# chongminggao/CIRS-codes

Hardware: AMD Instinct MI355X
Metric: simulator env-steps/s (collect + PPO update in the timed region), KuaishouEnv (higher is better)
Workload: dtype f32 (policy/tracker; rollout on the fp32 MFMA, PPO head products fp32-accurate from two fp16 pieces per operand (3 f16 MFMAs per product), fp32 accumulate) + f64 (env rewards, GAE)

## Files before the change

cirs-codes_amd/csrc/ppo.hip:

```cpp
#include "internal.h"
#include "optim.h"
#include "bf16x6.h"
#include "small_gemm.h"
#include "permutation.h"
#include "policy_kernels.h"

namespace cirs {
typedef float f32x4 __attribute__((ext_vector_type(4)));


constexpr int kBwdWaves = 4;
__host__ __device__ inline int n_row_blocks_of(int n_pad) { return (n_pad / kTileM + kBwdWaves - 1) / kBwdWaves; }
__host__ __device__ inline size_t dwa_slab_stride(int I) { return (((size_t)I * 64 + I) + 3) & ~(size_t)3; }
__host__ __device__ inline int n_dwa_slabs_of(int n_pad) { return n_row_blocks_of(n_pad); }

struct PpoLayout {
    long w1, b1, w2, b2, wa, ba, wc, bc, total, trunk;
};
__host__ __device__ inline PpoLayout ppo_layout(int I, int S) {
    PpoLayout L;
    L.w1 = 0; L.b1 = L.w1 + (long)kH * S; L.w2 = L.b1 + kH; L.b2 = L.w2 + (long)kH * kH;
    L.trunk = L.b2 + kH;
    L.wa = L.trunk; L.ba = L.wa + (long)I * kH; L.wc = L.ba + I; L.bc = L.wc + kH; L.total = L.bc + 1;
    return L;
// ... 350 lines not shown
#pragma unroll
    for (int off = 32; off > 0; off >>= 1) {
        const float om = __shfl_xor(m, off, CIRS_WAVE), os = __shfl_xor(s, off, CIRS_WAVE), ot = __shfl_xor(t, off, CIRS_WAVE);
        const float mn = fmaxf(m, om);
        if (mn > -INFINITY) {
            const float fa = __expf(m - mn), fb = __expf(om - mn);
            s = s * fa + os * fb; t = t * fa + ot * fb; m = mn;
        }
    }
    sRow[threadIdx.x >> 6][0][lane] = hl;
    sRow[threadIdx.x >> 6][1][lane] = wl;
    __builtin_amdgcn_wave_barrier();
    if (lane != 0) return;
    const float* hr = sRow[threadIdx.x >> 6][0];
    const float* wr = sRow[threadIdx.x >> 6][1];
    float z;
    if (za_in) {
        z = 0.f;
        for (int c = 0; c < n_chunks; ++c) {
            const float zc = za_in[(size_t)c * n_pad + j];
            if (zc == zc) z = zc;
        }
    } else {
        z = ba[a];
#pragma unroll
        for (int kk = 0; kk < 32; ++kk) {
            z = __builtin_fmaf(hr[kk], wr[kk], z);
            z = __builtin_fmaf(hr[32 + kk], wr[32 + kk], z);
        }
    }
    const float lse = m + __logf(s);
    v.lse[j] = lse;
    v.act[j] = a - item_base;
    v.dst_row[j] = (long)b.row_t[src] * n_env + b.row_env[src];
    const RowTerms rt = ppo_row_terms(cfg, z, lse, t / s, b.logp_old[src], b.adv[src], v.red[0], v.red[1], v.value[j], b.v_s[src], b.ret[src],
                                      1.0f / (float)mb_norm);
    v.clip_row[j] = rt.clip_row; v.c_logp[j] = rt.c_logp; v.vf_row[j] = rt.vf_row; v.dvalue[j] = rt.dvalue;
    v.c_ent[j] = rt.c_ent; v.h_ent[j] = rt.h_ent;
}

__device__ __forceinline__ float dz_of(float z, float lse, float c_logp, float c_ent, float h_ent, bool is_act, float& p_out) {
    const float p = __expf(z - lse);
    p_out = p;
    return c_logp * ((is_act ? 1.0f : 0.0f) - p) + c_ent * p * (z - lse + h_ent);
}

__device__ __forceinline__ void st_sc1(float* p, float a) { __hip_atomic_store(p, a, __ATOMIC_RELAXED, __HIP_MEMORY_SCOPE_AGENT); }
__device__ __forceinline__ float ld_sc1(const float* p) { return __hip_atomic_load(p, __ATOMIC_RELAXED, __HIP_MEMORY_SCOPE_AGENT); }
__device__ __forceinline__ float2 ld_sc1x2(const float* p) {
    const unsigned long long u = __hip_atomic_load(reinterpret_cast<const unsigned long long*>(p), __ATOMIC_RELAXED, __HIP_MEMORY_SCOPE_AGENT);
    return make_float2(__uint_as_float((unsigned)u), __uint_as_float((unsigned)(u >> 32)));
}
typedef unsigned wt_u32x4 __attribute__((ext_vector_type(4)));
struct WtBuf { __amdgpu_buffer_rsrc_t r; };
__device__ __forceinline__ WtBuf wt_buf(const void* base, unsigned bytes) {
    const unsigned long long a = reinterpret_cast<unsigned long long>(base);
    const unsigned lo = __builtin_amdgcn_readfirstlane((unsigned)a), hi = __builtin_amdgcn_readfirstlane((unsigned)(a >> 32));
    return WtBuf{__builtin_amdgcn_make_buffer_rsrc(reinterpret_cast<void*>(((unsigned long long)hi << 32) | lo), 0, (int)bytes, 0x00020000)};
}
__device__ __forceinline__ void st_wt16(const WtBuf& b, int byte_off, f32x4 x) {
    __builtin_amdgcn_raw_buffer_store_b128(__builtin_bit_cast(wt_u32x4, x), b.r, byte_off, 0, 16);
}
__device__ __forceinline__ void st_wt16(const WtBuf& b, int byte_off, uint4 x) { st_wt16(b, byte_off, __builtin_bit_cast(f32x4, x)); }

template <bool kWt = false> __device__ __forceinline__ void wa_planes_from_lds(int tile, uint4* __restrict__ planes, const float* sw);
__device__ __forceinline__ void wa_planes_block(int tile, int I, const float* __restrict__ wa, uint4* __restrict__ planes, float* sw) {
    const int tid = threadIdx.x, tile0 = tile * kTileN;
#pragma unroll
    for (int q = 0; q < 2; ++q) {
        const int f = tid + 256 * q, item = f >> 4, col = (f & 15) * 4;
        float4 t4 = make_float4(0.f, 0.f, 0.f, 0.f);
        if (tile0 + item < I) t4 = *reinterpret_cast<const float4*>(wa + (size_t)(tile0 + item) * kH + col);
        float* d = &sw[item * 65 + col];
        d[0] = t4.x; d[1] = t4.y; d[2] = t4.z; d[3] = t4.w;
    }
    __syncthreads();
    wa_planes_from_lds(tile, planes, sw);
}
template <bool kWt> __device__ __forceinline__ void wa_planes_from_lds(int tile, uint4* __restrict__ planes, const float* sw) {
    const int tid = threadIdx.x;
    uint4* out = planes + (size_t)tile * kPlaneTileU4;
    const WtBuf ob = wt_buf(out, kPlaneTileU4 * 16);
    {
        const float* r = &sw[(tid >> 3) * 65 + 8 * (tid & 7)];
        const HPl pl = hsplit8(kScWa * r[0], kScWa * r[1], kScWa * r[2], kScWa * r[3], kScWa * r[4], kScWa * r[5], kScWa * r[6], kScWa * r[7]);
        if constexpr (kWt) { st_wt16(ob, 16 * tid, __builtin_bit_cast(uint4, pl.h)); st_wt16(ob, 16 * (512 + tid), __builtin_bit_cast(uint4, pl.l)); }
        else { out[tid] = __builtin_bit_cast(uint4, pl.h); out[512 + tid] = __builtin_bit_cast(uint4, pl.l); }
    }
    {
        const int n = tid >> 2, t = (tid >> 1) & 1, hi = tid & 1;
        float x[8];
#pragma unroll
        for (int j = 0; j < 8; ++j) x[j] = kScWa * sw[acc_row(8 * t + j, hi) * 65 + n];
        const HPl pl = hsplit8(x[0], x[1], x[2], x[3], x[4], x[5], x[6], x[7]);
        if constexpr (kWt) { st_wt16(ob, 16 * (768 + tid), __builtin_bit_cast(uint4, pl.h)); st_wt16(ob, 16 * (1280 + tid), __builtin_bit_cast(uint4, pl.l)); }
        else { out[768 + tid] = __builtin_bit_cast(uint4, pl.h); out[1280 + tid] = __builtin_bit_cast(uint4, pl.l); }
    }
}

struct TrunkRowOut {
    float *h2, *value, *h1, *obs_copy;
    int32_t* act; long* dst;
    float* row4;
    uint4 *h2z, *h2b;
};
struct TrunkLds { const float* w1; int ld1; const float* w2; const float* wc; };

struct TrunkRowIn { int ri; float x; };
__device__ __forceinline__ TrunkRowIn trunk_row_gather(int j, int mb, const int32_t* __restrict__ idx, const float* __restrict__ obs_flat, long stride, int S,
                                                       int lane) {
    TrunkRowIn in;
    in.ri = idx[j < mb ? j : mb - 1];
    in.x = (j < mb && lane < S) ? obs_flat[(size_t)in.ri * stride + lane] : 0.f;
    return in;
}
__device__ __forceinline__ void trunk_row_pre(int S, const TrunkRowIn& in, int j, int mb, int n_pad, int lane, float* xs, const cirs_ppo_batch& bt, int n_env,
                                              const TrunkRowOut& o) {
    if (lane < S) {
        xs[lane] = in.x;
        o.obs_copy[(size_t)j * S + lane] = in.x;
    }
    if (o.act) {
        if (lane == 0) {
            o.act[j] = j < mb ? bt.act[in.ri] : 0;
            o.dst[j] = j < mb ? (long)bt.row_t[in.ri] * n_env + bt.row_env[in.ri] : 0;
        } else if (lane <= 4) {
            const float* srcp = lane == 1 ? bt.adv : lane == 2 ? bt.logp_old : lane == 3 ? bt.ret : bt.v_s;
            o.row4[(size_t)(lane - 1) * n_pad + j] = j < mb ? srcp[in.ri] : 0.f;
        }
    }
}
__device__ __forceinline__ void trunk_row_planes(float a, int j, int lane, const TrunkRowOut& o) {
    a *= kScH2;
    const uint32_t hp = cvt_pk_f16(a, 0.f) & 0xffffu;
    const float r1 = a - (float)__builtin_bit_cast(f16x2_b, hp).x;
    const uint32_t lp = cvt_pk_f16(r1, 0.f) & 0xffffu;
    const int tile = j >> 5, rr = j & 31, c = lane;
    unsigned short* z = reinterpret_cast<unsigned short*>(o.h2z + ((size_t)(tile * 12 + (c >> 4) * 3) * 64 + ((c >> 3) & 1) * 32 + rr)) + (c & 7);
    z[0] = (unsigned short)hp; z[2 * 64 * 8] = (unsigned short)lp;
    const int hi_b = (rr >> 2) & 1, sb = (rr & 3) + 4 * (rr >> 3);
    unsigned short* bq = reinterpret_cast<unsigned short*>(o.h2b + ((size_t)(tile * 12 + ((c >> 5) * 2 + (sb >> 3)) * 3) * 64 + hi_b * 32 + (c & 31))) + (sb & 7);
    bq[0] = (unsigned short)hp; bq[2 * 64 * 8] = (unsigned short)lp;
}
__device__ __forceinline__ void trunk_row_job(const cirs_policy_cfg& cfg, const cirs_policy_weights& w, const TrunkLds& L, const TrunkRowIn& in, int j, int mb,
                                              int n_pad, int lane, float* xs, float* hs, const cirs_ppo_batch& bt, int n_env, const TrunkRowOut& o) {
    trunk_row_pre(cfg.dim_state, in, j, mb, n_pad, lane, xs, bt, n_env, o);
    trunk_compute(cfg, w, xs, hs, lane, j, o.h2, o.value, o.h1, L.w1, L.ld1, L.w2, L.wc);
    trunk_row_planes(xs[lane], j, lane, o);
}
__global__ __launch_bounds__(256) void trunk_adv_kernel(cirs_policy_cfg cfg, cirs_policy_weights w, const float* __restrict__ obs_flat,
                                                        long stride, int n_pad, const int32_t* __restrict__ idx, int mb,
                                                        const float* __restrict__ adv_flat, const int32_t* __restrict__ sidx,
                                                        int m_stats, int enable, float* __restrict__ red, int n_row_wgs,
                                                        uint4* __restrict__ planes, cirs_ppo_batch bt, int n_env, TrunkRowOut out) {
    __shared__ float lds_raw[kTileN * 65];
    static_assert(kTileN * 65 >= 4 * 2 * kH, "the trunk rows use 4 x 2 x 64 floats of the same buffer");
    if ((int)blockIdx.x > n_row_wgs) {
        wa_planes_block((int)blockIdx.x - n_row_wgs - 1, cfg.n_items, w.wa, planes, lds_raw);
        return;
    }
    if ((int)blockIdx.x == n_row_wgs) {
        adv_stats_block(adv_flat, sidx, m_stats, enable, red, lds_raw);
        return;
    }
    __shared__ __attribute__((aligned(16))) float sW2[kH * kLdsRow2];
    __shared__ float sW1[kH * 33];
    __shared__ float sWc[kH];
    const int tid = threadIdx.x, lane = tid & 63, wv = tid >> 6, S = cfg.dim_state;
    const int j = blockIdx.x * 4 + wv;
    const int ld1 = S | 1;
    const bool al16 = (reinterpret_cast<uintptr_t>(w.w2) & 15) == 0;
    f32x4 t2[4];
    float t1[8];
#pragma unroll
    for (int q = 0; q < 4; ++q) {
        const float* p = w.w2 + (size_t)(tid + 256 * q) * 4;
        t2[q] = al16 ? *reinterpret_cast<const f32x4*>(p) : f32x4{p[0], p[1], p[2], p[3]};
    }
#pragma unroll
    for (int q = 0; q < 8; ++q) t1[q] = tid + 256 * q < kH * S ? w.w1[tid + 256 * q] : 0.f;
    const float tc = tid < kH ? w.wc[tid] : 0.f;
    const TrunkRowIn in = trunk_row_gather(j, mb, idx, obs_flat, stride, S, lane);
#pragma unroll
    for (int q = 0; q < 4; ++q) {
        const int i4 = tid + 256 * q;
        *reinterpret_cast<f32x4*>(&sW2[(i4 >> 4) * kLdsRow2 + (i4 & 15) * 4]) = t2[q];
    }
#pragma unroll
    for (int q = 0; q < 8; ++q) {
        const int i = tid + 256 * q;
        if (i < kH * S) sW1[(i / S) * ld1 + (i % S)] = t1[q];
    }
    if (tid < kH) sWc[tid] = tc;
    float (*rows)[2][kH] = reinterpret_cast<float (*)[2][kH]>(lds_raw);
    __syncthreads();
    trunk_row_job(cfg, w, TrunkLds{sW1, ld1, sW2, sWc}, in, j, mb, n_pad, lane, rows[wv][0], rows[wv][1], bt, n_env, out);
}

constexpr int kTStride = 36;
constexpr int kRSize = kTileN * kH + 2 * kTileN;
constexpr int kRowB = 144, kColB = 80;
constexpr int kRPlaneB = kTileN * kRowB, kCPlaneB = kH * kColB;
constexpr int kWBufB = 3 * kRPlaneB + 3 * kCPlaneB;

#ifdef CIRS_HEAD_PROF
__device__ unsigned long long g_step_prof[64];
#define CIRS_PSTAMP(COND, K) do { if ((COND) && threadIdx.x == 0) g_step_prof[K] = __builtin_amdgcn_s_memtime(); } while (0)
#else
#define CIRS_PSTAMP(COND, K) do { } while (0)
#endif
#ifdef CIRS_HEAD_PROF
__device__ unsigned long long g_head_prof[64];
#define CIRS_HSTAMP(K) do { if (blockIdx.x == 0 && blockIdx.y == 0 && threadIdx.x == 0 && it == 2) g_head_prof[K] = __builtin_amdgcn_s_memtime(); } while (0)
#define CIRS_HSTAMPB(K) do { if (blockIdx.x == 0 && blockIdx.y == 0 && threadIdx.x == 256 && it == 3) g_head_prof[K] = __builtin_amdgcn_s_memtime(); } while (0)
#define CIRS_TSTAMP(B, K) do { if ((int)blockIdx.x == (B) && threadIdx.x == 0) g_head_prof[K] = __builtin_amdgcn_s_memtime(); } while (0)
#define CIRS_SSTAMP(K) do { if (blockIdx.x == 0 && blockIdx.y == 0 && threadIdx.x == 0) g_head_prof[K] = __builtin_amdgcn_s_memtime(); } while (0)
#else
#define CIRS_HSTAMP(K) do { } while (0)
#define CIRS_HSTAMPB(K) do { } while (0)
#define CIRS_TSTAMP(B, K) do { } while (0)
#define CIRS_SSTAMP(K) do { } while (0)
#endif
template <bool kZout>
__global__ __launch_bounds__(256, 2) void head_stats_kernel(int I, int mb, int n_pad, int tiles_per_chunk,
                                                            const uint4* __restrict__ planes, const float* __restrict__ ba,
                                                            const uint4* __restrict__ h2z, ActorPartialView pv,
                                                            const int32_t* __restrict__ act_rows, float* __restrict__ za_out,
                                                            float4* __restrict__ zslab) {
    __shared__ __attribute__((aligned(16))) unsigned char sW[2][3 * kRPlaneB];
    __shared__ __attribute__((aligned(16))) float sB[2][kTileN];
    const int tid = threadIdx.x;
    CIRS_SSTAMP(40);
    const int lane = tid & 63, wv = tid >> 6;
    const int hi = lane >> 5, lo = lane & 31;
    const int row0 = (blockIdx.y * 4 + wv) * kTileM;
    const int chunk = blockIdx.x;
    const int jr = row0 + lo;
    const bool wave_ok = row0 < n_pad && (kZout || row0 < mb);
    const bool active = jr < mb;
    HPl hz[4];
    {
        const uint4* zp = h2z + (size_t)((wave_ok ? row0 : 0) >> 5) * 12 * 64 + lane;
#pragma unroll
        for (int s4 = 0; s4 < 4; ++s4) {
            HPL_SET(hz[s4], zp[(3 * s4) * 64], zp[(3 * s4 + 2) * 64]);
        }
    }
    float run_m = -INFINITY, run_s = 0.f, run_t = 0.f;
    const int act_r = (act_rows && active) ? act_rows[jr] : -1;
    float za_val = 0.f;
    bool za_have = false;
    const int first_tile = chunk * tiles_per_chunk * kTileN;
    const int n_tiles = max(0, min(tiles_per_chunk, (I - first_tile + kTileN - 1) / kTileN));
    const int dst_r = (tid >> 3) * kRowB + (tid & 7) * 16;
    uint4 g0, g2;
    float gb = 0.f;
#define CIRS_ISSUE(TILE0)                                                                                  \
    do {                                                                                                   \
        const uint4* src_ = planes + (size_t)((TILE0) / kTileN) * kPlaneTileU4 + tid;                      \
        g0 = src_[0]; g2 = src_[512];                                             \
        if (tid < kTileN) gb = ((TILE0) + tid) < I ? kScZ * ba[(TILE0) + tid] : 0.f;    \
    } while (0)
#define CIRS_COMMIT(BUF)                                                                                   \
    do {                                                                                                   \
        unsigned char* base_ = sW[BUF];                                                                    \
        *reinterpret_cast<uint4*>(base_ + dst_r) = g0;                                                     \
        \
        *reinterpret_cast<uint4*>(base_ + 2 * kRPlaneB + dst_r) = g2;                                      \
        if (tid < kTileN) sB[BUF][tid] = gb;                                                               \
    } while (0)
    CIRS_SSTAMP(41);
    if (n_tiles > 0) { CIRS_ISSUE(first_tile); CIRS_COMMIT(0); }
    __syncthreads();
    CIRS_SSTAMP(42);
    for (int it = 0; it < n_tiles; ++it) {
        const int buf = it & 1;
        const int tile0 = first_tile + it * kTileN;
        if (it == 2) CIRS_SSTAMP(43);
        if (it + 1 < n_tiles) CIRS_ISSUE(tile0 + kTileN);
        if (wave_ok) {
            const unsigned char* tw = sW[buf];
            HPl za[4];
#pragma unroll
            for (int s4 = 0; s4 < 4; ++s4) {
                const unsigned char* ap = tw + lo * kRowB + (16 * s4 + 8 * hi) * 2;
                HPL_SET(za[s4], *reinterpret_cast<const uint4*>(ap), *reinterpret_cast<const uint4*>(ap + 2 * kRPlaneB));
            }
            f32x16 acc, accs, acct;
#pragma unroll
            for (int r = 0; r < 16; ++r) { acc[r] = sB[buf][acc_row(r, hi)]; accs[r] = 0.f; acct[r] = 0.f; }
            if (it == 2) CIRS_SSTAMP(44);
            hmfma_split2(za[0], hz[0], za[1], hz[1], acc, accs, acct);
            hmfma_split2(za[2], hz[2], za[3], hz[3], acc, accs, acct);
#pragma unroll
            for (int r = 0; r < 16; ++r) acc[r] = acc[r] + (accs[r] + acct[r]);
            if (kZout) {
                const WtBuf zb = wt_buf(zslab + ((size_t)(tile0 / kTileN) * (n_pad / kTileM) + (row0 / kTileM)) * kZTileF4, kZTileF4 * 16);
#pragma unroll
                for (int q = 0; q < 4; ++q) st_wt16(zb, 16 * (q * 64 + lane), f32x4{acc[4 * q], acc[4 * q + 1], acc[4 * q + 2], acc[4 * q + 3]});
            }
#pragma unroll
            for (int r = 0; r < 16; ++r) acc[r] *= kScZi;
            if (it == 2) CIRS_SSTAMP(45);
            {
                const int arel = act_r - tile0;
                const bool mine = act_r >= 0 && arel >= 0 && arel < kTileN && ((arel >> 2) & 1) == hi;
                if (__any(mine)) {
                    const int rsel = (arel & 3) + 4 * (arel >> 3);
                    float zsel = acc[0];
// ... 1750 lines not shown
        }
    }
    acc = block_sum<256>(acc, sh);
    if (tid == 0) stats[blockIdx.x] = acc;
    if (blockIdx.x == 0 && tid < 8) {
        const long gi = P + tid;
        stats[kShardNormBlocks + tid] = (tid < 4 && gi >= begin && gi < begin + len) ? g_shard[gi - begin] : 0.f;
    }
}
__global__ __launch_bounds__(256) void shard_adam_kernel(float* __restrict__ p, const float* __restrict__ g, float* __restrict__ m,
                                                         float* __restrict__ v, long begin, long len, long n_first, long P, AdamSeg sa,
                                                         AdamSeg sb, float beta1, float beta2, float eps, cirs_ppo_cfg cfg,
                                                         const float* __restrict__ stats_all, int world, float* __restrict__ loss_out) {
    __shared__ float sh[256];
    const int tid = threadIdx.x;
    float acc = 0.f;
    const int n_part = world * kShardNormBlocks;
    for (int q = tid; q < n_part; q += 256) acc += stats_all[(size_t)(q / kShardNormBlocks) * kShardStatFloats + (q % kShardNormBlocks)];
    float total_norm;
    const float c = norm_coef(block_sum<256>(acc, sh), cfg, total_norm);
    if (blockIdx.x == 0 && tid == 0 && loss_out) {
        float t3[3] = {0.f, 0.f, 0.f};
        for (int r = 0; r < world; ++r)
            for (int j = 0; j < 3; ++j) t3[j] += stats_all[(size_t)r * kShardStatFloats + kShardNormBlocks + j];
        write_loss_row(loss_out, cfg, t3[0], t3[1], t3[2]);
    }
    const long i = blockIdx.x * (long)blockDim.x + threadIdx.x;
    if (i >= len || begin + i >= P) return;
    const AdamSeg sg = begin + i < n_first ? sa : sb;
    float gi = g[i];
    float pi = p[i], mi = m[i], vi = v[i];
    adam_elem_seg(pi, mi, vi, gi, sg, c, beta1, beta2, eps);
    p[i] = pi; m[i] = mi; v[i] = vi;
}

static int launch_adam(float* p, const float* g, float* m, float* v, long n, long step_before, int n_sub, float lr, float b1,
                       float b2, float eps, const float* grad_scale, int scale_pow, hipStream_t s) {
    CIRS_REQUIRE(n_sub == 1 || n_sub == 2, "n_sub must be 1 or 2");
    AdamBias ab[2] = {{0.f, 1.f, 1.f}, {0.f, 1.f, 1.f}};
    for (int q = 0; q < n_sub; ++q) ab[q] = adam_bias(lr, b1, b2, step_before + 1 + q);
    hipLaunchKernelGGL(adam_kernel, dim3(cdiv(n, 256)), dim3(256), 0, s, p, g, m, v, n, n_sub, b1, b2, eps, ab[0].step_size, ab[0].bc2s,
                       ab[1].step_size, ab[1].bc2s, grad_scale, scale_pow);
    CIRS_CHECK_LAUNCH("adam_kernel");
    return CIRS_OK;
}

#ifdef CIRS_HEAD_PROF
extern "C" int cirs_debug_step_prof(unsigned long long* out_host64) {
    return hipMemcpyFromSymbol(out_host64, HIP_SYMBOL(cirs::g_step_prof), 64 * sizeof(unsigned long long)) == hipSuccess ? 0 : -2;
}
extern "C" int cirs_debug_head_prof(unsigned long long* out_host32) {
    return hipMemcpyFromSymbol(out_host32, HIP_SYMBOL(cirs::g_head_prof), 64 * sizeof(unsigned long long)) == hipSuccess ? 0 : -2;
}
#endif

static int validate_ppo(const cirs_ppo_cfg* cfg) {
    CIRS_REQUIRE(cfg, "ppo cfg null");
    if (cfg->hidden != kH) return fail(CIRS_E_UNSUPPORTED, "this build supports hidden == 64 only");
    CIRS_REQUIRE(cfg->n_items > 0 && cfg->dim_state > 0 && cfg->dim_state <= 64, "bad n_items/dim_state");
    return CIRS_OK;
}

}

extern "C" int64_t cirs_ppo_param_count(const cirs_ppo_cfg* cfg) {
    if (!cfg) return 0;
    return cirs::ppo_layout(cfg->n_items, cfg->dim_state).total;
}

extern "C" int64_t cirs_ppo_workspace_bytes(const cirs_ppo_cfg* cfg, int32_t max_minibatch) {
    using namespace cirs;
    if (!cfg || max_minibatch <= 0) return 0;
    return (int64_t)(mb_ws_floats(n_pad_of(max_minibatch), cfg->n_items, cfg->dim_state) + 64 * 32) * 4;
}

extern "C" int cirs_ppo_prepare(const cirs_ppo_cfg* cfg, const cirs_traj* traj, const int32_t* lens,
                                const int32_t* offsets, int32_t n_env, int32_t max_turn, int32_t n_rows,
                                double* rms_state, const cirs_ppo_batch* out, void* stream) {
    using namespace cirs;
    if (int rc = validate_ppo(cfg)) return rc;
    CIRS_REQUIRE(traj && lens && offsets && rms_state && out, "null argument");
    CIRS_REQUIRE(out->obs && out->act && out->adv && out->ret && out->v_s && out->logp_old && out->row_env && out->row_t, "batch pointer null");
    CIRS_REQUIRE(n_env > 0 && max_turn > 0 && n_rows > 0, "bad sizes");
    hipStream_t s = (hipStream_t)stream;
    double* unnorm = nullptr;
    CIRS_HIP(hipMallocAsync((void**)&unnorm, sizeof(double) * (size_t)n_rows, s));
    hipLaunchKernelGGL(gae_kernel, dim3(cdiv(n_env, 64)), dim3(64), 0, s, *cfg, *traj, lens, offsets, n_env, cfg->dim_state,
                       rms_state, *out, unnorm);
    hipLaunchKernelGGL(compact_obs_kernel, dim3(cdiv((long)n_rows * cfg->dim_state, 256)), dim3(256), 0, s, *traj, *out, n_rows, n_env, cfg->dim_state);
    CIRS_CHECK_LAUNCH("gae_kernel");
    hipLaunchKernelGGL(returns_kernel, dim3(1), dim3(1024), 0, s, *cfg, unnorm, n_rows, rms_state, out->ret);
    CIRS_CHECK_LAUNCH("returns_kernel");
    CIRS_HIP(hipFreeAsync(unnorm, s));
    return CIRS_OK;
}

extern "C" int cirs_ppo_prepare_async_perms(const cirs_ppo_cfg* cfg, const cirs_traj* traj, const int32_t* lens, int32_t n_env, int32_t max_turn,
                                            int32_t* offsets_out, int32_t* n_rows_out, double* rms_state, const cirs_ppo_batch* out,
                                            double* scratch, uint64_t perm_seed, uint64_t perm_tag0, int32_t n_perm, int32_t* perm_out, int32_t offsets_ready,
                                            void* stream) {
    using namespace cirs;
    if (int rc = validate_ppo(cfg)) return rc;
    CIRS_REQUIRE(traj && lens && offsets_out && n_rows_out && rms_state && out && scratch, "null argument");
    CIRS_REQUIRE(out->obs && out->act && out->adv && out->ret && out->v_s && out->logp_old && out->row_env && out->row_t, "batch pointer null");
    CIRS_REQUIRE(n_env > 0 && n_env <= (1 << 20) && max_turn > 0, "bad sizes");
    CIRS_REQUIRE(n_perm >= 0 && n_perm <= kMaxPermKeys && (n_perm == 0 || perm_out), "permutations: at most 8 per call, perm_out non-null");
    hipStream_t s = (hipStream_t)stream;
    if (!offsets_ready) hipLaunchKernelGGL(offsets_kernel, dim3(1), dim3(1024), 0, s, lens, n_env, offsets_out, n_rows_out);
    hipLaunchKernelGGL(gae_kernel, dim3(cdiv(n_env, 64)), dim3(64), 0, s, *cfg, *traj, lens, (const int32_t*)offsets_out, n_env, cfg->dim_state,
                       rms_state, *out, scratch);
    const long upper = (long)n_env * max_turn;
    const int n_compact = (int)cdiv(upper * cfg->dim_state, 1024L);
    PermKeys keys{};
    for (int q = 0; q < n_perm; ++q) keys.k[q] = perm_key(perm_seed, perm_tag0 + (uint64_t)q);
    hipLaunchKernelGGL(prepare_tail_kernel, dim3(1 + n_compact + (int)cdiv((long)n_perm * upper, 1024L)), dim3(1024), 0, s, *cfg, *traj, *out, (const double*)scratch,
                       rms_state, (const int32_t*)n_rows_out, n_env, cfg->dim_state, n_compact, keys, (int)n_perm, upper, perm_out);
    CIRS_CHECK_LAUNCH("cirs_ppo_prepare_async");
    return CIRS_OK;
}
extern "C" int cirs_ppo_prepare_async(const cirs_ppo_cfg* cfg, const cirs_traj* traj, const int32_t* lens, int32_t n_env, int32_t max_turn,
                                      int32_t* offsets_out, int32_t* n_rows_out, double* rms_state, const cirs_ppo_batch* out,
                                      double* scratch, void* stream) {
    return cirs_ppo_prepare_async_perms(cfg, traj, lens, n_env, max_turn, offsets_out, n_rows_out, rms_state, out, scratch, 0, 0, 0, nullptr, 0, stream);
}

extern "C" int cirs_adam_step(float* params, const float* grads, float* m, float* v, int64_t n, int64_t step_before,
                              int32_t n_sub, float lr, float beta1, float beta2, float eps, const float* grad_scale,
                              int32_t scale_pow, void* stream) {
    using namespace cirs;
    CIRS_REQUIRE(params && grads && m && v && n > 0, "bad arguments");
    return launch_adam(params, grads, m, v, n, step_before, n_sub, lr, beta1, beta2, eps, grad_scale, scale_pow, (hipStream_t)stream);
}

struct PpoRun {
    const cirs_ppo_cfg* cfg;
    float *params, *grads, *adam_m, *adam_v;
    const cirs_ppo_batch* batch;
    int n_env;
    void* workspace;
    int n_pad_carve;
    hipStream_t s;
    int I, S;
    cirs::PpoLayout L;
    cirs_policy_cfg pcfg;
    cirs_policy_weights w;
    cirs::MbView v;
    float* tail;
    bool merge_launch;
    bool head_recompute;
    bool rows_kernel;
    bool learn_prefetch;
    int drop_arrival;
};
struct PpoStep { const int32_t* idx; int mb; const int32_t* sidx; int mb_norm; float* dobs; float* loss_out; long opt_step; };

static int env_int(const char* name, int unset) {
    const char* e = getenv(name);
    return e ? atoi(e) : unset;
}
static PpoRun ppo_run(const cirs_ppo_cfg* cfg, float* params, float* grads, float* adam_m, float* adam_v, const cirs_ppo_batch* batch, int n_env,
                      void* workspace, int max_mb, hipStream_t s) {
    using namespace cirs;
    PpoRun r;
    r.cfg = cfg; r.params = params; r.grads = grads; r.adam_m = adam_m; r.adam_v = adam_v; r.batch = batch; r.n_env = n_env; r.workspace = workspace;
    r.n_pad_carve = n_pad_of(max_mb); r.s = s; r.I = cfg->n_items; r.S = cfg->dim_state;
    r.L = ppo_layout(r.I, r.S);
    r.pcfg = cirs_policy_cfg{r.I, r.S, kH};
    r.w = cirs_policy_weights{params + r.L.w1, params + r.L.b1, params + r.L.w2, params + r.L.b2, params + r.L.wa, params + r.L.ba, params + r.L.wc,
                              params + r.L.bc};
    r.v = carve(workspace, r.n_pad_carve, r.I, r.S);
    r.tail = grads + r.L.total;
    r.merge_launch = env_int("CIRS_PPO_MERGE_KERNEL", 0) != 0;
    r.head_recompute = env_int("CIRS_PPO_HEAD_RECOMPUTE", 0) != 0;
    r.rows_kernel = env_int("CIRS_PPO_ROWS_KERNEL", 1) != 0;
    r.learn_prefetch = env_int("CIRS_PPO_LEARN_PREFETCH", 1) != 0;
    r.drop_arrival = env_int("CIRS_PPO_TEST_DROP_ARRIVAL", 0);
    return r;
}
static cirs::TrunkRowOut trunk_out_of(const cirs::MbView& v) { return cirs::TrunkRowOut{v.h2, v.value, v.h1, v.obs, v.act, v.dst_row, v.adv, v.h2z, v.h2b}; }
static long head_seg(const PpoRun& r) { return (long)r.I * cirs::kH + r.I; }

static int launch_trunk_adv(const PpoRun& r, const PpoStep& st, const cirs::TrunkRowOut& out) {
    using namespace cirs;
    const int n_pad = n_pad_of(st.mb);
    hipLaunchKernelGGL(trunk_adv_kernel, dim3(cdiv(n_pad, 4) + 1 + cdiv(r.I, kTileN)), dim3(256), 0, r.s, r.pcfg, r.w, (const float*)r.batch->obs, (long)r.S,
                       n_pad, st.idx, st.mb, (const float*)r.batch->adv, st.sidx, st.mb_norm, (int)r.cfg->norm_adv, r.v.red, (int)cdiv(n_pad, 4),
                       r.v.wa_planes, *r.batch, r.n_env, out);
    CIRS_CHECK_LAUNCH("trunk_adv_kernel");
    return CIRS_OK;
}
static int launch_head_stats(const PpoRun& r, const PpoStep& st, const int32_t* act_rows, float* za_out, cirs::HeadMergeArgs* hma) {
    using namespace cirs;
    const int n_pad = n_pad_of(st.mb), n_slabs = n_row_blocks_of(n_pad), n_item_tiles = cdiv(r.I, kTileN);
    const int tpc_s = head_tiles_per_chunk(n_item_tiles, n_slabs, 2);
    const int n_schunks = cdiv(n_item_tiles, tpc_s);
    *hma = HeadMergeArgs{*r.cfg, *r.batch, st.idx, st.mb_norm, n_schunks, partial_view(r.v.head_ws, n_pad, r.I)};
    const auto stats_fn = r.head_recompute ? head_stats_kernel<false> : head_stats_kernel<true>;
    CIRS_PROF_LAUNCH(2, r.s, hipLaunchKernelGGL(stats_fn, dim3(n_schunks, n_slabs), dim3(256), 0, r.s, r.I, st.mb, n_pad, tpc_s, (const uint4*)r.v.wa_planes,
                                                r.w.ba, (const uint4*)r.v.h2z, hma->pv, act_rows, za_out, r.v.zslab));
    CIRS_CHECK_LAUNCH("head_stats_kernel");
    return CIRS_OK;
}
static int launch_head_bwd(const PpoRun& r, const PpoStep& st, const cirs::HeadMergeArgs& hma, bool merge, int* n_bchunks_out) {
    using namespace cirs;
    const int n_pad = n_pad_of(st.mb), n_slabs = n_row_blocks_of(n_pad), n_item_tiles = cdiv(r.I, kTileN);
    const int tpc = head_tiles_per_chunk(n_item_tiles, n_slabs, 1);
    const int n_bchunks = cdiv(n_item_tiles, tpc);
    const dim3 bgrid((n_bchunks + 7) & ~7, n_slabs), bblock(head_bwd_threads(!r.head_recompute));
    const HeadBwdFn bwd_fn = head_bwd_fn(r.cfg->ent_coef != 0.f, merge, !r.head_recompute);
    CIRS_PROF_LAUNCH(1, r.s, hipLaunchKernelGGL(bwd_fn, bgrid, bblock, 0, r.s, r.I, st.mb, n_pad, tpc, (const uint4*)r.v.wa_planes, (const float*)r.w.ba, r.v,
                                                r.v.dwap, hma));
    CIRS_CHECK_LAUNCH("head_bwd_fused_kernel");
    *n_bchunks_out = n_bchunks;
    return CIRS_OK;
}
static int launch_dh2_sum(const PpoRun& r, const PpoStep& st, int n_bchunks, float* tp_dh2 = nullptr, float* tp_ent = nullptr) {
    using namespace cirs;
    const int n_pad = n_pad_of(st.mb);
    hipLaunchKernelGGL(dh2_sum_kernel, dim3(n_pad * (kH / 4) / 64 + cdiv(n_pad, 64)), dim3(64), 0, r.s, st.mb, n_pad, n_bchunks, r.v, tp_dh2, tp_ent);
    CIRS_CHECK_LAUNCH("dh2_sum_kernel");
    return CIRS_OK;
}
static cirs::DwJobs trunk_dw_jobs(const PpoRun& r, int n_pad) {
    using namespace cirs;
    const MbView& v = r.v;
    DwJobs jobs{};
    jobs.n = 3;
    jobs.j[0] = DwJob{v.dvalue, 1, v.h2, kH, 1, kH, r.grads + r.L.wc, r.grads + r.L.bc, 0, 0};
    jobs.j[1] = DwJob{v.da2, kH, v.h1, kH, kH, kH, r.grads + r.L.w2, r.grads + r.L.b2, 0, 0};
    jobs.j[2] = DwJob{v.da1, kH, v.obs, r.S, kH, r.S, r.grads + r.L.w1, r.grads + r.L.b1, 0, 0};
    const int n_dw_slabs = n_pad / kTileM;
    int off = 0, out = 0;
    for (int q = 0; q < 3; ++q) {
        jobs.j[q].part_off = off;
        off += n_dw_slabs * jobs.j[q].O * (jobs.j[q].K + 1);
        out += jobs.j[q].O * (jobs.j[q].K + 1);
    }
    jobs.total_out = out;
    return jobs;
}
static int launch_trunk_bwd(const PpoRun& r, const PpoStep& st, const cirs::MbView& v, int n_chunks, bool wa_sum) {
    using namespace cirs;
    static_assert(kH == 64, "trunk_bwd_kernel tiles assume hidden == 64");
    CIRS_REQUIRE(r.S <= 32, "dim_state > 32 is not supported by the trunk backward kernel");
    const int n_pad = n_pad_of(st.mb), n_slabs = n_row_blocks_of(n_pad);
    hipLaunchKernelGGL(trunk_bwd_kernel, dim3(n_pad / kTileM + (wa_sum ? kWaSumBlocks : 0)), dim3(512), 0, r.s, st.mb, n_pad, n_chunks, r.S, r.w.w1, r.w.w2,
                       r.w.wc, v, st.dobs, r.grads, (long)r.L.wa, head_seg(r), (long)dwa_slab_stride(r.I), n_slabs, trunk_dw_jobs(r, n_pad), v.dwp);
    CIRS_CHECK_LAUNCH("trunk_bwd_kernel");
    return CIRS_OK;
}
static bool rows_kernel_wanted(const PpoRun& r, int mb) {
    return cirs::n_pad_of(mb) / cirs::kRR <= cirs::kSyncA0 && r.rows_kernel;
}
static int launch_trunk_rows(const PpoRun& r, const PpoStep& st, int n_bchunks, bool with_loss_partials) {
    using namespace cirs;
    CIRS_REQUIRE(r.S <= 32, "dim_state > 32 is not supported by the trunk backward kernel");
    const int n_pad = n_pad_of(st.mb), n_slabs = n_row_blocks_of(n_pad);
    const long seg = head_seg(r);
    const int n_r = n_pad / kRR, n_f = cdiv(snap_floats(r.S), kFOut);
    CIRS_REQUIRE(n_r <= kSyncA0, "trunk_rows_kernel: more than 2048 rows in a minibatch (one arrival flag per 8 rows)");
    const long n4 = seg >> 2;
    int n_w = (int)cdiv(n4, 512L);
    n_w = n_w > kWaSlotsMax ? kWaSlotsMax : n_w;
    n_w = std::min(n_w, std::max(64, device_cu_count() - n_r));
    hipLaunchKernelGGL(trunk_rows_kernel, dim3(n_r + n_w + n_f + (with_loss_partials ? 1 : 0)), dim3(512), 0, r.s, st.mb, n_pad, n_bchunks, r.S, r.w.w1,
                       r.w.w2, r.w.wc, r.v, st.dobs, r.grads, (long)r.L.wa, seg, (long)dwa_slab_stride(r.I), n_slabs, n_r, snap_stride(r.S),
                       with_loss_partials ? r.tail : (float*)nullptr, st.mb_norm, n_w);
    CIRS_CHECK_LAUNCH("trunk_rows_kernel");
    return CIRS_OK;
}
static int launch_dw_final_loss(const PpoRun& r, const PpoStep& st) {
    using namespace cirs;
    const int n_pad = n_pad_of(st.mb);
    const DwJobs jobs = trunk_dw_jobs(r, n_pad);
    hipLaunchKernelGGL(dw_multi_final, dim3(cdiv(jobs.total_out, 256)), dim3(256), 0, r.s, jobs, n_pad / kTileM, (const float*)r.v.dwp);
    CIRS_CHECK_LAUNCH("dw_multi_final");
    hipLaunchKernelGGL(loss_partials_kernel, dim3(1), dim3(256), 0, r.s, st.mb, st.mb_norm, r.v, r.tail);
    CIRS_CHECK_LAUNCH("loss_partials_kernel");
    return CIRS_OK;
}
static int launch_sumsq(const PpoRun& r, const PpoStep& st, bool from_slabs) {
    using namespace cirs;
    const int n_pad = n_pad_of(st.mb);
    const DwJobs jobs = from_slabs ? trunk_dw_jobs(r, n_pad) : DwJobs{};
    hipLaunchKernelGGL(sumsq_partial_kernel, dim3(kNormBlocks), dim3(256), 0, r.s, r.grads, r.L.trunk, r.L.total, r.L.wa, head_seg(r), (int)from_slabs, jobs,
                       from_slabs ? n_pad / kTileM : 0, from_slabs ? (const float*)r.v.dwp : (const float*)nullptr, r.S, r.v.normp);
    CIRS_CHECK_LAUNCH("sumsq_partial_kernel");
    return CIRS_OK;
}
static cirs::AdamSeg adam_seg_of(const cirs_ppo_cfg* cfg, long step_before, int n_sub, int scale_pow) {
    cirs::AdamSeg sg{n_sub, scale_pow, 0.f, 1.f, 0.f, 1.f, 1.f, 1.f};
    for (int q = 0; q < n_sub; ++q) {
        const cirs::AdamBias ab = cirs::adam_bias(cfg->lr, cfg->beta1, cfg->beta2, step_before + 1 + q);
        if (q == 0) { sg.step_size0 = ab.step_size; sg.bc2s0 = ab.bc2s; sg.rbc2s0 = ab.rbc2s; }
        else { sg.step_size1 = ab.step_size; sg.bc2s1 = ab.bc2s; sg.rbc2s1 = ab.rbc2s; }
    }
    return sg;
}
static int launch_norm_adam(const PpoRun& r, const PpoStep& st, int phase, bool folded, const PpoStep* next) {
    using namespace cirs;
    const MbView& v = r.v;
    if (!(phase == 0 && folded)) { if (int rc = launch_sumsq(r, st, phase == 0)) return rc; }
    const AdamSeg sa = adam_seg_of(r.cfg, 2 * st.opt_step, 2, 2), sb = adam_seg_of(r.cfg, st.opt_step, 1, 1);
    AdamNext nx{};
    nx.n_p = cdiv(r.I, kTileN);
    nx.planes = v.wa_planes;
    if (next) {
        const int np = n_pad_of(next->mb);
        nx.n_t = np / kTrunkRowsPerWg; nx.n_s = 1;
        nx.pcfg = r.pcfg; nx.obs_flat = r.batch->obs; nx.idx = next->idx; nx.mb = next->mb; nx.n_pad = np;
        nx.adv_flat = r.batch->adv; nx.sidx = next->sidx; nx.m_stats = next->mb_norm; nx.enable = (int)r.cfg->norm_adv; nx.red = v.red;
        nx.bt = *r.batch; nx.n_env = r.n_env; nx.out = trunk_out_of(v); nx.s_magic = (65536 + r.S - 1) / r.S;
        nx.drop_arrival = r.drop_arrival;
    }
    nx.n_a0 = cdiv(r.L.trunk + kH + 1, 256);
    const int n_a = nx.n_a0 + cdiv(r.I, 256);
    const AdamArgs aa{r.params, r.grads, r.adam_m, r.adam_v, r.L, sa, sb, r.cfg->beta1, r.cfg->beta2, r.cfg->adam_eps, *r.cfg, v.normp, r.tail, st.loss_out,
                      phase == 0 ? st.mb : 0, st.mb_norm};
    hipLaunchKernelGGL(adam_next_kernel, dim3(nx.n_t + nx.n_s + nx.n_p + n_a), dim3(256), 0, r.s, aa, v, nx);
    CIRS_CHECK_LAUNCH("adam_next_kernel");
    return CIRS_OK;
}

static int launch_step_grads(const PpoRun& r, const PpoStep& st, bool head_done, bool for_allreduce) {
    using namespace cirs;
    const int n_pad = n_pad_of(st.mb);
    HeadMergeArgs hma;
    int n_bchunks = 0;
    if (!head_done) { if (int rc = launch_trunk_adv(r, st, trunk_out_of(r.v))) return rc; }
    if (int rc = launch_head_stats(r, st, r.v.act, r.v.za, &hma)) return rc;
    if (r.merge_launch) {
        hipLaunchKernelGGL(head_stats_merge_kernel, dim3(cdiv(n_pad, 4)), dim3(256), 0, r.s, *r.cfg, *r.batch, st.idx, st.mb, st.mb_norm, n_pad, hma.n_schunks,
                           r.n_env, hma.pv, r.w.wa, r.w.ba, r.v, (const float*)nullptr, 0);
        CIRS_CHECK_LAUNCH("head_stats_merge_kernel");
    }
    if (int rc = launch_head_bwd(r, st, hma, !r.merge_launch, &n_bchunks)) return rc;
    if (rows_kernel_wanted(r, st.mb)) return launch_trunk_rows(r, st, n_bchunks, for_allreduce);
    if (int rc = launch_dh2_sum(r, st, n_bchunks)) return rc;
    if (int rc = launch_trunk_bwd(r, st, r.v, n_bchunks, true)) return rc;
    return for_allreduce ? launch_dw_final_loss(r, st) : CIRS_OK;
}
static int launch_step(const PpoRun& r, const PpoStep& st, bool head_done, const PpoStep* next) {
    if (int rc = launch_step_grads(r, st, head_done, false)) return rc;
    return launch_norm_adam(r, st, 0, rows_kernel_wanted(r, st.mb), next);
}

struct DpChain { int max_mb; int head_done; const int32_t* next_idx; int next_mb; const int32_t* next_idx_global; int next_mb_global; };
static int ppo_minibatch_impl(const cirs_ppo_cfg* cfg, float* params, float* grads, float* adam_m, float* adam_v, int64_t opt_step,
                              const cirs_ppo_batch* batch, const int32_t* idx, int32_t mb, const int32_t* idx_global,
                              int32_t mb_global, float* dobs_accum, int32_t n_env, float* loss_out, void* workspace,
                              int64_t workspace_bytes, int phase, void* stream, const DpChain* ch = nullptr) {
    using namespace cirs;
    if (int rc = validate_ppo(cfg)) return rc;
    CIRS_REQUIRE(params && grads && adam_m && adam_v && batch && loss_out && workspace, "null argument");
    CIRS_REQUIRE(phase >= 0 && phase <= 2, "phase must be 0, 1 or 2");
    CIRS_REQUIRE(mb >= 1 && mb_global >= 2 && mb <= mb_global, "bad minibatch sizes (need mb_global >= 2 for the unbiased std)");
    const int carve_mb = ch ? (ch->max_mb > mb ? ch->max_mb : mb) : mb;
    CIRS_REQUIRE(!ch || !ch->next_idx || ch->next_mb <= carve_mb, "next minibatch larger than max_mb");
    CIRS_REQUIRE(workspace_bytes >= cirs_ppo_workspace_bytes(cfg, carve_mb), "workspace too small");
    const PpoRun r = ppo_run(cfg, params, grads, adam_m, adam_v, batch, n_env, workspace, carve_mb, (hipStream_t)stream);
    const PpoStep st{idx, (int)mb, idx_global ? idx_global : idx, (int)(idx_global ? mb_global : mb), dobs_accum, loss_out, (long)opt_step};
    if (phase == 2) {
        if (!(ch && ch->next_idx)) return launch_norm_adam(r, st, 2, false, nullptr);
        const PpoStep nxt{ch->next_idx, ch->next_mb, ch->next_idx_global ? ch->next_idx_global : ch->next_idx,
                          ch->next_idx_global ? ch->next_mb_global : ch->next_mb, nullptr, nullptr, (long)opt_step + 1};
        return launch_norm_adam(r, st, 2, false, &nxt);
    }
    const bool head_done = ch && ch->head_done;
    CIRS_REQUIRE(idx != nullptr || head_done, "idx is null");
    if (phase == 1) return launch_step_grads(r, st, head_done, true);
    return launch_step(r, st, head_done, nullptr);
}

extern "C" int cirs_ppo_minibatch(const cirs_ppo_cfg* cfg, float* params, float* grads, float* adam_m, float* adam_v,
                                  int64_t opt_step, const cirs_ppo_batch* batch, const int32_t* idx, int32_t mb,
                                  float* dobs_accum, int32_t n_env, float* loss_out, void* workspace,
                                  int64_t workspace_bytes, void* stream) {
    if (mb < 2) return cirs::fail(CIRS_E_INVALID, "minibatch needs >= 2 rows (unbiased std)");
    return ppo_minibatch_impl(cfg, params, grads, adam_m, adam_v, opt_step, batch, idx, mb, nullptr, mb, dobs_accum, n_env, loss_out,
                              workspace, workspace_bytes, 0, stream);
}

static int ppo_slice_count(int n, int bs) {
    int k = 0;
    const bool merge_last = n % bs > 0;
    for (int s0 = 0; s0 < n; s0 += bs) { ++k; if (merge_last && s0 + 2 * bs >= n) break; }
    return k;
}
static void ppo_slice(int n, int bs, int k, int* b, int* e) {
    const bool merge_last = n % bs > 0;
    const int s0 = k * bs;
    *b = s0;
    *e = (merge_last && s0 + 2 * bs >= n) ? n : (s0 + bs < n ? s0 + bs : n);
}
extern "C" int cirs_ppo_handoff_status(int32_t* lost_out, int32_t reset, void* stream) {
    CIRS_REQUIRE(lost_out, "cirs_ppo_handoff_status: lost_out is null");
    hipLaunchKernelGGL(cirs::handoff_status_kernel, dim3(1), dim3(1), 0, (hipStream_t)stream, (int*)lost_out, (int)reset);
    CIRS_CHECK_LAUNCH("handoff_status_kernel");
    return CIRS_OK;
}

extern "C" int cirs_ppo_update_readback(const int32_t* lens, int32_t n_env, int32_t* lens_host_pinned, int32_t* lost_host_pinned, int32_t* offsets_out,
                                        int32_t* n_rows_out, void* stream) {
    CIRS_REQUIRE(lens && lens_host_pinned && n_env > 0 && (!offsets_out == !n_rows_out), "cirs_ppo_update_readback: bad arguments");
    if (offsets_out) {
        CIRS_REQUIRE(n_env <= (1 << 20), "cirs_ppo_update_readback: n_env");
        hipLaunchKernelGGL(cirs::update_readback_offsets_kernel, dim3(1), dim3(1024), 0, (hipStream_t)stream, lens, (int)n_env, lens_host_pinned, lost_host_pinned,
                           offsets_out, n_rows_out);
    } else
    hipLaunchKernelGGL(cirs::update_readback_kernel, dim3(cirs::cdiv(n_env, 256)), dim3(256), 0, (hipStream_t)stream, lens, (int)n_env, lens_host_pinned,
                       lost_host_pinned);
    CIRS_CHECK_LAUNCH("update_readback_kernel");
    return CIRS_OK;
}

extern "C" int32_t cirs_ppo_learn_steps(int32_t n_rows, int32_t batch_size, int32_t n_repeat) {
    if (n_rows < 1 || batch_size < 1 || n_repeat < 1) return 0;
    return n_repeat * ppo_slice_count(n_rows, batch_size);
}
extern "C" int cirs_ppo_learn(const cirs_ppo_cfg* cfg, float* params, float* grads, float* adam_m, float* adam_v, int64_t opt_step,
                              const cirs_ppo_batch* batch, const int32_t* perms, int32_t n_rows, int32_t batch_size, int32_t n_repeat,
                              float* dobs_accum, int64_t dobs_floats, int32_t n_env, float* losses, void* workspace, int64_t workspace_bytes,
                              void* stream) {
    using namespace cirs;
    if (int rc = validate_ppo(cfg)) return rc;
    CIRS_REQUIRE(params && grads && adam_m && adam_v && batch && perms && losses && workspace, "null argument");
    CIRS_REQUIRE(n_rows >= 2 && batch_size >= 2 && n_repeat >= 1, "need n_rows >= 2, batch_size >= 2, n_repeat >= 1");
    CIRS_REQUIRE(!dobs_accum || dobs_floats > 0, "dobs_floats must be the size of dobs_accum");
    const int n_sl = ppo_slice_count(n_rows, batch_size);
    int max_mb = 0;
    for (int k = 0; k < n_sl; ++k) { int b, e; ppo_slice(n_rows, batch_size, k, &b, &e); CIRS_REQUIRE(e - b >= 2, "a minibatch of one row has no unbiased std"); max_mb = e - b > max_mb ? e - b : max_mb; }
    CIRS_REQUIRE(workspace_bytes >= cirs_ppo_workspace_bytes(cfg, max_mb), "workspace too small");
    const PpoRun r = ppo_run(cfg, params, grads, adam_m, adam_v, batch, n_env, workspace, max_mb, (hipStream_t)stream);
    const bool prefetch = r.learn_prefetch && !r.merge_launch;
    const int n_steps = n_repeat * n_sl;
    auto step_of = [&](int k) {
        const int rep = k / n_sl;
        int b, e; ppo_slice(n_rows, batch_size, k % n_sl, &b, &e);
        const int32_t* idx = perms + (size_t)rep * n_rows + b;
        return PpoStep{idx, e - b, idx, e - b, (dobs_accum && rep == n_repeat - 1) ? dobs_accum : nullptr, losses + 4 * (size_t)k, (long)(opt_step + k)};
    };
    bool have_head = false;
    for (int k = 0; k < n_steps; ++k) {
        const PpoStep st = step_of(k);
        if (dobs_accum && k == (n_repeat - 1) * n_sl) {
            if (hipMemsetAsync(dobs_accum, 0, sizeof(float) * (size_t)dobs_floats, r.s) != hipSuccess) return fail(CIRS_E_LAUNCH, "hipMemsetAsync(dobs_accum)");
        }
        const bool has_next = prefetch && k + 1 < n_steps;
        const PpoStep nxt = has_next ? step_of(k + 1) : PpoStep{};
        if (int rc = launch_step(r, st, have_head, has_next ? &nxt : nullptr)) return rc;
        have_head = has_next;
    }
    return CIRS_OK;
}

extern "C" int cirs_ppo_minibatch_dp(const cirs_ppo_cfg* cfg, float* params, float* grads, float* adam_m, float* adam_v,
                                     int64_t opt_step, const cirs_ppo_batch* batch, const int32_t* idx_local, int32_t mb_local,
                                     const int32_t* idx_global, int32_t mb_global, float* dobs_accum, int32_t n_env,
                                     float* loss_out, void* workspace, int64_t workspace_bytes, int32_t phase, void* stream) {
    if (phase != 2 && !idx_global) return cirs::fail(CIRS_E_INVALID, "idx_global is null");
    return ppo_minibatch_impl(cfg, params, grads, adam_m, adam_v, opt_step, batch, idx_local, mb_local, idx_global, mb_global,
                              dobs_accum, n_env, loss_out, workspace, workspace_bytes, phase, stream);
}

extern "C" int cirs_ppo_minibatch_dp_chain(const cirs_ppo_cfg* cfg, float* params, float* grads, float* adam_m, float* adam_v, int64_t opt_step,
                                           const cirs_ppo_batch* batch, const int32_t* idx_local, int32_t mb_local, const int32_t* idx_global,
                                           int32_t mb_global, float* dobs_accum, int32_t n_env, float* loss_out, void* workspace,
                                           int64_t workspace_bytes, int32_t phase, int32_t max_mb_local, int32_t head_done,
                                           const int32_t* next_idx_local, int32_t next_mb_local, const int32_t* next_idx_global,
                                           int32_t next_mb_global, void* stream) {
    if (phase != 1 && phase != 2) return cirs::fail(CIRS_E_INVALID, "phase must be 1 or 2");
    if (phase == 1 && !idx_global) return cirs::fail(CIRS_E_INVALID, "idx_global is null");
    if (next_idx_local && (!next_idx_global || next_mb_local < 1 || next_mb_global < 2)) return cirs::fail(CIRS_E_INVALID, "bad next minibatch");
    const DpChain ch{(int)max_mb_local, (int)head_done, next_idx_local, (int)next_mb_local, next_idx_global, (int)next_mb_global};
    return ppo_minibatch_impl(cfg, params, grads, adam_m, adam_v, opt_step, batch, idx_local, mb_local, idx_global, mb_global, dobs_accum, n_env,
                              loss_out, workspace, workspace_bytes, phase, stream, &ch);
}

extern "C" int64_t cirs_ppo_tp_exchange_floats(int32_t n_rows, int32_t world) {
    return (int64_t)cirs::n_pad_of(n_rows) * (cirs::kH + 1) + (int64_t)world * cirs::kWaSumBlocks;
}

extern "C" int cirs_ppo_minibatch_tp(const cirs_ppo_cfg* cfg, float* params, float* grads, float* adam_m, float* adam_v, int64_t opt_step,
                                     const cirs_ppo_batch* batch, const int32_t* idx, int32_t mb, int32_t item_base, int32_t rank,
                                     int32_t world, float* stats4, const float* stats_all, float* red, float* dobs_accum, int32_t n_env,
                                     float* loss_out, void* workspace, int64_t workspace_bytes, int32_t phase, void* stream) {
    using namespace cirs;
    if (int rc = validate_ppo(cfg)) return rc;
    CIRS_REQUIRE(params && grads && adam_m && adam_v && batch && idx && workspace && red, "null argument");
    CIRS_REQUIRE(phase >= 1 && phase <= 3, "phase must be 1, 2 or 3");
    CIRS_REQUIRE(mb >= 2 && world >= 1 && rank >= 0 && rank < world && item_base >= 0, "bad minibatch / rank arguments");
    CIRS_REQUIRE(workspace_bytes >= cirs_ppo_workspace_bytes(cfg, mb), "workspace too small");
    CIRS_REQUIRE(cfg->dim_state <= 32, "dim_state > 32 is not supported by the trunk backward kernel");
    const PpoRun r = ppo_run(cfg, params, grads, adam_m, adam_v, batch, n_env, workspace, mb, (hipStream_t)stream);
    const PpoStep st{idx, (int)mb, idx, (int)mb, dobs_accum, loss_out, (long)opt_step};
    const MbView& v = r.v;
    const int n_pad = n_pad_of(mb);
    float* red_dh2 = red;
    float* red_ent = red + (size_t)n_pad * kH;
    float* red_slots = red_ent + n_pad;
    if (phase == 1) {
        CIRS_REQUIRE(stats4, "stats4 is null");
        if (int rc = launch_trunk_adv(r, st, TrunkRowOut{v.h2, v.value, v.h1, v.obs, nullptr, nullptr, nullptr, v.h2z, v.h2b})) return rc;
        HeadMergeArgs hma;
        if (int rc = launch_head_stats(r, st, nullptr, nullptr, &hma)) return rc;
        hipLaunchKernelGGL(head_tp_fold_kernel, dim3(cdiv(n_pad, 4)), dim3(256), 0, r.s, *batch, idx, (int)mb, n_pad, hma.n_schunks, hma.pv, (const float*)r.w.wa,
                           (const float*)r.w.ba, (int)item_base, r.I, (const float*)v.h2, stats4);
        CIRS_CHECK_LAUNCH("head_tp_fold_kernel");
        return CIRS_OK;
    }
    if (phase == 2) {
        CIRS_REQUIRE(stats_all, "stats_all is null");
        ActorPartialView pa{};
        pa.m = const_cast<float*>(stats_all); pa.s = pa.m + (size_t)world * n_pad; pa.score = pa.s + (size_t)world * n_pad;
        const float* za = pa.score + (size_t)world * n_pad;
        hipLaunchKernelGGL(head_stats_merge_kernel, dim3(cdiv(n_pad, 4)), dim3(256), 0, r.s, *cfg, *batch, idx, (int)mb, (int)mb, n_pad, (int)world,
                           (int)n_env, pa, (const float*)nullptr, (const float*)nullptr, v, za, (int)item_base);
        CIRS_CHECK_LAUNCH("head_stats_merge_kernel");
        int n_bchunks = 0;
        if (int rc = launch_head_bwd(r, st, HeadMergeArgs{}, false, &n_bchunks)) return rc;
        CIRS_HIP(hipMemsetAsync(red_slots, 0, sizeof(float) * (size_t)world * kWaSumBlocks, r.s));
        if (int rc = launch_dh2_sum(r, st, n_bchunks, red_dh2, red_ent)) return rc;
        hipLaunchKernelGGL(wa_slab_sum_kernel, dim3(kWaSumBlocks), dim3(512), 0, r.s, grads, (long)r.L.wa, head_seg(r), (const float*)v.dwap,
                           (long)dwa_slab_stride(r.I), n_row_blocks_of(n_pad), red_slots + (size_t)rank * kWaSumBlocks);
        CIRS_CHECK_LAUNCH("wa_slab_sum_kernel");
        return CIRS_OK;
    }
    CIRS_REQUIRE(loss_out, "loss_out is null");
    hipLaunchKernelGGL(tp_post_kernel, dim3(cdiv(n_pad, 256)), dim3(256), 0, r.s, (int)mb, n_pad, (int)world, (const float*)red_ent, (const float*)red_slots, v);
    CIRS_CHECK_LAUNCH("tp_post_kernel");
    MbView v3 = v;
    v3.dh2p = red_dh2;
    if (int rc = launch_trunk_bwd(r, st, v3, 1, false)) return rc;
    if (int rc = launch_sumsq(r, st, true)) return rc;
    hipLaunchKernelGGL(adam2_kernel, dim3(cdiv(r.L.total, 256)), dim3(256), 0, r.s, params, grads, adam_m, adam_v, r.L.total, r.L.trunk,
                       adam_seg_of(cfg, 2 * opt_step, 2, 2), adam_seg_of(cfg, opt_step, 1, 1), cfg->beta1, cfg->beta2, cfg->adam_eps, *cfg, v.normp, r.tail, v3,
                       loss_out, (int)mb, (int)mb);
    CIRS_CHECK_LAUNCH("adam2_kernel");
    return CIRS_OK;
}

extern "C" int32_t cirs_ppo_shard_stat_floats(void) { return cirs::kShardStatFloats; }

extern "C" int cirs_ppo_shard_norm(const cirs_ppo_cfg* cfg, const float* grads_shard, int64_t shard_begin, int64_t shard_len,
                                   float* stats_out, void* stream) {
    using namespace cirs;
    if (int rc = validate_ppo(cfg)) return rc;
    CIRS_REQUIRE(grads_shard && stats_out && shard_begin >= 0 && shard_len > 0, "bad shard arguments");
    const PpoLayout L = ppo_layout(cfg->n_items, cfg->dim_state);
    hipLaunchKernelGGL(shard_sumsq_kernel, dim3(kShardNormBlocks), dim3(256), 0, (hipStream_t)stream, grads_shard, (long)shard_begin,
                       (long)shard_len, L.trunk, L.total, stats_out);
    CIRS_CHECK_LAUNCH("shard_sumsq_kernel");
    return CIRS_OK;
}

extern "C" int cirs_ppo_shard_adam(const cirs_ppo_cfg* cfg, float* params_shard, const float* grads_shard, float* adam_m_shard,
                                   float* adam_v_shard, int64_t shard_begin, int64_t shard_len, int64_t opt_step,
                                   const float* stats_all, int32_t world, float* loss_out, void* stream) {
    using namespace cirs;
    if (int rc = validate_ppo(cfg)) return rc;
    CIRS_REQUIRE(params_shard && grads_shard && adam_m_shard && adam_v_shard && stats_all, "null argument");
    CIRS_REQUIRE(shard_begin >= 0 && shard_len > 0 && world >= 1, "bad shard arguments");
    const PpoLayout L = ppo_layout(cfg->n_items, cfg->dim_state);
    hipLaunchKernelGGL(shard_adam_kernel, dim3(cdiv(shard_len, 256)), dim3(256), 0, (hipStream_t)stream, params_shard, grads_shard,
                       adam_m_shard, adam_v_shard, (long)shard_begin, (long)shard_len, L.trunk, L.total, adam_seg_of(cfg, 2 * opt_step, 2, 2),
                       adam_seg_of(cfg, opt_step, 1, 1), cfg->beta1, cfg->beta2, cfg->adam_eps, *cfg, stats_all, (int)world, loss_out);
    CIRS_CHECK_LAUNCH("shard_adam_kernel");
    return CIRS_OK;
}
```

cirs-codes_amd/csrc/tracker_bwd.hip:

```cpp
#include <algorithm>
#include "tracker_rows.h"
#include "rng.h"

namespace cirs {

#ifdef CIRS_TBWD_PROF
__device__ unsigned long long g_tbwd_prof[64];
#define CIRS_BSTAMP(K) do { if ((int)blockIdx.x == 300 && threadIdx.x == 0) g_tbwd_prof[K] = __builtin_amdgcn_s_memtime(); } while (0)
__device__ unsigned long long g_tbwd_wg[2048 * 3];
#define CIRS_BWG(SEL, WHICH) do { if ((SEL) && threadIdx.x == 0 && blockIdx.x < 2048) { g_tbwd_wg[blockIdx.x * 3 + (WHICH)] = __builtin_amdgcn_s_memtime(); \
    if ((WHICH) == 0) { unsigned hw; asm volatile("s_getreg_b32 %0, hwreg(HW_REG_HW_ID)" : "=s"(hw)); unsigned xcc; asm volatile("s_getreg_b32 %0, hwreg(HW_REG_XCC_ID)" : "=s"(xcc)); g_tbwd_wg[blockIdx.x * 3 + 2] = ((unsigned long long)xcc << 32) | hw; } } } while (0)
#else
#define CIRS_BSTAMP(K) do { } while (0)
#define CIRS_BWG(SEL, WHICH) do { } while (0)
#endif
constexpr int kChunkRows = 256;

struct DropCfg {
    int on;
    uint32_t thr;
    float inv;
    uint64_t seed;
    int env_base;
};
// ... 148 lines not shown
    __builtin_amdgcn_fence(__ATOMIC_ACQUIRE, "wavefront");
    const int half = lane >> 5, d = lane & (tD - 1), hd = d / HD;
    float acc = 0.f;
    for (int j0 = half; j0 <= p; j0 += 16) {
        float k8[8];
#pragma unroll
        for (int u = 0; u < 8; ++u) k8[u] = j0 + 2 * u <= p ? QKV[(size_t)(base + j0 + 2 * u) * 96 + tD + d] : 0.f;
#pragma unroll
        for (int u = 0; u < 8; ++u)
            if (j0 + 2 * u <= p) acc = __builtin_fmaf(sds[hd * Lp + j0 + 2 * u], k8[u], acc);
    }
    acc += __shfl_xor(acc, 32, CIRS_WAVE);
    if (lane < tD) dQKV[(size_t)r * 96 + d] = acc * scale;
}

template <int NH>
__global__ __launch_bounds__(256) void attn_bwd_kv(const float* __restrict__ QKV, const float* __restrict__ P, const float* __restrict__ dS,
                                                   const float* __restrict__ dATT, const int32_t* __restrict__ row_env,
                                                   const int32_t* __restrict__ row_t, const int32_t* __restrict__ offsets,
                                                   const int32_t* __restrict__ lens, int R, int Lp, float* __restrict__ dQKV) {
    constexpr int HD = tD / NH;
    const int lane = threadIdx.x & 63;
    const int r = blockIdx.x * 4 + (threadIdx.x >> 6);
    if (r >= R) return;
    const int b = row_env[r], pk = row_t[r], base = offsets[b], len = lens[b];
    const float scale = 1.0f / sqrtf((float)HD);
    const int d = lane & (tD - 1), which = lane >> 5, h = d / HD;
    const float* coef = (which == 0 ? dS : P) + ((size_t)base * NH + h) * Lp + pk;
    const float* vec = which == 0 ? QKV + (size_t)base * 96 + d : dATT + (size_t)base * tD + d;
    const size_t cstride = (size_t)NH * Lp, vstride = which == 0 ? 96 : tD;
    const float cs = which == 0 ? scale : 1.0f;
    float acc = 0.f;
    int p = pk;
    for (; p < len; p += 8) {
        float c8[8], v8[8];
#pragma unroll
        for (int u = 0; u < 8; ++u) {
            const bool ok = p + u < len;
            c8[u] = ok ? coef[(size_t)(p + u) * cstride] : 0.f;
            v8[u] = ok ? vec[(size_t)(p + u) * vstride] : 0.f;
        }
#pragma unroll
        for (int u = 0; u < 8; ++u)
            if (p + u < len) acc = __builtin_fmaf(c8[u] * cs, v8[u], acc);
    }
    dQKV[(size_t)r * 96 + tD + lane] = acc;
}

template <int NH> struct EpGeo {
    static constexpr int NW = NH < 4 ? NH : 4;
    static constexpr int SL = 64 / NW;
    static constexpr int HPL = NH / NW;
    static constexpr int HD = tD / NH;
    static constexpr int DPL = HPL * HD;
    __host__ __device__ static constexpr int strip(int Lp) { return (HPL * Lp) | 1; }
    __host__ __device__ static constexpr size_t keep_words(int Lp) { return 2 * (size_t)NH * Lp; }
    __host__ __device__ static constexpr size_t fwd_floats(int Lp) { return (size_t)Lp * 64 + (size_t)NW * (Lp + 1) * strip(Lp) + keep_words(Lp); }
    __host__ __device__ static constexpr size_t bwd_floats(int Lp) { return (size_t)Lp * 128 + (size_t)NW * (Lp + 1) * strip(Lp) + 2 * (size_t)NH * Lp + keep_words(Lp); }
};

__device__ __forceinline__ void ep_stage(float* __restrict__ dst, const float* __restrict__ src, int rows, int src_stride, int cols, int tid, int nt) {
    const int c4n = cols >> 2;
    for (int i = tid; i < rows * c4n; i += nt) {
        const int row = i / c4n, c4 = i - row * c4n;
        *reinterpret_cast<f32x4*>(dst + (size_t)row * cols + 4 * c4) = *reinterpret_cast<const f32x4*>(src + (size_t)row * src_stride + 4 * c4);
    }
}
template <int COLS, int NQ>
__device__ __forceinline__ void ep_stage_issue(f32x4 (&r)[NQ], const float* __restrict__ src, int rows, int src_stride, int tid) {
    constexpr int c4n = COLS >> 2;
    static_assert(NQ * 64 >= 32 * c4n, "registers for 32 rows");
    const int n = rows * c4n;
#pragma unroll
    for (int q = 0; q < NQ; ++q) {
        const int i = min(tid + 64 * q, n - 1), row = i / c4n, c4 = i - row * c4n;
        r[q] = *reinterpret_cast<const f32x4*>(src + (size_t)row * src_stride + 4 * c4);
    }
}
template <int COLS, int NQ>
__device__ __forceinline__ void ep_stage_commit(float* __restrict__ dst, const f32x4 (&r)[NQ], int rows, int tid) {
    constexpr int c4n = COLS >> 2;
    const int n = rows * c4n;
#pragma unroll
    for (int q = 0; q < NQ; ++q) {
        const int i = tid + 64 * q, row = i / c4n, c4 = i - row * c4n;
        if (i < n) *reinterpret_cast<f32x4*>(dst + (size_t)row * COLS + 4 * c4) = r[q];
    }
}
__device__ __forceinline__ void ep_wave_sync() {
    asm volatile("s_waitcnt lgkmcnt(0)" ::: "memory");
    __builtin_amdgcn_wave_barrier();
}
template <int N> __device__ __forceinline__ void ep_load(float (&v)[N], const float* __restrict__ src) {
#pragma unroll
    for (int d4 = 0; d4 < N / 4; ++d4) {
        const f32x4 t = *reinterpret_cast<const f32x4*>(src + 4 * d4);
        v[4 * d4] = t.x; v[4 * d4 + 1] = t.y; v[4 * d4 + 2] = t.z; v[4 * d4 + 3] = t.w;
    }
}
template <int N> __device__ __forceinline__ void ep_store(float* __restrict__ dst, const float (&v)[N], float a) {
#pragma unroll
    for (int d4 = 0; d4 < N / 4; ++d4)
        *reinterpret_cast<f32x4*>(dst + 4 * d4) = f32x4{v[4 * d4] * a, v[4 * d4 + 1] * a, v[4 * d4 + 2] * a, v[4 * d4 + 3] * a};
}
__device__ __forceinline__ float ep_exp2(float x) { return __builtin_amdgcn_exp2f(x); }
template <int HD> __device__ __forceinline__ float ep_dot(const float* a, const float* b) {
    float s = 0.f;
#pragma unroll
    for (int d = 0; d < HD; ++d) s = __builtin_fmaf(a[d], b[d], s);
    return s;
}
template <int NH>
__device__ __forceinline__ void ep_keep_build(uint32_t* __restrict__ sK, int len, int b, int layer, const DropCfg& dc, int tid, int nt) {
    for (int i = tid; i < len * NH * 2; i += nt) sK[i] = 0u;
    ep_wave_sync();
    const int half = (len + 1) >> 1;
    const int bpr = (((len + 1) * NH + 3) >> 2) + 1;
    for (int i = tid; i < half * bpr; i += nt) {
        const int fr = i / bpr, g0 = i - fr * bpr;
        const int pA = fr, pB = len - 1 - fr;
        const int nA = ((pA + 1) * NH + 3) >> 2, nB = pB > pA ? ((pB + 1) * NH + 3) >> 2 : 0;
        const bool inA = g0 < nA;
        const int p = inA ? pA : pB, g = inA ? g0 : g0 - nA;
        if (g0 < nA + nB) {
            const u32x4 r = dropout_block(dc.seed, (uint32_t)(dc.env_base + b), (uint32_t)p, (uint32_t)layer, (uint32_t)CIRS_DROP_ATTN, (uint32_t)g);
#pragma unroll
            for (int wd = 0; wd < 4; ++wd) {
                const int elem = 4 * g + wd, j = elem / NH, h = elem - j * NH;
                if (j <= p && block_word(r, (uint32_t)wd) >= dc.thr) atomicOr(&sK[(p * NH + h) * 2 + (j >> 5)], 1u << (j & 31));
            }
        }
    }
    ep_wave_sync();
}
template <int NH>
__device__ __forceinline__ void ep_keep_build_row(uint32_t* __restrict__ sK, int p, int b, int layer, const DropCfg& dc, int tid, int nt) {
    for (int i = tid; i < NH * 2; i += nt) sK[i] = 0u;
    __syncthreads();
    for (int g = tid; 4 * g < (p + 1) * NH; g += nt) {
        const u32x4 r = dropout_block(dc.seed, (uint32_t)(dc.env_base + b), (uint32_t)p, (uint32_t)layer, (uint32_t)CIRS_DROP_ATTN, (uint32_t)g);
#pragma unroll
        for (int wd = 0; wd < 4; ++wd) {
            const int elem = 4 * g + wd, j = elem / NH, h = elem - j * NH;
            if (j <= p && block_word(r, (uint32_t)wd) >= dc.thr) atomicOr(&sK[h * 2 + (j >> 5)], 1u << (j & 31));
        }
    }
    __syncthreads();
}
__device__ __forceinline__ bool ep_keep_bit(const uint32_t (&m)[2], int j) { return ((j < 32 ? m[0] : m[1]) >> (j & 31)) & 1u; }

template <int NH, bool kDrop>
__global__ __launch_bounds__(64) void attn_fwd_ep(const float* __restrict__ QKV, const int32_t* __restrict__ offsets,
                                                  const int32_t* __restrict__ lens, int Lp, float* __restrict__ ATT, DropCfg dc, int layer,
                                                  uint32_t* __restrict__ keep_out ) {
    using G = EpGeo<NH>;
    constexpr int HPL = G::HPL, DPL = G::DPL, HD = G::HD, SL = G::SL;
    extern __shared__ __attribute__((aligned(16))) float smem[];
    const int b = blockIdx.x, len = lens[b];
    if (len <= 0) return;
    const int lane = threadIdx.x, hg = lane / SL, slot = lane - hg * SL;
    const int base = offsets[b], STR = G::strip(Lp);
    float* sKV = smem;
    float* sS = smem + (size_t)Lp * 64;
    uint32_t* sK = reinterpret_cast<uint32_t*>(sS + (size_t)G::NW * (Lp + 1) * STR);
    const int len32 = min(len, 32);
    f32x4 st_kv[8];
    ep_stage_issue<64, 8>(st_kv, QKV + (size_t)base * 96 + tD, len32, 96, lane);
    if (kDrop) {
        ep_keep_build<NH>(sK, len, b, layer, dc, lane, 64);
        if (keep_out)
            for (int i = lane; i < len * NH * 2; i += 64) keep_out[(size_t)base * NH * 2 + i] = sK[i];
    }
    ep_stage_commit<64, 8>(sKV, st_kv, len32, lane);
    if (len > 32) ep_stage(sKV + 32 * 64, QKV + (size_t)(base + 32) * 96 + tD, len - 32, 96, 64, lane, 64);
    __syncthreads();
    const float scale = 1.0f / sqrtf((float)HD), qs = scale * 1.4426950408889634f;
    for (int s0 = 0; 2 * s0 < len; s0 += SL) {
        const int pA = s0 + slot, pB = len - 1 - pA;
        const bool actA = pA <= pB, actB = pA < pB;
        const int rA = actA ? pA : 0, rB = actB ? pB : 0;
        const int jn = len - s0;
        float* myA = sS + ((size_t)hg * (Lp + 1) + (actA ? pA : Lp)) * STR;
        float* myB = sS + ((size_t)hg * (Lp + 1) + (actB ? pB : Lp)) * STR;
        float qA[DPL], qB[DPL];
        ep_load(qA, QKV + (size_t)(base + rA) * 96 + hg * DPL);
        ep_load(qB, QKV + (size_t)(base + rB) * 96 + hg * DPL);
#pragma unroll
        for (int d = 0; d < DPL; ++d) { qA[d] *= qs; qB[d] *= qs; }
        float mxA[HPL], mxB[HPL], smA[HPL], smB[HPL];
#pragma unroll
        for (int h = 0; h < HPL; ++h) { mxA[h] = mxB[h] = -INFINITY; smA[h] = smB[h] = 0.f; }
        float kq[DPL];
        ep_load(kq, sKV + hg * DPL);
#pragma unroll 4
        for (int j = 0; j < jn; ++j) {
            float k[DPL];
#pragma unroll
            for (int d = 0; d < DPL; ++d) k[d] = kq[d];
            ep_load(kq, sKV + (size_t)(j + 1 < jn ? j + 1 : j) * 64 + hg * DPL);
            const bool inA = actA && j <= pA, inB = actB && j <= pB;
#pragma unroll
            for (int h = 0; h < HPL; ++h) {
                const float sa = ep_dot<HD>(qA + h * HD, k + h * HD), sb = ep_dot<HD>(qB + h * HD, k + h * HD);
                myA[h * Lp + j] = sa; myB[h * Lp + j] = sb;
                mxA[h] = inA ? fmaxf(mxA[h], sa) : mxA[h];
                mxB[h] = inB ? fmaxf(mxB[h], sb) : mxB[h];
            }
        }
        float accA[DPL], accB[DPL];
#pragma unroll
        for (int d = 0; d < DPL; ++d) accA[d] = accB[d] = 0.f;
        uint32_t kmA[HPL][2], kmB[HPL][2];
        if (kDrop) {
#pragma unroll
            for (int h = 0; h < HPL; ++h) {
                kmA[h][0] = sK[(rA * NH + hg * HPL + h) * 2]; kmA[h][1] = sK[(rA * NH + hg * HPL + h) * 2 + 1];
                kmB[h][0] = sK[(rB * NH + hg * HPL + h) * 2]; kmB[h][1] = sK[(rB * NH + hg * HPL + h) * 2 + 1];
            }
        }
        float vq[DPL];
        ep_load(vq, sKV + 32 + hg * DPL);
#pragma unroll 4
        for (int j = 0; j < jn; ++j) {
            float v[DPL];
#pragma unroll
            for (int d = 0; d < DPL; ++d) v[d] = vq[d];
            ep_load(vq, sKV + (size_t)(j + 1 < jn ? j + 1 : j) * 64 + 32 + hg * DPL);
            const bool inA = actA && j <= pA, inB = actB && j <= pB;
#pragma unroll
            for (int h = 0; h < HPL; ++h) {
                float ea = ep_exp2(myA[h * Lp + j] - mxA[h]), eb = ep_exp2(myB[h * Lp + j] - mxB[h]);
                ea = inA ? ea : 0.f; eb = inB ? eb : 0.f;
                smA[h] += ea; smB[h] += eb;
                if (kDrop) {
                    if (!ep_keep_bit(kmA[h], j)) ea = 0.f;
                    if (!ep_keep_bit(kmB[h], j)) eb = 0.f;
                }
#pragma unroll
                for (int d = 0; d < HD; ++d) {
                    accA[h * HD + d] = __builtin_fmaf(ea, v[h * HD + d], accA[h * HD + d]);
                    accB[h * HD + d] = __builtin_fmaf(eb, v[h * HD + d], accB[h * HD + d]);
                }
            }
        }
#pragma unroll
        for (int h = 0; h < HPL; ++h) {
            const float ia = (kDrop ? dc.inv : 1.0f) / smA[h], ib = (kDrop ? dc.inv : 1.0f) / smB[h];
#pragma unroll
            for (int d = 0; d < HD; ++d) { accA[h * HD + d] *= ia; accB[h * HD + d] *= ib; }
        }
        if (actA) ep_store(ATT + (size_t)(base + pA) * tD + hg * DPL, accA, 1.0f);
        if (actB) ep_store(ATT + (size_t)(base + pB) * tD + hg * DPL, accB, 1.0f);
    }
}

template <int NH, bool kDrop>
__global__ __launch_bounds__(64) void attn_bwd_ep(const float* __restrict__ QKV, const float* __restrict__ dATT,
                                                  const int32_t* __restrict__ offsets, const int32_t* __restrict__ lens, int Lp,
                                                  float* __restrict__ dQKV, DropCfg dc, int layer,
                                                  const uint32_t* __restrict__ keep_in ) {
    using G = EpGeo<NH>;
    constexpr int HPL = G::HPL, DPL = G::DPL, HD = G::HD, SL = G::SL;
    extern __shared__ __attribute__((aligned(16))) float smem[];
    const int b = blockIdx.x, len = lens[b];
    if (len <= 0) return;
    const int lane = threadIdx.x, hg = lane / SL, slot = lane - hg * SL;
    const int base = offsets[b], STR = G::strip(Lp);
    float* sQKV = smem;
    float* sdA = smem + (size_t)Lp * 96;
    float* sS = sdA + (size_t)Lp * 32;
    float* sM = sS + (size_t)G::NW * (Lp + 1) * STR;
    float* sI = sM + (size_t)NH * Lp;
    uint32_t* sK = reinterpret_cast<uint32_t*>(sI + (size_t)NH * Lp);
    CIRS_BWG(layer == 1, 0);
    CIRS_BSTAMP(39);
    const int len32 = min(len, 32);
    f32x4 st_q[12], st_d[4];
    ep_stage_issue<96, 12>(st_q, QKV + (size_t)base * 96, len32, 96, lane);
    ep_stage_issue<tD, 4>(st_d, dATT + (size_t)base * tD, len32, tD, lane);
    CIRS_BSTAMP(38);
    if (kDrop) {
        if (keep_in) {
            for (int i = lane; i < len * NH * 2; i += 64) sK[i] = keep_in[(size_t)base * NH * 2 + i];
        } else {
            ep_keep_build<NH>(sK, len, b, layer, dc, lane, 64);
        }
    }
    ep_stage_commit<96, 12>(sQKV, st_q, len32, lane);
    ep_stage_commit<tD, 4>(sdA, st_d, len32, lane);
    if (len > 32) {
        ep_stage(sQKV + 32 * 96, QKV + (size_t)(base + 32) * 96, len - 32, 96, 96, lane, 64);
        ep_stage(sdA + 32 * tD, dATT + (size_t)(base + 32) * tD, len - 32, tD, tD, lane, 64);
    }
    __syncthreads();
    CIRS_BSTAMP(40);
    const float scale = 1.0f / sqrtf((float)HD), qs = scale * 1.4426950408889634f;
    const float dinv = kDrop ? dc.inv : 1.0f;
    for (int s0 = 0; 2 * s0 < len; s0 += SL) {
        const int pA = s0 + slot, pB = len - 1 - pA;
        const bool actA = pA <= pB, actB = pA < pB;
        const int rA = actA ? pA : 0, rB = actB ? pB : 0;
        const int jn = len - s0;
        float* myA = sS + ((size_t)hg * (Lp + 1) + (actA ? pA : Lp)) * STR;
        float* myB = sS + ((size_t)hg * (Lp + 1) + (actB ? pB : Lp)) * STR;
        float qA[DPL], qB[DPL], daA[DPL], daB[DPL];
        ep_load(qA, sQKV + (size_t)rA * 96 + hg * DPL);
        ep_load(qB, sQKV + (size_t)rB * 96 + hg * DPL);
        ep_load(daA, sdA + (size_t)rA * tD + hg * DPL);
        ep_load(daB, sdA + (size_t)rB * tD + hg * DPL);
#pragma unroll
// ... 58 lines not shown
            dotA[h] *= invA[h]; dotB[h] *= invB[h];
            if (actA) { sM[((size_t)hg * Lp + pA) * HPL + h] = mxA[h]; sI[((size_t)hg * Lp + pA) * HPL + h] = invA[h]; }
            if (actB) { sM[((size_t)hg * Lp + pB) * HPL + h] = mxB[h]; sI[((size_t)hg * Lp + pB) * HPL + h] = invB[h]; }
        }
        float dqA[DPL], dqB[DPL];
#pragma unroll
        for (int d = 0; d < DPL; ++d) dqA[d] = dqB[d] = 0.f;
        ep_load(kq, sQKV + 32 + hg * DPL);
        ep_load(vq, sQKV + 64 + hg * DPL);
#pragma unroll 4
        for (int j = 0; j < jn; ++j) {
            float k[DPL], v[DPL];
#pragma unroll
            for (int d = 0; d < DPL; ++d) { k[d] = kq[d]; v[d] = vq[d]; }
            ep_load(kq, sQKV + (size_t)(j + 1 < jn ? j + 1 : j) * 96 + 32 + hg * DPL);
            ep_load(vq, sQKV + (size_t)(j + 1 < jn ? j + 1 : j) * 96 + 64 + hg * DPL);
            const bool inA = actA && j <= pA, inB = actB && j <= pB;
#pragma unroll
            for (int h = 0; h < HPL; ++h) {
                float dpa = ep_dot<HD>(daA + h * HD, v + h * HD), dpb = ep_dot<HD>(daB + h * HD, v + h * HD);
                if (kDrop) {
                    dpa = (inA && ep_keep_bit(kmA[h], j)) ? dpa * dinv : 0.f;
                    dpb = (inB && ep_keep_bit(kmB[h], j)) ? dpb * dinv : 0.f;
                }
                float dsa = myA[h * Lp + j] * invA[h] * (dpa - dotA[h]), dsb = myB[h * Lp + j] * invB[h] * (dpb - dotB[h]);
                dsa = inA ? dsa : 0.f; dsb = inB ? dsb : 0.f;
                myA[h * Lp + j] = dsa; myB[h * Lp + j] = dsb;
#pragma unroll
                for (int d = 0; d < HD; ++d) {
                    dqA[h * HD + d] = __builtin_fmaf(dsa, k[h * HD + d], dqA[h * HD + d]);
                    dqB[h * HD + d] = __builtin_fmaf(dsb, k[h * HD + d], dqB[h * HD + d]);
                }
            }
        }
        if (actA) ep_store(dQKV + (size_t)(base + pA) * 96 + hg * DPL, dqA, scale);
        if (actB) ep_store(dQKV + (size_t)(base + pB) * 96 + hg * DPL, dqB, scale);
    }
    __syncthreads();
    CIRS_BSTAMP(41);
    for (int s0 = 0; 2 * s0 < len; s0 += SL) {
        const int jA = s0 + slot, jB = len - 1 - jA;
        const bool actA = jA <= jB, actB = jA < jB;
        const int rA = actA ? jA : 0, rB = actB ? jB : 0;
        float kA[DPL], kB[DPL], dKA[DPL], dVA[DPL], dKB[DPL], dVB[DPL];
        ep_load(kA, sQKV + (size_t)rA * 96 + 32 + hg * DPL);
        ep_load(kB, sQKV + (size_t)rB * 96 + 32 + hg * DPL);
#pragma unroll
        for (int d = 0; d < DPL; ++d) { kA[d] *= qs; kB[d] *= qs; dKA[d] = dVA[d] = dKB[d] = dVB[d] = 0.f; }
        float qn[DPL], dn[DPL];
        ep_load(qn, sQKV + (size_t)s0 * 96 + hg * DPL);
        ep_load(dn, sdA + (size_t)s0 * tD + hg * DPL);
#pragma unroll 4
        for (int pq = s0; pq < len; ++pq) {
            float q[DPL], da[DPL];
#pragma unroll
            for (int d = 0; d < DPL; ++d) { q[d] = qn[d]; da[d] = dn[d]; }
            ep_load(qn, sQKV + (size_t)(pq + 1 < len ? pq + 1 : pq) * 96 + hg * DPL);
            ep_load(dn, sdA + (size_t)(pq + 1 < len ? pq + 1 : pq) * tD + hg * DPL);
            const size_t st = ((size_t)hg * Lp + pq), ss = ((size_t)hg * (Lp + 1) + pq) * STR;
            const bool inA = actA && pq >= jA, inB = actB && pq >= jB;
#pragma unroll
            for (int h = 0; h < HPL; ++h) {
                const float m = sM[st * HPL + h], iv = sI[st * HPL + h];
                float pa = ep_exp2(fminf(ep_dot<HD>(q + h * HD, kA + h * HD) - m, 0.f)) * iv;
                float pb = ep_exp2(fminf(ep_dot<HD>(q + h * HD, kB + h * HD) - m, 0.f)) * iv;
                pa = inA ? pa : 0.f; pb = inB ? pb : 0.f;
                if (kDrop) {
                    const uint32_t* kw = sK + (pq * NH + hg * HPL + h) * 2;
                    pa = (inA && ((kw[rA >> 5] >> (rA & 31)) & 1u)) ? pa * dinv : 0.f;
                    pb = (inB && ((kw[rB >> 5] >> (rB & 31)) & 1u)) ? pb * dinv : 0.f;
                }
                float dsa = sS[ss + h * Lp + rA], dsb = sS[ss + h * Lp + rB];
                dsa = inA ? dsa : 0.f; dsb = inB ? dsb : 0.f;
#pragma unroll
                for (int d = 0; d < HD; ++d) {
                    dKA[h * HD + d] = __builtin_fmaf(dsa, q[h * HD + d], dKA[h * HD + d]);
                    dVA[h * HD + d] = __builtin_fmaf(pa, da[h * HD + d], dVA[h * HD + d]);
                    dKB[h * HD + d] = __builtin_fmaf(dsb, q[h * HD + d], dKB[h * HD + d]);
                    dVB[h * HD + d] = __builtin_fmaf(pb, da[h * HD + d], dVB[h * HD + d]);
                }
            }
        }
        if (actA) {
            float* o = dQKV + (size_t)(base + jA) * 96 + 32 + hg * DPL;
            ep_store(o, dKA, scale); ep_store(o + 32, dVA, 1.0f);
        }
        if (actB) {
            float* o = dQKV + (size_t)(base + jB) * 96 + 32 + hg * DPL;
            ep_store(o, dKB, scale); ep_store(o + 32, dVB, 1.0f);
        }
    }
    CIRS_BSTAMP(42);
    CIRS_BWG(layer == 1, 1);
}
#undef EP_KEEP

constexpr int kRowT = 132;
__device__ __forceinline__ void mm_block(sg_f32x16& acc, const float (&a)[16], const float* __restrict__ wr) {
    float bv[16];
    ep_load(bv, wr);
#pragma unroll
    for (int j = 0; j < 16; ++j) acc = __builtin_amdgcn_mfma_f32_32x32x2f32(a[j], bv[j], acc, 0, 0, 0);
}
__device__ __forceinline__ void acc_to_lds(float* __restrict__ sT, const sg_f32x16& acc, int col, int hi) {
#pragma unroll
    for (int s = 0; s < 16; ++s) sT[acc_row(s, hi) * kRowT + col] = acc[s];
}
__device__ __forceinline__ void ln_half_row(const float (&y)[16], const float* __restrict__ g, const float* __restrict__ b, int hi,
                                            float (&xh)[16], float (&out)[16], float& rs) {
    float sum = 0.f;
#pragma unroll
    for (int j = 0; j < 16; ++j) sum += y[j];
    sum += __shfl_xor(sum, 32, CIRS_WAVE);
    const float mean = sum * (1.0f / tD);
    float q = 0.f;
#pragma unroll
    for (int j = 0; j < 16; ++j) { const float t = y[j] - mean; q = __builtin_fmaf(t, t, q); }
    q += __shfl_xor(q, 32, CIRS_WAVE);
    rs = 1.0f / sqrtf(q * (1.0f / tD) + 1e-5f);
    float gg[16], bb[16];
    ep_load(gg, g + 16 * hi);
    ep_load(bb, b + 16 * hi);
#pragma unroll
    for (int j = 0; j < 16; ++j) { xh[j] = (y[j] - mean) * rs; out[j] = xh[j] * gg[j] + bb[j]; }
}

struct LayerFwdArgs {
    const float *ATT, *H;
    cirs_tracker_layer y;
    const float *win_next, *bin_next;
    float *XH1, *RS1, *H1N, *FF1, *XH2, *RS2, *Hout, *QKVnext;
    const int32_t *row_env, *row_t;
    int R, layer;
};
__device__ __forceinline__ void mm_regs(sg_f32x16& acc, const float (&a)[16], const float (&bv)[16]) {
#pragma unroll
    for (int j = 0; j < 16; ++j) acc = __builtin_amdgcn_mfma_f32_32x32x2f32(a[j], bv[j], acc, 0, 0, 0);
}
__device__ __forceinline__ void ln_apply(const float (&y)[16], const float (&gg)[16], const float (&bb)[16], float (&xh)[16], float (&out)[16], float& rs) {
    float sum = 0.f;
#pragma unroll
    for (int j = 0; j < 16; ++j) sum += y[j];
    sum += __shfl_xor(sum, 32, CIRS_WAVE);
    const float mean = sum * (1.0f / tD);
    float q = 0.f;
#pragma unroll
    for (int j = 0; j < 16; ++j) { const float t = y[j] - mean; q = __builtin_fmaf(t, t, q); }
    q += __shfl_xor(q, 32, CIRS_WAVE);
    rs = 1.0f / sqrtf(q * (1.0f / tD) + 1e-5f);
#pragma unroll
    for (int j = 0; j < 16; ++j) { xh[j] = (y[j] - mean) * rs; out[j] = xh[j] * gg[j] + bb[j]; }
}
template <bool kDrop>
__global__ __launch_bounds__(64) void layer_rows_fwd(LayerFwdArgs a, DropCfg dc) {
    __shared__ __attribute__((aligned(16))) float sT[10 * 1024];
    CIRS_BSTAMP(0);
    const int lane = threadIdx.x, hi = lane >> 5, lo = lane & 31;
    const int row0 = blockIdx.x * 32, row = row0 + lo;
    const bool row_ok = row < a.R;
    const size_t rr = (size_t)(row_ok ? row : 0);
    const int env = kDrop ? a.row_env[rr] : 0, pos = kDrop ? a.row_t[rr] : 0;
    float x[16], hrow[16], wo[16], w1[4][16], g1[16], be1[16];
    ep_load(x, a.ATT + rr * tD + 16 * hi);
    ep_load(wo, a.y.out_proj_w + (size_t)lo * tD + 16 * hi);
    ep_load(hrow, a.H + rr * tD + 16 * hi);
    ep_load(g1, a.y.norm1_w + 16 * hi);
    ep_load(be1, a.y.norm1_b + 16 * hi);
#pragma unroll
    for (int nt = 0; nt < 4; ++nt) ep_load(w1[nt], a.y.lin1_w + (size_t)(nt * 32 + lo) * tD + 16 * hi);
    const float bo = a.y.out_proj_b[lo], bl2 = a.y.lin2_b[lo];
    float bl1[4];
#pragma unroll
    for (int nt = 0; nt < 4; ++nt) bl1[nt] = a.y.lin1_b[nt * 32 + lo];
    if (!row_ok) {
#pragma unroll
        for (int j = 0; j < 16; ++j) x[j] = 0.f;
    }
    sg_f32x16 acc;
#pragma unroll
    for (int s = 0; s < 16; ++s) acc[s] = bo;
    CIRS_BSTAMP(1);
    mm_regs(acc, x, wo);
    CIRS_BSTAMP(2);
    acc_to_lds(sT, acc, lo, hi);
    __syncthreads();
    float w2[4][16];
#pragma unroll
    for (int kb = 0; kb < 4; ++kb) ep_load(w2[kb], a.y.lin2_w + (size_t)lo * tH + kb * 32 + 16 * hi);
    float y[16], xh[16], h1n[16], rs;
    {
        float t[16];
        ep_load(t, sT + lo * kRowT + 16 * hi);
#pragma unroll
        for (int j = 0; j < 16; ++j) {
            float v = t[j];
            if (kDrop) v = drop_apply(dc, v, env, pos, a.layer, CIRS_DROP_RES1, 16 * hi + j);
            y[j] = row_ok ? hrow[j] + v : 0.f;
        }
    }
    CIRS_BSTAMP(3);
    ln_apply(y, g1, be1, xh, h1n, rs);
    CIRS_BSTAMP(4);
    if (row_ok) {
        ep_store(a.XH1 + rr * tD + 16 * hi, xh, 1.0f);
        ep_store(a.H1N + rr * tD + 16 * hi, h1n, 1.0f);
        if (hi == 0) a.RS1[rr] = rs;
    } else {
#pragma unroll
        for (int j = 0; j < 16; ++j) h1n[j] = 0.f;
    }
    __syncthreads();
    CIRS_BSTAMP(5);
#pragma unroll
    for (int nt = 0; nt < 4; ++nt) {
        const int n = nt * 32 + lo;
#pragma unroll
        for (int s = 0; s < 16; ++s) acc[s] = bl1[nt];
        mm_regs(acc, h1n, w1[nt]);
#pragma unroll
        for (int s = 0; s < 16; ++s) acc[s] = fmaxf(acc[s], 0.f);
        acc_to_lds(sT, acc, n, hi);
    }
    __syncthreads();
    CIRS_BSTAMP(6);
    float g2[16], be2[16], wn[3][16], bn[3];
    ep_load(g2, a.y.norm2_w + 16 * hi);
    ep_load(be2, a.y.norm2_b + 16 * hi);
    if (a.win_next) {
#pragma unroll
        for (int nt = 0; nt < 3; ++nt) {
            ep_load(wn[nt], a.win_next + (size_t)(nt * 32 + lo) * tD + 16 * hi);
            bn[nt] = a.bin_next[nt * 32 + lo];
        }
    }
#pragma unroll
    for (int s = 0; s < 16; ++s) acc[s] = bl2;
#pragma unroll
    for (int kb = 0; kb < 4; ++kb) {
        float f[16];
        ep_load(f, sT + lo * kRowT + kb * 32 + 16 * hi);
#pragma unroll
        for (int j = 0; j < 16; ++j) {
            if (kDrop) f[j] = drop_apply(dc, f[j], env, pos, a.layer, CIRS_DROP_FF, kb * 32 + 16 * hi + j);
            if (!row_ok) f[j] = 0.f;
        }
        if (row_ok) ep_store(a.FF1 + rr * tH + kb * 32 + 16 * hi, f, 1.0f);
        mm_regs(acc, f, w2[kb]);
    }
    CIRS_BSTAMP(7);
    __syncthreads();
    acc_to_lds(sT, acc, lo, hi);
    __syncthreads();
    float hn[16];
    {
        float t[16];
        ep_load(t, sT + lo * kRowT + 16 * hi);
#pragma unroll
        for (int j = 0; j < 16; ++j) {
            float v = t[j];
            if (kDrop) v = drop_apply(dc, v, env, pos, a.layer, CIRS_DROP_RES2, 16 * hi + j);
            y[j] = row_ok ? h1n[j] + v : 0.f;
        }
    }
    CIRS_BSTAMP(8);
    ln_apply(y, g2, be2, xh, hn, rs);
    CIRS_BSTAMP(9);
    if (row_ok) {
        ep_store(a.XH2 + rr * tD + 16 * hi, xh, 1.0f);
        ep_store(a.Hout + rr * tD + 16 * hi, hn, 1.0f);
        if (hi == 0) a.RS2[rr] = rs;
    } else {
#pragma unroll
        for (int j = 0; j < 16; ++j) hn[j] = 0.f;
    }
    CIRS_BSTAMP(10);
    if (a.win_next) {
#pragma unroll
        for (int nt = 0; nt < 3; ++nt) {
            const int n = nt * 32 + lo;
#pragma unroll
            for (int s = 0; s < 16; ++s) acc[s] = bn[nt];
            mm_regs(acc, hn, wn[nt]);
#pragma unroll
            for (int s = 0; s < 16; ++s) {
                const int r = row0 + acc_row(s, hi);
                if (r < a.R) a.QKVnext[(size_t)r * 96 + n] = acc[s];
            }
        }
    }
    CIRS_BSTAMP(11);
}

template <bool kDrop>
__global__ __launch_bounds__(64) void embed_inproj(const float* __restrict__ x_hist, const float* __restrict__ pe,
                                                   const int32_t* __restrict__ row_env, const int32_t* __restrict__ row_t, int R, int L,
                                                   const float* __restrict__ win, const float* __restrict__ bin, float* __restrict__ H0,
                                                   float* __restrict__ QKV, DropCfg dc) {
    const int lane = threadIdx.x, hi = lane >> 5, lo = lane & 31;
    const int row0 = blockIdx.x * 32, row = row0 + lo;
    const bool row_ok = row < R;
    const size_t rr = (size_t)(row_ok ? row : 0);
    const int b = row_env[rr], p = row_t[rr];
    float x[16], pp[16], h[16];
    ep_load(x, x_hist + ((size_t)b * L + p) * tD + 16 * hi);
    ep_load(pp, pe + (size_t)p * tD + 16 * hi);
#pragma unroll
    for (int j = 0; j < 16; ++j) {
        float v = x[j] * 5.656854249492381f + pp[j];
        if (kDrop) v = drop_apply(dc, v, b, p, 0, CIRS_DROP_POS, 16 * hi + j);
        h[j] = row_ok ? v : 0.f;
    }
    if (row_ok) ep_store(H0 + rr * tD + 16 * hi, h, 1.0f);
    sg_f32x16 acc;
#pragma unroll
    for (int nt = 0; nt < 3; ++nt) {
        const int n = nt * 32 + lo;
        const float bias = bin[n];
#pragma unroll
        for (int s = 0; s < 16; ++s) acc[s] = bias;
        mm_block(acc, h, win + (size_t)n * tD + 16 * hi);
#pragma unroll
        for (int s = 0; s < 16; ++s) {
            const int r = row0 + acc_row(s, hi);
            if (r < R) QKV[(size_t)r * 96 + n] = acc[s];
        }
    }
}

__device__ __forceinline__ void load_wcols(float (&bv)[16], const float* __restrict__ W, int ldw, int k0, int n) {
#pragma unroll
    for (int j = 0; j < 16; ++j) bv[j] = W[(size_t)(k0 + j) * ldw + n];
}
__device__ __forceinline__ void ln_bwd_half_row(const float (&dout)[16], const float (&xh)[16], const float (&gg)[16], float rs, float (&dy)[16]) {
    float s1 = 0.f, s2 = 0.f, dxh[16];
#pragma unroll
    for (int j = 0; j < 16; ++j) { dxh[j] = dout[j] * gg[j]; s1 += dxh[j]; s2 = __builtin_fmaf(dxh[j], xh[j], s2); }
    s1 += __shfl_xor(s1, 32, CIRS_WAVE);
    s2 += __shfl_xor(s2, 32, CIRS_WAVE);
    const float m1 = s1 * (1.0f / tD), m2 = s2 * (1.0f / tD);
#pragma unroll
    for (int j = 0; j < 16; ++j) dy[j] = rs * (dxh[j] - m1 - xh[j] * m2);
}
struct LayerBwdArgs {
    const float *dHin, *dY1p, *dQKVp, *winp;
    float* dHout;
    int only_pre;
    cirs_tracker_layer y;
    const float *XH2, *RS2, *FF1, *XH1, *RS1;
    float *dB2, *dFF1, *dH1N, *dY1, *dB1, *dATT;
    const int32_t *row_env, *row_t;
    int R, layer;
};
template <int LDW> __device__ __forceinline__ void load_wcols_c(float (&bv)[16], const float* __restrict__ W, int k0, int n) {
#pragma unroll
    for (int j = 0; j < 16; ++j) bv[j] = W[(k0 + j) * LDW + n];
}
template <bool kDrop>
__global__ __launch_bounds__(64) void layer_rows_bwd(LayerBwdArgs a, DropCfg dc) {
    __shared__ __attribute__((aligned(16))) float sT[10 * 1024];
    CIRS_BSTAMP(20);
    const int lane = threadIdx.x, hi = lane >> 5, lo = lane & 31;
    const int row0 = blockIdx.x * 32, row = row0 + lo;
    const bool row_ok = row < a.R;
    const size_t rr = (size_t)(row_ok ? row : 0);
    const int env = kDrop ? a.row_env[rr] : 0, pos = kDrop ? a.row_t[rr] : 0;
    const float dinv = kDrop ? dc.inv : 1.0f;
    sg_f32x16 acc;
    float dh[16];
    if (a.dQKVp) {
        float q[3][16], res[16], bv[3][16];
        ep_load(res, a.dY1p + rr * tD + 16 * hi);
#pragma unroll
        for (int kb = 0; kb < 3; ++kb) {
            ep_load(q[kb], a.dQKVp + rr * 96 + kb * 32 + 16 * hi);
            load_wcols_c<tD>(bv[kb], a.winp, kb * 32 + 16 * hi, lo);
        }
#pragma unroll
        for (int s = 0; s < 16; ++s) acc[s] = 0.f;
#pragma unroll
        for (int kb = 0; kb < 3; ++kb) {
            if (!row_ok) {
#pragma unroll
                for (int j = 0; j < 16; ++j) q[kb][j] = 0.f;
            }
            mm_regs(acc, q[kb], bv[kb]);
        }
        acc_to_lds(sT, acc, lo, hi);
        __syncthreads();
        float t[16];
        ep_load(t, sT + lo * kRowT + 16 * hi);
#pragma unroll
        for (int j = 0; j < 16; ++j) {
            dh[j] = row_ok ? res[j] + t[j] : 0.f;
            if (kDrop && a.only_pre) dh[j] = drop_apply(dc, dh[j], env, pos, 0, CIRS_DROP_POS, 16 * hi + j);
        }
        if (row_ok) ep_store(a.dHout + rr * tD + 16 * hi, dh, 1.0f);
        if (a.only_pre) return;
        __syncthreads();
    } else {
        ep_load(dh, a.dHin + rr * tD + 16 * hi);
        if (!row_ok) {
#pragma unroll
            for (int j = 0; j < 16; ++j) dh[j] = 0.f;
        }
    }
    CIRS_BSTAMP(21);
    float xh2[16], g2[16], xh1[16], g1[16], w2[4][16], ffr[4][16];
    ep_load(xh2, a.XH2 + rr * tD + 16 * hi);
    ep_load(g2, a.y.norm2_w + 16 * hi);
    const float rs2 = a.RS2[rr], rs1 = a.RS1[rr];
#pragma unroll
    for (int nt = 0; nt < 4; ++nt) load_wcols_c<tH>(w2[nt], a.y.lin2_w, 16 * hi, nt * 32 + lo);
#pragma unroll
    for (int kb = 0; kb < 4; ++kb) ep_load(ffr[kb], a.FF1 + rr * tH + kb * 32 + 16 * hi);
    ep_load(xh1, a.XH1 + rr * tD + 16 * hi);
    ep_load(g1, a.y.norm1_w + 16 * hi);
    float dy2[16], db2[16];
    ln_bwd_half_row(dh, xh2, g2, rs2, dy2);
#pragma unroll
    for (int j = 0; j < 16; ++j) {
        if (!row_ok) dy2[j] = 0.f;
        db2[j] = kDrop ? drop_apply(dc, dy2[j], env, pos, a.layer, CIRS_DROP_RES2, 16 * hi + j) : dy2[j];
    }
    if (row_ok) ep_store(a.dB2 + rr * tD + 16 * hi, db2, 1.0f);
    CIRS_BSTAMP(22);
#pragma unroll
    for (int nt = 0; nt < 4; ++nt) {
#pragma unroll
        for (int s = 0; s < 16; ++s) acc[s] = 0.f;
        mm_regs(acc, db2, w2[nt]);
        acc_to_lds(sT, acc, nt * 32 + lo, hi);
    }
    float w1[4][16], wo[16];
#pragma unroll
    for (int kb = 0; kb < 4; ++kb) load_wcols_c<tD>(w1[kb], a.y.lin1_w, kb * 32 + 16 * hi, lo);
    load_wcols_c<tD>(wo, a.y.out_proj_w, 16 * hi, lo);
    __syncthreads();
    CIRS_BSTAMP(23);
    float f[4][16];
#pragma unroll
    for (int kb = 0; kb < 4; ++kb) {
        ep_load(f[kb], sT + lo * kRowT + kb * 32 + 16 * hi);
#pragma unroll
        for (int j = 0; j < 16; ++j) f[kb][j] = (row_ok && ffr[kb][j] > 0.f) ? f[kb][j] * dinv : 0.f;
        if (row_ok) ep_store(a.dFF1 + rr * tH + kb * 32 + 16 * hi, f[kb], 1.0f);
    }
    CIRS_BSTAMP(24);
#pragma unroll
    for (int s = 0; s < 16; ++s) acc[s] = 0.f;
#pragma unroll
// ... 525 lines not shown
    constexpr int HD = tD / NH, EPW = 64 / NH;
    __shared__ uint32_t sK[EPW * NH * 2];
    const int tid = threadIdx.x, el = tid / NH, h = tid - el * NH, e0 = blockIdx.x * EPW, e = e0 + el;
    if (kDrop) last_keep_build<NH>(sK, lens, e0, E, Lp, layer, dc, tid);
    if (e >= E) return;
    const int len = lens[e];
    float acc[HD], hrow[HD];
    if (len <= 0) {
#pragma unroll
        for (int d = 0; d < HD; ++d) acc[d] = 0.f;
        ep_store(ATTc + (size_t)e * tD + h * HD, acc, 1.0f);
        ep_store(Hc + (size_t)e * tD + h * HD, acc, 1.0f);
        stats[((size_t)e * NH + h) * 2] = 0.f; stats[((size_t)e * NH + h) * 2 + 1] = 0.f;
        if (h == 0) { env_c[e] = e; t_c[e] = 0; }
        return;
    }
    const int p = len - 1;
    const size_t base = (size_t)offsets[e];
    const float* rows = QKV + base * 96 + h * HD;
    const float scale = 1.0f / sqrtf((float)HD), qs = scale * 1.4426950408889634f;
    float q[HD];
    ep_load(q, rows + (size_t)p * 96);
    ep_load(hrow, H + (base + p) * tD + h * HD);
#pragma unroll
    for (int d = 0; d < HD; ++d) q[d] *= qs;
    float mx = -INFINITY;
#pragma unroll 4
    for (int j = 0; j <= p; ++j) {
        float k[HD];
        ep_load(k, rows + (size_t)j * 96 + 32);
        mx = fmaxf(mx, ep_dot<HD>(q, k));
    }
    uint32_t km[2] = {0u, 0u};
    if (kDrop) { km[0] = sK[(el * NH + h) * 2]; km[1] = sK[(el * NH + h) * 2 + 1]; }
    float sm = 0.f;
#pragma unroll
    for (int d = 0; d < HD; ++d) acc[d] = 0.f;
#pragma unroll 4
    for (int j = 0; j <= p; ++j) {
        float k[HD], v[HD];
        ep_load(k, rows + (size_t)j * 96 + 32);
        ep_load(v, rows + (size_t)j * 96 + 64);
        float ex = ep_exp2(ep_dot<HD>(q, k) - mx);
        sm += ex;
        if (kDrop) {
            if (!ep_keep_bit(km, j)) ex = 0.f;
        }
#pragma unroll
        for (int d = 0; d < HD; ++d) acc[d] = __builtin_fmaf(ex, v[d], acc[d]);
    }
    const float ia = (kDrop ? dc.inv : 1.0f) / sm;
#pragma unroll
    for (int d = 0; d < HD; ++d) acc[d] *= ia;
    ep_store(ATTc + (size_t)e * tD + h * HD, acc, 1.0f);
    ep_store(Hc + (size_t)e * tD + h * HD, hrow, 1.0f);
    stats[((size_t)e * NH + h) * 2] = mx; stats[((size_t)e * NH + h) * 2 + 1] = 1.0f / sm;
    if (h == 0) { env_c[e] = row_env[base + p]; t_c[e] = row_t[base + p]; }
}
template <int NH, bool kDrop>
__global__ __launch_bounds__(64) void attn_last_bwd(const float* __restrict__ QKV, const float* __restrict__ dATTc, const float* __restrict__ dY1c,
                                                    const float* __restrict__ stats, const int32_t* __restrict__ offsets, const int32_t* __restrict__ lens,
                                                    int E, int Lp, float* __restrict__ dQKV, float* __restrict__ dY1, DropCfg dc, int layer) {
    constexpr int HD = tD / NH, EPW = 64 / NH;
    __shared__ uint32_t sK[EPW * NH * 2];
    const int tid = threadIdx.x, el = tid / NH, h = tid - el * NH, e0 = blockIdx.x * EPW, e = e0 + el;
    if (kDrop) last_keep_build<NH>(sK, lens, e0, E, Lp, layer, dc, tid);
    if (e >= E) return;
    const int len = lens[e];
    if (len <= 0) return;
    const int p = len - 1;
    const size_t base = (size_t)offsets[e];
    const float* rows = QKV + base * 96 + h * HD;
    const float scale = 1.0f / sqrtf((float)HD), qs = scale * 1.4426950408889634f, dinv = kDrop ? dc.inv : 1.0f;
    float qr[HD], q[HD], da[HD], res[HD], zero[HD];
    ep_load(qr, rows + (size_t)p * 96);
    ep_load(da, dATTc + (size_t)e * tD + h * HD);
    ep_load(res, dY1c + (size_t)e * tD + h * HD);
#pragma unroll
    for (int d = 0; d < HD; ++d) { q[d] = qr[d] * qs; zero[d] = 0.f; }
    const float mx = stats[((size_t)e * NH + h) * 2], inv = stats[((size_t)e * NH + h) * 2 + 1];
    uint32_t km[2] = {0u, 0u};
    if (kDrop) { km[0] = sK[(el * NH + h) * 2]; km[1] = sK[(el * NH + h) * 2 + 1]; }
    float dot = 0.f;
#pragma unroll 4
    for (int j = 0; j <= p; ++j) {
        float k[HD], v[HD];
        ep_load(k, rows + (size_t)j * 96 + 32);
        ep_load(v, rows + (size_t)j * 96 + 64);
        const float ex = ep_exp2(ep_dot<HD>(q, k) - mx);
        float dp = ep_dot<HD>(da, v);
        if (kDrop) dp = ep_keep_bit(km, j) ? dp * dinv : 0.f;
        dot = __builtin_fmaf(ex, dp, dot);
    }
    dot *= inv;
    float dq[HD];
#pragma unroll
    for (int d = 0; d < HD; ++d) dq[d] = 0.f;
    float* orow = dQKV + base * 96 + h * HD;
    float* yrow = dY1 + base * tD + h * HD;
#pragma unroll 2
    for (int j = 0; j <= p; ++j) {
        float k[HD], v[HD];
        ep_load(k, rows + (size_t)j * 96 + 32);
        ep_load(v, rows + (size_t)j * 96 + 64);
        const float pj = ep_exp2(ep_dot<HD>(q, k) - mx) * inv;
        float dp = ep_dot<HD>(da, v), pm = pj;
        if (kDrop) {
            const bool keep = ep_keep_bit(km, j);
            dp = keep ? dp * dinv : 0.f;
            pm = keep ? pj * dinv : 0.f;
        }
        const float ds = pj * (dp - dot);
#pragma unroll
        for (int d = 0; d < HD; ++d) dq[d] = __builtin_fmaf(ds, k[d], dq[d]);
        ep_store(orow + (size_t)j * 96 + 32, qr, ds * scale);
        ep_store(orow + (size_t)j * 96 + 64, da, pm);
        if (j < p) {
            ep_store(orow + (size_t)j * 96, zero, 1.0f);
            ep_store(yrow + (size_t)j * tD, zero, 1.0f);
        }
    }
    ep_store(orow + (size_t)p * 96, dq, scale);
    ep_store(yrow + (size_t)p * tD, res, 1.0f);
}
__global__ __launch_bounds__(256) void dstate_last_rows(const float* __restrict__ dstate_last, const int32_t* __restrict__ lens, int E, int S,
                                                        float* __restrict__ G) {
    const long i = blockIdx.x * (long)blockDim.x + threadIdx.x;
    if (i >= (long)E * S) return;
    G[i] = lens[i / S] > 0 ? dstate_last[i] : 0.f;
}
__global__ __launch_bounds__(256) void dstate_last_full(const float* __restrict__ dstate_last, const int32_t* __restrict__ row_env,
                                                        const int32_t* __restrict__ offsets, const int32_t* __restrict__ lens, int R, int S,
                                                        float* __restrict__ G) {
    const long i = blockIdx.x * (long)blockDim.x + threadIdx.x;
    if (i >= (long)R * S) return;
    const int r = (int)(i / S), s = (int)(i % S), b = row_env[r];
    G[i] = r == offsets[b] + lens[b] - 1 ? dstate_last[(size_t)b * S + s] : 0.f;
}
}

extern "C" int64_t cirs_tracker_backward_workspace_bytes(const cirs_tracker_cfg* cfg, int32_t n_rows) {
    if (!cfg || n_rows <= 0) return 0;
    return (int64_t)cirs::bwd_floats(cfg, n_rows) * 4;
}

static inline size_t spread_dyn_lds(long n_blocks, size_t static_bytes, size_t dyn_bytes) {
    if (n_blocks > cirs::device_cu_count()) return dyn_bytes;
    const size_t want = 81 * 1024;
    return static_bytes + dyn_bytes >= want ? dyn_bytes : want - static_bytes;
}
template <typename K> static inline void lds_optin(K k, size_t dyn) {
    if (dyn > 8 * 1024) (void)hipFuncSetAttribute(reinterpret_cast<const void*>(k), hipFuncAttributeMaxDynamicSharedMemorySize, (int)dyn);
}
#define CIRS_LAUNCH_SPREAD(KERNEL, GRID, STATIC_B, DYN_B, STREAM, ...)                                  \
    do {                                                                                               \
        const size_t dyn_ = spread_dyn_lds((long)(GRID), (STATIC_B), (DYN_B));                         \
        if (dyn_ != (size_t)(DYN_B)) lds_optin(KERNEL, dyn_);                                          \
        hipLaunchKernelGGL(KERNEL, dim3(GRID), dim3(64), dyn_, STREAM, __VA_ARGS__);                   \
    } while (0)

static int tracker_rows_impl(const cirs_tracker_cfg* cfg, const cirs_tracker_weights* w, const cirs_tracker_state* st,
                             const int32_t* users, const int64_t* act, const double* rew, const int32_t* row_env,
                             const int32_t* row_t, const int32_t* offsets, const int32_t* lens, int32_t n_rows,
                             const float* dstate, const cirs_tracker_grads* grads, void* workspace,
                             int64_t workspace_bytes, void* stream, float* state_out, int64_t state_stride, const float* dstate_last = nullptr,
                             const cirs::TrunkFuse* ptf = nullptr, int* ptf_fused = nullptr) {
    using namespace cirs;
    CIRS_REQUIRE(cfg && w && st && row_env && row_t && offsets && lens && workspace, "null argument");
    CIRS_REQUIRE(state_out || (users && act && rew && (dstate || dstate_last) && grads), "null argument");
    if (cfg->dim_model != tD || cfg->d_hid != tH) return fail(CIRS_E_UNSUPPORTED, "dim_model == 32 and d_hid == 128 only");
    CIRS_REQUIRE(cfg->nhead == 1 || cfg->nhead == 2 || cfg->nhead == 4 || cfg->nhead == 8, "nhead must be 1,2,4,8");
    CIRS_REQUIRE(n_rows > 0, "n_rows must be positive");
    const int n_carve = dstate_last && cfg->n_env > n_rows ? cfg->n_env : n_rows;
    CIRS_REQUIRE(workspace_bytes >= cirs_tracker_backward_workspace_bytes(cfg, n_carve), "workspace too small");
    hipStream_t s = (hipStream_t)stream;
    const int R = n_rows, B = cfg->n_env, S = cfg->dim_state, L = cfg->max_len, NH = cfg->nhead, nl = cfg->nlayers;
    BwdScratch sc = carve_bwd(workspace, cfg, n_carve);
    auto g1 = [&](long n) { return dim3(cdiv(n, 256)); };

    DwList dwl{};
#define ATT_DISPATCH_SH(KERNEL, SHMEM, ...)                                                               \
    do {                                                                                                  \
        switch (NH) {                                                                                     \
            case 1: hipLaunchKernelGGL(KERNEL<1>, dim3(cdiv(R, 4)), dim3(256), SHMEM, s, __VA_ARGS__); break; \
            case 2: hipLaunchKernelGGL(KERNEL<2>, dim3(cdiv(R, 4)), dim3(256), SHMEM, s, __VA_ARGS__); break; \
            case 4: hipLaunchKernelGGL(KERNEL<4>, dim3(cdiv(R, 4)), dim3(256), SHMEM, s, __VA_ARGS__); break; \
            default: hipLaunchKernelGGL(KERNEL<8>, dim3(cdiv(R, 4)), dim3(256), SHMEM, s, __VA_ARGS__); break; \
        }                                                                                                 \
    } while (0)
#define ATT_DISPATCH(KERNEL, ...) ATT_DISPATCH_SH(KERNEL, 0, __VA_ARGS__)
    auto ep_bytes = [&](bool bwd) -> size_t {
        switch (NH) {
            case 1: return 4 * (bwd ? EpGeo<1>::bwd_floats(L) : EpGeo<1>::fwd_floats(L));
            case 2: return 4 * (bwd ? EpGeo<2>::bwd_floats(L) : EpGeo<2>::fwd_floats(L));
            case 4: return 4 * (bwd ? EpGeo<4>::bwd_floats(L) : EpGeo<4>::fwd_floats(L));
            default: return 4 * (bwd ? EpGeo<8>::bwd_floats(L) : EpGeo<8>::fwd_floats(L));
        }
    };
    const bool ep = L <= 64 && ep_bytes(true) <= 64 * 1024 && !getenv("CIRS_TRACKER_ATTN_ROWS");
#define ATT_EP1(KERNEL, N, BWD, ...)                                                                                            \
    do {                                                                                                                        \
        if (dc.on) CIRS_LAUNCH_SPREAD((KERNEL<N, true>), B, 0, ep_bytes(BWD), s, __VA_ARGS__);       \
        else CIRS_LAUNCH_SPREAD((KERNEL<N, false>), B, 0, ep_bytes(BWD), s, __VA_ARGS__);           \
    } while (0)
#define ATT_EP(KERNEL, BWD, ...)                                  \
    do {                                                          \
        switch (NH) {                                             \
            case 1: ATT_EP1(KERNEL, 1, BWD, __VA_ARGS__); break;  \
            case 2: ATT_EP1(KERNEL, 2, BWD, __VA_ARGS__); break;  \
            case 4: ATT_EP1(KERNEL, 4, BWD, __VA_ARGS__); break;  \
            default: ATT_EP1(KERNEL, 8, BWD, __VA_ARGS__); break; \
        }                                                         \
    } while (0)

    DropCfg dc{};
    if (cfg->dropout_p > 0.f) {
        CIRS_REQUIRE(cfg->dropout_p < 1.f, "dropout_p must be in [0, 1)");
        dc.on = 1; dc.thr = dropout_threshold(cfg->dropout_p); dc.inv = 1.0f / (1.0f - cfg->dropout_p);
        dc.seed = cfg->dropout_seed; dc.env_base = cfg->drop_env_base;
    }
    if (state_out && ep && L <= 32 && S <= 64 && !getenv("CIRS_TRACKER_PREFIX_LAUNCHES")) {
        PrefixEnvArgs pa{};
        pa.x_hist = st->x_hist; pa.pe = w->pe; pa.row_env = row_env; pa.row_t = row_t; pa.offsets = offsets; pa.lens = lens;
        for (int l = 0; l < nl; ++l) pa.layer[l] = w->layer[l];
        pa.dec_w = w->dec_w; pa.dec_b = w->dec_b; pa.state_out = state_out; pa.state_stride = (long)state_stride; pa.nl = nl; pa.L = L; pa.S = S;
        if (ptf && ptf->on) {
            CIRS_REQUIRE(ptf->cfg.hidden == kH && ptf->cfg.dim_state == S && ptf->h2, "prefix states: trunk shape mismatch");
            pa.tf = *ptf;
            if (ptf_fused) *ptf_fused = 1;
        }
#define PREFIX_ENV(N)                                                                                                                        \
    do {                                                                                                                                     \
        const size_t sh = std::max<size_t>(4 * prefix_env_lds_floats<N>(), 40 * 1024);           \
        if (dc.on) hipLaunchKernelGGL((prefix_env_kernel<N, true>), dim3(B), dim3(64), sh, s, pa, dc);                                        \
        else hipLaunchKernelGGL((prefix_env_kernel<N, false>), dim3(B), dim3(64), sh, s, pa, dc);                                             \
    } while (0)
        switch (NH) {
            case 1: PREFIX_ENV(1); break;
            case 2: PREFIX_ENV(2); break;
            case 4: PREFIX_ENV(4); break;
            default: PREFIX_ENV(8); break;
        }
#undef PREFIX_ENV
        CIRS_CHECK_LAUNCH("prefix_env_kernel");
        return CIRS_OK;
    }
    if (dc.on) CIRS_LAUNCH_SPREAD(embed_inproj<true>, cdiv(R, 32), 0, 0, s, st->x_hist, w->pe, row_env, row_t, R, L, w->layer[0].in_proj_w,
                                  w->layer[0].in_proj_b, sc.H[0], sc.QKV[0], dc);
    else CIRS_LAUNCH_SPREAD(embed_inproj<false>, cdiv(R, 32), 0, 0, s, st->x_hist, w->pe, row_env, row_t, R, L, w->layer[0].in_proj_w,
                            w->layer[0].in_proj_b, sc.H[0], sc.QKV[0], dc);
    const bool top_last = dstate_last && ep && nl >= 2 && !getenv("CIRS_TRACKER_LAST_FULL");
    float *dY1c = sc.LC, *att_stats = sc.LC + (size_t)B * tD;
    int32_t *env_c = reinterpret_cast<int32_t*>(att_stats + (size_t)B * 16), *t_c = env_c + B;
#define ATT_LAST1(KERNEL, N, ...)                                                                                        \
    do {                                                                                                                 \
        if (dc.on) hipLaunchKernelGGL((KERNEL<N, true>), dim3(cdiv(B, 64 / N)), dim3(64), 0, s, __VA_ARGS__);             \
        else hipLaunchKernelGGL((KERNEL<N, false>), dim3(cdiv(B, 64 / N)), dim3(64), 0, s, __VA_ARGS__);                  \
    } while (0)
#define ATT_LAST(KERNEL, ...)                                  \
    do {                                                       \
        switch (NH) {                                          \
            case 1: ATT_LAST1(KERNEL, 1, __VA_ARGS__); break;  \
            case 2: ATT_LAST1(KERNEL, 2, __VA_ARGS__); break;  \
            case 4: ATT_LAST1(KERNEL, 4, __VA_ARGS__); break;  \
            default: ATT_LAST1(KERNEL, 8, __VA_ARGS__); break; \
        }                                                      \
    } while (0)
    for (int l = 0; l < nl; ++l) {
        const cirs_tracker_layer& y = w->layer[l];
        if (top_last && l == nl - 1) {
            float* Hc = sc.T1;
            ATT_LAST(attn_last_fwd, (const float*)sc.QKV[l], (const float*)sc.H[l], row_env, row_t, offsets, lens, B, L, sc.ATT[l], Hc, att_stats, env_c, t_c,
                     dc, l);
            LayerFwdArgs fa{sc.ATT[l], Hc, y, nullptr, nullptr, sc.XH1[l], sc.RS1[l], sc.H1N[l], sc.FF1[l], sc.XH2[l], sc.RS2[l], sc.H[l + 1], nullptr,
                            env_c, t_c, B, l};
            if (dc.on) CIRS_LAUNCH_SPREAD(layer_rows_fwd<true>, cdiv(B, 32), 40 * 1024, 0, s, fa, dc);
            else CIRS_LAUNCH_SPREAD(layer_rows_fwd<false>, cdiv(B, 32), 40 * 1024, 0, s, fa, dc);
            continue;
        }
        if (ep) ATT_EP(attn_fwd_ep, false, (const float*)sc.QKV[l], offsets, lens, L, sc.ATT[l], dc, l, (dc.on && !state_out) ? reinterpret_cast<uint32_t*>(sc.P[l]) : (uint32_t*)nullptr);
        else ATT_DISPATCH_SH(attn_fwd, (size_t)4 * NH * L * sizeof(float), sc.QKV[l], row_env, row_t, offsets, R, L, sc.P[l], sc.ATT[l], dc, l, sc.PM[l]);
        if (state_out && l == nl - 1) {
            static_assert(tD == 32, "prefix_last_rows_kernel maps 32 columns to 32 threads");
            float *ATTc = sc.T0, *Hc = sc.T1;
            int32_t *env_c = reinterpret_cast<int32_t*>(sc.T2), *t_c = env_c + B;
            hipLaunchKernelGGL(prefix_last_rows_kernel, dim3(cdiv(B, 8)), dim3(256), 0, s, (const float*)sc.ATT[l], (const float*)sc.H[l], row_env, row_t, offsets,
                               lens, B, ATTc, Hc, env_c, t_c);
            LayerFwdArgs fa{ATTc, Hc, y, nullptr, nullptr, sc.XH1[l], sc.RS1[l], sc.H1N[l], sc.FF1[l], sc.XH2[l], sc.RS2[l], sc.H[l + 1], nullptr,
                            env_c, t_c, B, l};
            if (dc.on) CIRS_LAUNCH_SPREAD(layer_rows_fwd<true>, cdiv(B, 32), 40 * 1024, 0, s, fa, dc);
            else CIRS_LAUNCH_SPREAD(layer_rows_fwd<false>, cdiv(B, 32), 40 * 1024, 0, s, fa, dc);
            continue;
        }
        LayerFwdArgs fa{sc.ATT[l], sc.H[l], y, l + 1 < nl ? w->layer[l + 1].in_proj_w : nullptr, l + 1 < nl ? w->layer[l + 1].in_proj_b : nullptr,
                        sc.XH1[l], sc.RS1[l], sc.H1N[l], sc.FF1[l], sc.XH2[l], sc.RS2[l], sc.H[l + 1], l + 1 < nl ? sc.QKV[l + 1] : nullptr,
                        row_env, row_t, R, l};
        if (dc.on) CIRS_LAUNCH_SPREAD(layer_rows_fwd<true>, cdiv(R, 32), 40 * 1024, 0, s, fa, dc);
        else CIRS_LAUNCH_SPREAD(layer_rows_fwd<false>, cdiv(R, 32), 40 * 1024, 0, s, fa, dc);
    }
    CIRS_CHECK_LAUNCH("tracker forward recompute");
    if (state_out) {
        hipLaunchKernelGGL(prefix_decoder_kernel, dim3(cdiv(B, 4)), dim3(256), 0, s, (const float*)sc.H[nl], lens, B, S, w->dec_w, w->dec_b,
                           state_out, (long)state_stride);
        CIRS_CHECK_LAUNCH("prefix_decoder_kernel");
        return CIRS_OK;
    }
    float* dH = sc.T0;
    if (top_last) {
        hipLaunchKernelGGL(dstate_last_rows, g1((long)B * S), dim3(256), 0, s, dstate_last, lens, B, S, sc.G);
        launch_rows_gemm(false, sc.G, S, w->dec_w, tD, nullptr, B, S, tD, 0, nullptr, 0, dH, tD, s);
    } else {
        if (dstate_last) hipLaunchKernelGGL(dstate_last_full, g1((long)R * S), dim3(256), 0, s, dstate_last, row_env, offsets, lens, R, S, sc.G);
        else hipLaunchKernelGGL(gather_dstate, g1((long)R * S), dim3(256), 0, s, dstate, row_env, row_t, R, S, B, sc.G);
        launch_rows_gemm_dw(dwl, sc.H[nl], tD, S, tD, grads->dec_w, grads->dec_b, sc.partial, false, sc.G, S, w->dec_w, tD, nullptr, R, S, tD, 0, nullptr, 0,
                            dH, tD, s);
    }
    for (int l = nl - 1; l >= 0; --l) {
        const cirs_tracker_layer& y = w->layer[l];
        const cirs_tracker_layer_grads& gy = grads->layer[l];
        if (top_last && l == nl - 1) {
            float* dB1 = dc.on ? sc.T4 : dY1c;
            LayerBwdArgs ba{sc.T0, nullptr, nullptr, nullptr, sc.T0, 0, y, sc.XH2[l], sc.RS2[l], sc.FF1[l], sc.XH1[l], sc.RS1[l], sc.T3, sc.dFF1, sc.T1, dY1c, dB1,
                            sc.T5, env_c, t_c, B, l};
            if (dc.on) CIRS_LAUNCH_SPREAD(layer_rows_bwd<true>, cdiv(B, 32), 40 * 1024, 0, s, ba, dc);
            else CIRS_LAUNCH_SPREAD(layer_rows_bwd<false>, cdiv(B, 32), 40 * 1024, 0, s, ba, dc);
            DwBatch bt{};
            dw_batch_add(bt, dwl, sc.G, S, sc.H[nl], tD, R, S, tD, grads->dec_w, grads->dec_b, 0, sc.partial);
            dw_batch_add(bt, dwl, sc.T0, tD, sc.XH2[l], tD, R, tD, tD, gy.norm2_w, gy.norm2_b, 1, sc.partial);
            dw_batch_add(bt, dwl, sc.T3, tD, sc.FF1[l], tH, R, tD, tH, gy.lin2_w, gy.lin2_b, 0, sc.partial);
            dw_batch_add(bt, dwl, sc.dFF1, tH, sc.H1N[l], tD, R, tH, tD, gy.lin1_w, gy.lin1_b, 0, sc.partial);
            dw_batch_add(bt, dwl, sc.T1, tD, sc.XH1[l], tD, R, tD, tD, gy.norm1_w, gy.norm1_b, 1, sc.partial);
            dw_batch_add(bt, dwl, dB1, tD, sc.ATT[l], tD, R, tD, tD, gy.out_proj_w, gy.out_proj_b, 0, sc.partial);
            dw_batch_launch(bt, R, s, B);
            ATT_LAST(attn_last_bwd, (const float*)sc.QKV[l], (const float*)sc.T5, (const float*)dY1c, (const float*)att_stats, offsets, lens, B, L, sc.dQKV,
                     sc.T2, dc, l);
            continue;
        }
        const bool pre = l + 1 < nl;
        float* dB1 = dc.on ? sc.T4 : sc.T2;
        LayerBwdArgs ba{sc.T0, pre ? sc.T2 : nullptr, pre ? sc.dQKV : nullptr, pre ? w->layer[l + 1].in_proj_w : nullptr, sc.T0, 0, y,
                        sc.XH2[l], sc.RS2[l], sc.FF1[l], sc.XH1[l], sc.RS1[l], sc.T3, sc.dFF1, sc.T1, sc.T2, dB1, sc.T5, row_env, row_t, R, l};
        if (dc.on) CIRS_LAUNCH_SPREAD(layer_rows_bwd<true>, cdiv(R, 32), 40 * 1024, 0, s, ba, dc);
        else CIRS_LAUNCH_SPREAD(layer_rows_bwd<false>, cdiv(R, 32), 40 * 1024, 0, s, ba, dc);
        DwBatch bt{};
        if (pre) dw_batch_add(bt, dwl, sc.dQKV, 96, sc.H[l + 1], tD, R, 96, tD, grads->layer[l + 1].in_proj_w, grads->layer[l + 1].in_proj_b, 0, sc.partial);
        dw_batch_add(bt, dwl, sc.T0, tD, sc.XH2[l], tD, R, tD, tD, gy.norm2_w, gy.norm2_b, 1, sc.partial);
        dw_batch_add(bt, dwl, sc.T3, tD, sc.FF1[l], tH, R, tD, tH, gy.lin2_w, gy.lin2_b, 0, sc.partial);
        dw_batch_add(bt, dwl, sc.dFF1, tH, sc.H1N[l], tD, R, tH, tD, gy.lin1_w, gy.lin1_b, 0, sc.partial);
        dw_batch_add(bt, dwl, sc.T1, tD, sc.XH1[l], tD, R, tD, tD, gy.norm1_w, gy.norm1_b, 1, sc.partial);
        dw_batch_add(bt, dwl, dB1, tD, sc.ATT[l], tD, R, tD, tD, gy.out_proj_w, gy.out_proj_b, 0, sc.partial);
        dw_batch_launch(bt, R, s);
        const float* dATT = sc.T5;
        if (ep) {
            ATT_EP(attn_bwd_ep, true, (const float*)sc.QKV[l], dATT, offsets, lens, L, sc.dQKV, dc, l, dc.on ? reinterpret_cast<const uint32_t*>(sc.P[l]) : (const uint32_t*)nullptr);
        } else {
            ATT_DISPATCH_SH(attn_bwd_q, (size_t)4 * NH * L * sizeof(float), sc.QKV[l], sc.P[l], dATT, row_env, row_t, offsets, R, L, sc.dS, sc.dQKV,
                            (const float*)sc.PM[l], dc.inv);
            ATT_DISPATCH(attn_bwd_kv, sc.QKV[l], dc.on ? sc.PM[l] : sc.P[l], sc.dS, dATT, row_env, row_t, offsets, lens, R, L, sc.dQKV);
        }
    }
    {
        LayerBwdArgs ba{};
        ba.dY1p = sc.T2; ba.dQKVp = sc.dQKV; ba.winp = w->layer[0].in_proj_w; ba.dHout = sc.T0; ba.only_pre = 1;
        ba.row_env = row_env; ba.row_t = row_t; ba.R = R;
        if (dc.on) CIRS_LAUNCH_SPREAD(layer_rows_bwd<true>, cdiv(R, 32), 40 * 1024, 0, s, ba, dc);
        else CIRS_LAUNCH_SPREAD(layer_rows_bwd<false>, cdiv(R, 32), 40 * 1024, 0, s, ba, dc);
    }
    CIRS_CHECK_LAUNCH("tracker backward layers");
    float* DU = sc.T1;
    float* EU = sc.H[nl];
    float* DPRE = sc.H1N[0];
    float* CU = sc.QKV[0];
    float* CI = sc.QKV[0] + (size_t)R * tD;
    int32_t* key_user = (int32_t*)sc.RS1[0];
    int32_t* key_item = (int32_t*)sc.RS2[0];
    const bool merged = B <= R;
    const int slot_rpw = R >= (1 << 17) ? 8 : 1;
    hipLaunchKernelGGL(slot_bwd, dim3(cdiv(R, 4 * slot_rpw)), dim3(256), 0, s, *w, dH, users, act, rew, row_env, row_t, R, B, DU, EU, DPRE,
                       sc.GIN, CU, CI, key_user, key_item, merged ? CI + (size_t)R * tD : nullptr, slot_rpw, 5.656854249492381f);
    if (merged) {
        if (int rc = emb_scatter_merged(key_item, users, lens, CI, R, B, cfg->n_items, cfg->n_users, grads->emb_item, grads->emb_user, sc.sort,
                                        emb_sort_bytes(R + B), s)) return rc;
    } else {
        int32_t* keys_c = (int32_t*)sc.T0;
        float* contrib_c = sc.T2;
        CIRS_HIP(hipMemsetAsync(keys_c, 0xFF, sizeof(int32_t) * (size_t)B, s));
        hipLaunchKernelGGL(compact_user_rows, dim3(cdiv(R, 8)), dim3(256), 0, s, row_env, row_t, users, (const float*)CU, R, keys_c, contrib_c);
        if (int rc = emb_scatter_sorted(keys_c, contrib_c, B, cfg->n_users, grads->emb_user, sc.sort, emb_sort_bytes(R), s)) return rc;
        if (int rc = emb_scatter_sorted(key_item, CI, R, cfg->n_items, grads->emb_item, sc.sort, emb_sort_bytes(R), s)) return rc;
    }
    DwBatch bt{};
    dw_batch_add(bt, dwl, sc.dQKV, 96, sc.H[0], tD, R, 96, tD, grads->layer[0].in_proj_w, grads->layer[0].in_proj_b, 0, sc.partial);
    dw_batch_add(bt, dwl, DU, tD, EU, tD, R, tD, tD, grads->ffn_user_w, grads->ffn_user_b, 0, sc.partial);
    dw_batch_add(bt, dwl, DPRE, tD, sc.GIN, tD + 1, R, tD, tD + 1, grads->gate_w, grads->gate_b, 0, sc.partial);
    dw_batch_launch(bt, R, s);
    launch_dw_list_final(dwl, R, sc.partial, s);
    CIRS_CHECK_LAUNCH("tracker backward slots");
#undef ATT_LAST
#undef ATT_LAST1
#undef ATT_DISPATCH
#undef ATT_EP
#undef ATT_EP1
#undef ATT_DISPATCH_SH
    return CIRS_OK;
}

extern "C" int cirs_tracker_backward(const cirs_tracker_cfg* cfg, const cirs_tracker_weights* w, const cirs_tracker_state* st,
                                     const int32_t* users, const int64_t* act, const double* rew, const int32_t* row_env,
                                     const int32_t* row_t, const int32_t* offsets, const int32_t* lens, int32_t n_rows,
                                     const float* dstate, const cirs_tracker_grads* grads, void* workspace,
                                     int64_t workspace_bytes, void* stream) {
    CIRS_REQUIRE(users && act && rew && dstate && grads, "null argument");
    return tracker_rows_impl(cfg, w, st, users, act, rew, row_env, row_t, offsets, lens, n_rows, dstate, grads, workspace, workspace_bytes, stream,
                             nullptr, 0);
}

extern "C" int cirs_tracker_backward_last(const cirs_tracker_cfg* cfg, const cirs_tracker_weights* w, const cirs_tracker_state* st,
                                          const int32_t* users, const int64_t* act, const double* rew, const int32_t* row_env,
                                          const int32_t* row_t, const int32_t* offsets, const int32_t* lens, int32_t n_rows,
                                          const float* dstate_last, const cirs_tracker_grads* grads, void* workspace,
                                          int64_t workspace_bytes, void* stream) {
    CIRS_REQUIRE(users && act && rew && dstate_last && grads, "null argument");
    return tracker_rows_impl(cfg, w, st, users, act, rew, row_env, row_t, offsets, lens, n_rows, nullptr, grads, workspace, workspace_bytes, stream,
                             nullptr, 0, dstate_last);
}

extern "C" int cirs_tracker_prefix_states(const cirs_tracker_cfg* cfg, const cirs_tracker_weights* w, const cirs_tracker_state* st,
                                          const int32_t* row_env, const int32_t* row_t, const int32_t* offsets, const int32_t* lens,
                                          int32_t n_rows, float* state_out, int64_t state_stride, void* workspace, int64_t workspace_bytes,
                                          void* stream) {
    CIRS_REQUIRE(state_out && state_stride >= (cfg ? cfg->dim_state : 0), "bad state_out");
    return tracker_rows_impl(cfg, w, st, nullptr, nullptr, nullptr, row_env, row_t, offsets, lens, n_rows, nullptr, nullptr, workspace, workspace_bytes,
                             stream, state_out, state_stride);
}

int cirs::tracker_prefix_states_trunk(const cirs_tracker_cfg* cfg, const cirs_tracker_weights* w, const cirs_tracker_state* st, const int32_t* row_env,
                                      const int32_t* row_t, const int32_t* offsets, const int32_t* lens, int32_t n_rows, float* state_out, int64_t state_stride,
                                      void* workspace, int64_t workspace_bytes, void* stream, const TrunkFuse* tf, int* fused) {
    CIRS_REQUIRE(state_out && state_stride >= (cfg ? cfg->dim_state : 0) && fused, "bad state_out");
    *fused = 0;
    return tracker_rows_impl(cfg, w, st, nullptr, nullptr, nullptr, row_env, row_t, offsets, lens, n_rows, nullptr, nullptr, workspace, workspace_bytes,
                             stream, state_out, state_stride, nullptr, tf, fused);
}

extern "C" int64_t cirs_embedding_scatter_workspace_bytes(int64_t n_rows) { return (int64_t)cirs::emb_sort_bytes(n_rows) + 1024; }

extern "C" int cirs_embedding_scatter(const int32_t* keys, const float* contrib, int64_t n_rows, int32_t n_table_rows, float* grad_table,
                                      void* workspace, int64_t workspace_bytes, void* stream) {
    using namespace cirs;
    CIRS_REQUIRE(keys && contrib && grad_table && workspace && n_rows > 0 && n_table_rows > 0, "bad arguments");
    CIRS_REQUIRE(n_rows < (1ll << 31), "too many rows");
    CIRS_REQUIRE(workspace_bytes >= cirs_embedding_scatter_workspace_bytes(n_rows), "workspace too small");
    void* ws = (void*)(((uintptr_t)workspace + 255) & ~(uintptr_t)255);
    return emb_scatter_sorted(keys, contrib, (int)n_rows, n_table_rows, grad_table, ws, (size_t)workspace_bytes - 256, (hipStream_t)stream);
}
```

cirs-codes_amd/csrc/tracker_rows.h:

```cpp
#pragma once
#include <hipcub/hipcub.hpp>
#include "small_gemm.h"
#include "internal.h"

namespace cirs {
typedef float f32x4 __attribute__((ext_vector_type(4)));

constexpr int tD = 32, tH = 128;

constexpr int kMaxDwBatch = 8;
struct DwBatchJob { const float* dY; int ldy; const float* X; int ldx; int O, K, tile_begin; float* partial; };
struct DwBatch { DwBatchJob j[kMaxDwBatch]; int n, total_tiles; };
static __global__ __launch_bounds__(64) void dw_batch_kernel(DwBatch jobs, int R, int rows_per_slab) {
    int ji = 0;
    for (; ji + 1 < jobs.n && (int)blockIdx.x >= jobs.j[ji + 1].tile_begin; ++ji) {}
    const DwBatchJob& jb = jobs.j[ji];
    dw_gemm_body((int)blockIdx.x - jb.tile_begin, blockIdx.y, jb.dY, jb.ldy, jb.X, jb.ldx, R, jb.O, jb.K, rows_per_slab, jb.partial);
}
static inline void dw_batch_add(DwBatch& b, DwList& list, const float* dY, int ldy, const float* X, int ldx, int R, int O, int K, float* dW,
                                float* db, int diag, float* partial) {
    const int slabs = dwg_slabs(R);
    DwListJob& lj = list.j[list.n++];
    lj.O = O; lj.K = K; lj.part_off = list.part_floats; lj.diag = diag; lj.dW = dW; lj.db = db;
    DwBatchJob& jb = b.j[b.n++];
    jb.dY = dY; jb.ldy = ldy; jb.X = X; jb.ldx = ldx; jb.O = O; jb.K = K; jb.tile_begin = b.total_tiles; jb.partial = partial + lj.part_off;
    b.total_tiles += cdiv(O, 32) * cdiv(K, 32);
    list.part_floats += slabs * O * (K + 1);
    list.total_out += O * (K + 1);
}
static inline void dw_batch_launch(const DwBatch& b, int R, hipStream_t s, int R_rows = -1) {
    if (!b.n) return;
    if (R_rows < 0) R_rows = R;
    const int slabs = dwg_slabs(R);
    int rows_per_slab = (R_rows + slabs - 1) / slabs;
    rows_per_slab = (rows_per_slab + 15) & ~15;
    hipLaunchKernelGGL(dw_batch_kernel, dim3(b.total_tiles, slabs), dim3(64), 0, s, b, R_rows, rows_per_slab);
}

static __global__ __launch_bounds__(256) void gather_dstate(const float* __restrict__ dstate, const int32_t* __restrict__ row_env,
                                                     const int32_t* __restrict__ row_t, int R, int S, int B, float* __restrict__ G) {
    const long i = blockIdx.x * (long)blockDim.x + threadIdx.x;
    if (i >= (long)R * S) return;
    const int r = (int)(i / S), s = (int)(i % S);
    G[i] = dstate[((size_t)row_t[r] * B + row_env[r]) * S + s];
}

__device__ __forceinline__ float lane_bcast(float x, int k) {
    return __builtin_bit_cast(float, __builtin_amdgcn_readlane(__builtin_bit_cast(int, x), k));
}

static __global__ __launch_bounds__(256) void slot_bwd(cirs_tracker_weights w, const float* __restrict__ dH0, const int32_t* __restrict__ users,
                                                const int64_t* __restrict__ act, const double* __restrict__ rew,
                                                const int32_t* __restrict__ row_env, const int32_t* __restrict__ row_t, int R, int B,
                                                float* __restrict__ DU, float* __restrict__ EU, float* __restrict__ DPRE,
                                                float* __restrict__ GIN, float* __restrict__ CU, float* __restrict__ CI,
                                                int32_t* __restrict__ key_user, int32_t* __restrict__ key_item,
                                                float* __restrict__ contrib_c ,
                                                int rows_per_wave, float in_scale ) {
    const int lane = threadIdx.x & 63;
    __shared__ float sG[tD * (tD + 1)];
    for (int q = threadIdx.x; q < tD * (tD + 1); q += 256) sG[q] = w.gate_w[q];
    __syncthreads();
    for (int it_r = 0; it_r < rows_per_wave; ++it_r) {
    const int r = (blockIdx.x * rows_per_wave + it_r) * 4 + (threadIdx.x >> 6);
    if (r >= R) return;
    const int b = row_env[r], p = row_t[r];
    const int d = lane & 31;
    const float dx = dH0[(size_t)r * tD + d] * in_scale;
    if (p == 0) {
        const int u = users[b];
        const float eu = w.emb_user[(size_t)u * tD + d];
        if (lane < tD) {
            DU[(size_t)r * tD + d] = dx; EU[(size_t)r * tD + d] = eu;
            DPRE[(size_t)r * tD + d] = 0.f;
        }
        if (lane <= tD) GIN[(size_t)r * (tD + 1) + lane] = 0.f;
        float acc = 0.f;
#pragma unroll
        for (int o = 0; o < tD; ++o) acc = __builtin_fmaf(lane_bcast(dx, o), w.ffn_user_w[(size_t)o * tD + d], acc);
        if (lane < tD) {
            CU[(size_t)r * tD + d] = acc; CI[(size_t)r * tD + d] = 0.f;
            if (contrib_c) contrib_c[(size_t)b * tD + d] = acc;
        }
        if (lane == 0) { key_user[r] = u; key_item[r] = -1; }
    } else {
        const size_t ti = (size_t)(p - 1) * B + b;
        const long it = act[ti];
        const float rw = (float)rew[ti];
        const float a = w.emb_item[(size_t)it * tD + d];
        const float* gw = sG + d * (tD + 1);
        float pre = w.gate_b[d];
        pre = __builtin_fmaf(gw[0], rw, pre);
#pragma unroll
        for (int k = 0; k < tD; ++k) pre = __builtin_fmaf(gw[1 + k], lane_bcast(a, k), pre);
        const float g = 1.0f / (1.0f + expf(-pre));
        const float dpre = dx * a * g * (1.0f - g);
        if (lane < tD) {
            DPRE[(size_t)r * tD + d] = dpre;
            DU[(size_t)r * tD + d] = 0.f; EU[(size_t)r * tD + d] = 0.f;
            GIN[(size_t)r * (tD + 1) + 1 + d] = a;
        }
        if (lane == 0) GIN[(size_t)r * (tD + 1)] = rw;
        float acc = dx * g;
#pragma unroll
        for (int o = 0; o < tD; ++o) acc = __builtin_fmaf(lane_bcast(dpre, o), sG[o * (tD + 1) + 1 + d], acc);
        if (lane < tD) { CI[(size_t)r * tD + d] = acc; CU[(size_t)r * tD + d] = 0.f; }
        if (lane == 0) { key_item[r] = (int32_t)it; key_user[r] = -1; }
    }
    }
}

static __global__ __launch_bounds__(256) void scatter_keys_kernel(const int32_t* __restrict__ keys, int R, int n_table,
                                                           uint32_t* __restrict__ keys_u, int32_t* __restrict__ rows) {
    const int r = blockIdx.x * blockDim.x + threadIdx.x;
    if (r >= R) return;
    const int32_t k = keys[r];
    keys_u[r] = (k < 0 || k >= n_table) ? (uint32_t)n_table : (uint32_t)k;
    rows[r] = r;
}

static __global__ __launch_bounds__(256) void compact_user_rows(const int32_t* __restrict__ row_env, const int32_t* __restrict__ row_t,
                                                         const int32_t* __restrict__ users, const float* __restrict__ CU, int R,
                                                         int32_t* __restrict__ keys_c, float* __restrict__ contrib_c) {
    const int d = threadIdx.x & 31;
    const int r = blockIdx.x * 8 + (threadIdx.x >> 5);
    if (r >= R || row_t[r] != 0) return;
    const int b = row_env[r];
    contrib_c[(size_t)b * tD + d] = CU[(size_t)r * tD + d];
    if (d == 0) keys_c[b] = users[b];
}

constexpr int kSubRun = 64;
static __global__ __launch_bounds__(256) void emb_subrun_kernel(const uint32_t* __restrict__ ks, const int32_t* __restrict__ rs,
                                                         const float* __restrict__ contrib, int R, int n_table, float* __restrict__ part) {
    const int d = threadIdx.x & 31, half = (threadIdx.x >> 5) & 1;
    const int p = blockIdx.x * 8 + (threadIdx.x >> 5);
    const bool in = p < R;
    const uint32_t key = in ? ks[p] : 0xffffffffu;
    const bool start = in && key < (uint32_t)n_table && ((p % kSubRun) == 0 || ks[p - 1] != key);
    const int end = min(R, (p / kSubRun + 1) * kSubRun);
    const int q0 = p + d, q1 = p + 32 + d;
    const bool s0 = start && q0 < end && ks[q0] == key, s1 = start && q1 < end && ks[q1] == key;
    const int r0 = s0 ? rs[q0] : 0, r1 = s1 ? rs[q1] : 0;
    const unsigned long long m0 = __ballot(s0), m1 = __ballot(s1);
    if (!start) return;
    const uint32_t h0 = (uint32_t)(m0 >> (32 * half)), h1 = (uint32_t)(m1 >> (32 * half));
    const int n = h0 == 0xffffffffu ? 32 + (h1 == 0xffffffffu ? 32 : __builtin_ctz(~h1)) : __builtin_ctz(~h0);
    float acc = 0.f;
    for (int q = 0; q < n; q += 16) {
        float t[16];
#pragma unroll
        for (int u = 0; u < 16; ++u) {
            const int qq = q + u;
            const int row = __shfl(qq < 32 ? r0 : r1, (qq & 31) + 32 * half, CIRS_WAVE);
            t[u] = qq < n ? contrib[(size_t)row * tD + d] : 0.f;
        }
#pragma unroll
        for (int u = 0; u < 16; ++u) acc += (q + u < n) ? t[u] : 0.f;
    }
    part[(size_t)p * tD + d] = acc;
}

static __global__ __launch_bounds__(256) void emb_segment_sum_kernel(const uint32_t* __restrict__ ks, const float* __restrict__ part, int R,
                                                              int n_table, float* __restrict__ g_emb, int n_first = 0x7fffffff,
                                                              float* __restrict__ g_second = nullptr) {
    const int d = threadIdx.x & 31;
    const int p = blockIdx.x * 8 + (threadIdx.x >> 5);
    if (p >= R) return;
    const uint32_t key = ks[p];
    if (key >= (uint32_t)n_table || (p > 0 && ks[p - 1] == key)) return;
    float acc = part[(size_t)p * tD + d];
    for (int q = (p / kSubRun + 1) * kSubRun; q < R; q += 8 * kSubRun) {
        float t8[8];
        int n_ok = 0;
#pragma unroll
        for (int u = 0; u < 8; ++u) {
            const int qq = q + u * kSubRun;
            const bool ok = (n_ok == u) && qq < R && ks[qq] == key;
            t8[u] = ok ? part[(size_t)qq * tD + d] : 0.f;
            n_ok += ok;
        }
#pragma unroll
        for (int u = 0; u < 8; ++u) acc += (u < n_ok) ? t8[u] : 0.f;
        if (n_ok < 8) break;
    }
    if (key < (uint32_t)n_first) g_emb[(size_t)key * tD + d] = acc;
    else g_second[(size_t)(key - (uint32_t)n_first) * tD + d] = acc;
}

static size_t emb_sort_bytes(long R) { return (size_t)R * (64 + 4 * tD) + (1u << 20); }

static int emb_scatter_sorted(const int32_t* keys, const float* contrib, int R, int n_table, float* g_emb, void* scratch,
                              size_t scratch_bytes, hipStream_t s) {
    static_assert(tD == 32, "emb_segment_sum_kernel maps one lane per embedding dimension");
    uint32_t* k_in = (uint32_t*)scratch;
    uint32_t* k_out = k_in + R;
    int32_t* r_in = (int32_t*)(k_out + R);
    int32_t* r_out = r_in + R;
    float* part = (float*)(((uintptr_t)(r_out + R) + 255) & ~(uintptr_t)255);
    char* temp = (char*)(((uintptr_t)(part + (size_t)R * tD) + 255) & ~(uintptr_t)255);
    const size_t avail = scratch_bytes - (size_t)(temp - (char*)scratch);
    int end_bit = 1;
    while ((1u << end_bit) <= (uint32_t)n_table && end_bit < 32) ++end_bit;
    size_t need = 0;
    CIRS_HIP(hipcub::DeviceRadixSort::SortPairs(nullptr, need, k_in, k_out, r_in, r_out, R, 0, end_bit, s));
    CIRS_REQUIRE(need <= avail, "embedding scatter: sort scratch too small");
    CIRS_HIP(hipMemsetAsync(g_emb, 0, (size_t)n_table * tD * sizeof(float), s));
    hipLaunchKernelGGL(scatter_keys_kernel, dim3(cdiv(R, 256)), dim3(256), 0, s, keys, R, n_table, k_in, r_in);
    CIRS_HIP(hipcub::DeviceRadixSort::SortPairs(temp, need, k_in, k_out, r_in, r_out, R, 0, end_bit, s));
    hipLaunchKernelGGL(emb_subrun_kernel, dim3(cdiv(R, 8)), dim3(256), 0, s, k_out, r_out, contrib, R, n_table, part);
    hipLaunchKernelGGL(emb_segment_sum_kernel, dim3(cdiv(R, 8)), dim3(256), 0, s, k_out, (const float*)part, R, n_table, g_emb);
    CIRS_CHECK_LAUNCH("emb_segment_sum_kernel");
    return CIRS_OK;
}

static __global__ __launch_bounds__(256) void scatter_keys2_kernel(const int32_t* __restrict__ key_item, const int32_t* __restrict__ users,
                                                            const int32_t* __restrict__ lens, int R, int B, int n_items, int n_users,
                                                            uint32_t* __restrict__ keys_u, int32_t* __restrict__ rows,
                                                            float* __restrict__ zero_table , long zero_floats) {
    const int p = blockIdx.x * blockDim.x + threadIdx.x;
    if (zero_table)
        for (long i = (long)p * 4; i < zero_floats; i += (long)gridDim.x * blockDim.x * 4) *reinterpret_cast<f32x4*>(zero_table + i) = f32x4{0.f, 0.f, 0.f, 0.f};
    if (p >= R + B) return;
    const uint32_t sent = (uint32_t)n_items + (uint32_t)n_users;
    uint32_t k = sent;
    if (p < R) {
        const int32_t v = key_item[p];
        if (v >= 0 && v < n_items) k = (uint32_t)v;
    } else {
        const int b = p - R;
        const int32_t u = users[b];
        if (lens[b] > 0 && u >= 0 && u < n_users) k = (uint32_t)n_items + (uint32_t)u;
    }
    keys_u[p] = k;
    rows[p] = p;
}
static int emb_scatter_merged(const int32_t* key_item, const int32_t* users, const int32_t* lens, const float* contrib, int R, int B,
                              int n_items, int n_users, float* g_item, float* g_user, void* scratch, size_t scratch_bytes, hipStream_t s) {
    const int N = R + B, n_table = n_items + n_users;
    uint32_t* k_in = (uint32_t*)scratch;
    uint32_t* k_out = k_in + N;
    int32_t* r_in = (int32_t*)(k_out + N);
    int32_t* r_out = r_in + N;
    float* part = (float*)(((uintptr_t)(r_out + N) + 255) & ~(uintptr_t)255);
    char* temp = (char*)(((uintptr_t)(part + (size_t)N * tD) + 255) & ~(uintptr_t)255);
    const size_t avail = scratch_bytes - (size_t)(temp - (char*)scratch);
    int end_bit = 1;
    while ((1u << end_bit) <= (uint32_t)n_table && end_bit < 32) ++end_bit;
    size_t need = 0;
    CIRS_HIP(hipcub::DeviceRadixSort::SortPairs(nullptr, need, k_in, k_out, r_in, r_out, N, 0, end_bit, s));
    CIRS_REQUIRE(need <= avail, "embedding scatter: sort scratch too small");
    float* zero_table = nullptr;
    if (g_user + (size_t)n_users * tD == g_item) zero_table = g_user;
    else if (g_item + (size_t)n_items * tD == g_user) zero_table = g_item;
    if (zero_table && ((uintptr_t)zero_table & 15)) zero_table = nullptr;
    if (!zero_table) {
        CIRS_HIP(hipMemsetAsync(g_item, 0, (size_t)n_items * tD * sizeof(float), s));
        CIRS_HIP(hipMemsetAsync(g_user, 0, (size_t)n_users * tD * sizeof(float), s));
    }
    hipLaunchKernelGGL(scatter_keys2_kernel, dim3(cdiv(N, 256)), dim3(256), 0, s, key_item, users, lens, R, B, n_items, n_users, k_in, r_in, zero_table,
                       (long)n_table * tD);
    CIRS_HIP(hipcub::DeviceRadixSort::SortPairs(temp, need, k_in, k_out, r_in, r_out, N, 0, end_bit, s));
    hipLaunchKernelGGL(emb_subrun_kernel, dim3(cdiv(N, 8)), dim3(256), 0, s, k_out, r_out, contrib, N, n_table, part);
    hipLaunchKernelGGL(emb_segment_sum_kernel, dim3(cdiv(N, 8)), dim3(256), 0, s, k_out, (const float*)part, N, n_table, g_item, n_items, g_user);
    CIRS_CHECK_LAUNCH("emb_segment_sum_kernel (merged)");
    return CIRS_OK;
}

}
```

Measured before the change: 5.960 million.

## Piggyback embedding radix-sort stages, dstate gather and dobs clear onto existing kernels

Replaces the library radix sort used for embedding-gradient ordering with a custom multi-pass LSD sort. Its stages run as extra blocks appended to the tracker forward kernels (embed_inproj, attention, layer_rows_fwd). The dstate gather kernel and the dobs_accum memset are likewise folded in as extra blocks of the embed and trunk_adv launches. The goal is to remove standalone launches and serial stream gaps. In exchange the kernels grow in complexity, and correctness depends on the sort stages being ordered across launches.

```diff
diff --git a/cirs-codes_amd/csrc/ppo.hip b/cirs-codes_amd/csrc/ppo.hip
--- a/cirs-codes_amd/csrc/ppo.hip
+++ b/cirs-codes_amd/csrc/ppo.hip
@@ -526,9 +526,16 @@
                                                         long stride, int n_pad, const int32_t* __restrict__ idx, int mb,
                                                         const float* __restrict__ adv_flat, const int32_t* __restrict__ sidx,
                                                         int m_stats, int enable, float* __restrict__ red, int n_row_wgs,
-                                                        uint4* __restrict__ planes, cirs_ppo_batch bt, int n_env, TrunkRowOut out) {
+                                                        uint4* __restrict__ planes, cirs_ppo_batch bt, int n_env, TrunkRowOut out,
+                                                        float* __restrict__ clear , long clear_floats, int clear_first) {
     __shared__ float lds_raw[kTileN * 65];
     static_assert(kTileN * 65 >= 4 * 2 * kH, "the trunk rows use 4 x 2 x 64 floats of the same buffer");
+    if ((int)blockIdx.x >= clear_first) {
+        const long n4 = clear_floats >> 2, step = (long)(gridDim.x - clear_first) * 256;
+        for (long i = (long)((int)blockIdx.x - clear_first) * 256 + threadIdx.x; i < n4; i += step) reinterpret_cast<f32x4*>(clear)[i] = f32x4{0.f, 0.f, 0.f, 0.f};
+        if ((int)blockIdx.x == clear_first && threadIdx.x < (clear_floats & 3)) clear[(n4 << 2) + threadIdx.x] = 0.f;
+        return;
+    }
     if ((int)blockIdx.x > n_row_wgs) {
         wa_planes_block((int)blockIdx.x - n_row_wgs - 1, cfg.n_items, w.wa, planes, lds_raw);
         return;
@@ -2585,7 +2592,10 @@
     bool learn_prefetch;
     int drop_arrival;
 };
-struct PpoStep { const int32_t* idx; int mb; const int32_t* sidx; int mb_norm; float* dobs; float* loss_out; long opt_step; };
+struct PpoStep {
+    const int32_t* idx; int mb; const int32_t* sidx; int mb_norm; float* dobs; float* loss_out; long opt_step;
+    float* clear; long clear_floats;
+};
 
 static int env_int(const char* name, int unset) {
     const char* e = getenv(name);
@@ -2616,9 +2626,11 @@
 static int launch_trunk_adv(const PpoRun& r, const PpoStep& st, const cirs::TrunkRowOut& out) {
     using namespace cirs;
     const int n_pad = n_pad_of(st.mb);
-    hipLaunchKernelGGL(trunk_adv_kernel, dim3(cdiv(n_pad, 4) + 1 + cdiv(r.I, kTileN)), dim3(256), 0, r.s, r.pcfg, r.w, (const float*)r.batch->obs, (long)r.S,
+    const int grid = cdiv(n_pad, 4) + 1 + cdiv(r.I, kTileN);
+    const int n_clear = st.clear ? (int)std::min<long>(256, cdiv(st.clear_floats, 256 * 4 * 4)) : 0;
+    hipLaunchKernelGGL(trunk_adv_kernel, dim3(grid + n_clear), dim3(256), 0, r.s, r.pcfg, r.w, (const float*)r.batch->obs, (long)r.S,
                        n_pad, st.idx, st.mb, (const float*)r.batch->adv, st.sidx, st.mb_norm, (int)r.cfg->norm_adv, r.v.red, (int)cdiv(n_pad, 4),
-                       r.v.wa_planes, *r.batch, r.n_env, out);
+                       r.v.wa_planes, *r.batch, r.n_env, out, st.clear, st.clear_floats, n_clear ? grid : 0x7fffffff);
     CIRS_CHECK_LAUNCH("trunk_adv_kernel");
     return CIRS_OK;
 }
@@ -2874,9 +2886,11 @@
         return PpoStep{idx, e - b, idx, e - b, (dobs_accum && rep == n_repeat - 1) ? dobs_accum : nullptr, losses + 4 * (size_t)k, (long)(opt_step + k)};
     };
     bool have_head = false;
+    const bool clear_seated = dobs_accum && ((uintptr_t)dobs_accum & 15) == 0;
     for (int k = 0; k < n_steps; ++k) {
-        const PpoStep st = step_of(k);
-        if (dobs_accum && k == (n_repeat - 1) * n_sl) {
+        PpoStep st = step_of(k);
+        if (clear_seated && k == 0) { st.clear = dobs_accum; st.clear_floats = (long)dobs_floats; }
+        if (dobs_accum && !clear_seated && k == (n_repeat - 1) * n_sl) {
             if (hipMemsetAsync(dobs_accum, 0, sizeof(float) * (size_t)dobs_floats, r.s) != hipSuccess) return fail(CIRS_E_LAUNCH, "hipMemsetAsync(dobs_accum)");
         }
         const bool has_next = prefetch && k + 1 < n_steps;
diff --git a/cirs-codes_amd/csrc/tracker_bwd.hip b/cirs-codes_amd/csrc/tracker_bwd.hip
--- a/cirs-codes_amd/csrc/tracker_bwd.hip
+++ b/cirs-codes_amd/csrc/tracker_bwd.hip
@@ -324,10 +324,15 @@
 template <int NH, bool kDrop>
 __global__ __launch_bounds__(64) void attn_fwd_ep(const float* __restrict__ QKV, const int32_t* __restrict__ offsets,
                                                   const int32_t* __restrict__ lens, int Lp, float* __restrict__ ATT, DropCfg dc, int layer,
-                                                  uint32_t* __restrict__ keep_out ) {
+                                                  uint32_t* __restrict__ keep_out ,
+                                                  EmbOrder seat) {
     using G = EpGeo<NH>;
     constexpr int HPL = G::HPL, DPL = G::DPL, HD = G::HD, SL = G::SL;
     extern __shared__ __attribute__((aligned(16))) float smem[];
+    if ((int)blockIdx.x >= seat.first_block) {
+        emb_order_stage(seat, (int)blockIdx.x - seat.first_block, reinterpret_cast<uint32_t*>(smem));
+        return;
+    }
     const int b = blockIdx.x, len = lens[b];
     if (len <= 0) return;
     const int lane = threadIdx.x, hg = lane / SL, slot = lane - hg * SL;
@@ -692,8 +697,12 @@
     for (int j = 0; j < 16; ++j) { xh[j] = (y[j] - mean) * rs; out[j] = xh[j] * gg[j] + bb[j]; }
 }
 template <bool kDrop>
-__global__ __launch_bounds__(64) void layer_rows_fwd(LayerFwdArgs a, DropCfg dc) {
+__global__ __launch_bounds__(64) void layer_rows_fwd(LayerFwdArgs a, DropCfg dc, EmbOrder seat) {
     __shared__ __attribute__((aligned(16))) float sT[10 * 1024];
+    if ((int)blockIdx.x >= seat.first_block) {
+        emb_order_stage(seat, (int)blockIdx.x - seat.first_block, reinterpret_cast<uint32_t*>(sT));
+        return;
+    }
     CIRS_BSTAMP(0);
     const int lane = threadIdx.x, hi = lane >> 5, lo = lane & 31;
     const int row0 = blockIdx.x * 32, row = row0 + lo;
@@ -835,7 +844,16 @@
 __global__ __launch_bounds__(64) void embed_inproj(const float* __restrict__ x_hist, const float* __restrict__ pe,
                                                    const int32_t* __restrict__ row_env, const int32_t* __restrict__ row_t, int R, int L,
                                                    const float* __restrict__ win, const float* __restrict__ bin, float* __restrict__ H0,
-                                                   float* __restrict__ QKV, DropCfg dc) {
+                                                   float* __restrict__ QKV, DropCfg dc, EmbOrder seat, GatherSeat gs) {
+    if ((int)blockIdx.x >= gs.first_block) {
+        gather_dstate_seat(gs, (int)blockIdx.x - gs.first_block);
+        return;
+    }
+    if ((int)blockIdx.x >= seat.first_block) {
+        __shared__ uint32_t sH[256];
+        emb_order_stage(seat, (int)blockIdx.x - seat.first_block, sH);
+        return;
+    }
     const int lane = threadIdx.x, hi = lane >> 5, lo = lane & 31;
     const int row0 = blockIdx.x * 32, row = row0 + lo;
     const bool row_ok = row < R;
@@ -1667,12 +1685,13 @@
 template <typename K> static inline void lds_optin(K k, size_t dyn) {
     if (dyn > 8 * 1024) (void)hipFuncSetAttribute(reinterpret_cast<const void*>(k), hipFuncAttributeMaxDynamicSharedMemorySize, (int)dyn);
 }
-#define CIRS_LAUNCH_SPREAD(KERNEL, GRID, STATIC_B, DYN_B, STREAM, ...)                                  \
+#define CIRS_LAUNCH_SPREAD_X(KERNEL, GRID, XTRA, STATIC_B, DYN_B, STREAM, ...)                          \
     do {                                                                                               \
         const size_t dyn_ = spread_dyn_lds((long)(GRID), (STATIC_B), (DYN_B));                         \
         if (dyn_ != (size_t)(DYN_B)) lds_optin(KERNEL, dyn_);                                          \
-        hipLaunchKernelGGL(KERNEL, dim3(GRID), dim3(64), dyn_, STREAM, __VA_ARGS__);                   \
+        hipLaunchKernelGGL(KERNEL, dim3((GRID) + (XTRA)), dim3(64), dyn_, STREAM, __VA_ARGS__);        \
     } while (0)
+#define CIRS_LAUNCH_SPREAD(KERNEL, GRID, STATIC_B, DYN_B, STREAM, ...) CIRS_LAUNCH_SPREAD_X(KERNEL, GRID, 0, STATIC_B, DYN_B, STREAM, __VA_ARGS__)
 
 static int tracker_rows_impl(const cirs_tracker_cfg* cfg, const cirs_tracker_weights* w, const cirs_tracker_state* st,
                              const int32_t* users, const int64_t* act, const double* rew, const int32_t* row_env,
@@ -1713,19 +1732,19 @@
         }
     };
     const bool ep = L <= 64 && ep_bytes(true) <= 64 * 1024 && !getenv("CIRS_TRACKER_ATTN_ROWS");
-#define ATT_EP1(KERNEL, N, BWD, ...)                                                                                            \
+#define ATT_EP1(KERNEL, N, BWD, XTRA, ...)                                                                                      \
     do {                                                                                                                        \
-        if (dc.on) CIRS_LAUNCH_SPREAD((KERNEL<N, true>), B, 0, ep_bytes(BWD), s, __VA_ARGS__);       \
-        else CIRS_LAUNCH_SPREAD((KERNEL<N, false>), B, 0, ep_bytes(BWD), s, __VA_ARGS__);           \
+        if (dc.on) CIRS_LAUNCH_SPREAD_X((KERNEL<N, true>), B, XTRA, 0, ep_bytes(BWD), s, __VA_ARGS__);       \
+        else CIRS_LAUNCH_SPREAD_X((KERNEL<N, false>), B, XTRA, 0, ep_bytes(BWD), s, __VA_ARGS__);           \
     } while (0)
-#define ATT_EP(KERNEL, BWD, ...)                                  \
-    do {                                                          \
-        switch (NH) {                                             \
-            case 1: ATT_EP1(KERNEL, 1, BWD, __VA_ARGS__); break;  \
-            case 2: ATT_EP1(KERNEL, 2, BWD, __VA_ARGS__); break;  \
-            case 4: ATT_EP1(KERNEL, 4, BWD, __VA_ARGS__); break;  \
-            default: ATT_EP1(KERNEL, 8, BWD, __VA_ARGS__); break; \
-        }                                                         \
+#define ATT_EP(KERNEL, BWD, XTRA, ...)                                  \
+    do {                                                                \
+        switch (NH) {                                                   \
+            case 1: ATT_EP1(KERNEL, 1, BWD, XTRA, __VA_ARGS__); break;  \
+            case 2: ATT_EP1(KERNEL, 2, BWD, XTRA, __VA_ARGS__); break;  \
+            case 4: ATT_EP1(KERNEL, 4, BWD, XTRA, __VA_ARGS__); break;  \
+            default: ATT_EP1(KERNEL, 8, BWD, XTRA, __VA_ARGS__); break; \
+        }                                                               \
     } while (0)
 
     DropCfg dc{};
@@ -1760,10 +1779,22 @@
         CIRS_CHECK_LAUNCH("prefix_env_kernel");
         return CIRS_OK;
     }
-    if (dc.on) CIRS_LAUNCH_SPREAD(embed_inproj<true>, cdiv(R, 32), 0, 0, s, st->x_hist, w->pe, row_env, row_t, R, L, w->layer[0].in_proj_w,
-                                  w->layer[0].in_proj_b, sc.H[0], sc.QKV[0], dc);
-    else CIRS_LAUNCH_SPREAD(embed_inproj<false>, cdiv(R, 32), 0, 0, s, st->x_hist, w->pe, row_env, row_t, R, L, w->layer[0].in_proj_w,
-                            w->layer[0].in_proj_b, sc.H[0], sc.QKV[0], dc);
+    const bool merged = !state_out && B <= R;
+    EmbOrderPlan ord{};
+    ord.o = emb_order_none();
+    if (merged) {
+        const char* how = getenv("CIRS_TRACKER_EMB_ORDER");
+        const bool lib_sort = how && !strcmp(how, "library"), launches = how && !strcmp(how, "launches");
+        if (int rc = emb_order_plan(ord, nullptr, act, row_env, row_t, users, lens, R, B, cfg->n_items, cfg->n_users, grads->emb_item, grads->emb_user, sc.sort,
+                                    emb_sort_bytes(R + B), s, lib_sort ? 1 : launches ? 0 : -1)) return rc;
+        if (launches) { if (int rc = emb_order_finish(ord, s)) return rc; }
+    }
+    EmbOrder seat = emb_order_seat(ord, cdiv(R, 32));
+    const GatherSeat gs = (!state_out && !dstate_last) ? gather_seat(dstate, row_env, row_t, R, S, B, sc.G, cdiv(R, 32) + seat.n_blocks) : gather_seat_none();
+    if (dc.on) CIRS_LAUNCH_SPREAD_X(embed_inproj<true>, cdiv(R, 32), seat.n_blocks + gs.n_blocks, 1024, 0, s, st->x_hist, w->pe, row_env, row_t, R, L,
+                                    w->layer[0].in_proj_w, w->layer[0].in_proj_b, sc.H[0], sc.QKV[0], dc, seat, gs);
+    else CIRS_LAUNCH_SPREAD_X(embed_inproj<false>, cdiv(R, 32), seat.n_blocks + gs.n_blocks, 1024, 0, s, st->x_hist, w->pe, row_env, row_t, R, L,
+                              w->layer[0].in_proj_w, w->layer[0].in_proj_b, sc.H[0], sc.QKV[0], dc, seat, gs);
     const bool top_last = dstate_last && ep && nl >= 2 && !getenv("CIRS_TRACKER_LAST_FULL");
     float *dY1c = sc.LC, *att_stats = sc.LC + (size_t)B * tD;
     int32_t *env_c = reinterpret_cast<int32_t*>(att_stats + (size_t)B * 16), *t_c = env_c + B;
@@ -1789,11 +1820,16 @@
                      dc, l);
             LayerFwdArgs fa{sc.ATT[l], Hc, y, nullptr, nullptr, sc.XH1[l], sc.RS1[l], sc.H1N[l], sc.FF1[l], sc.XH2[l], sc.RS2[l], sc.H[l + 1], nullptr,
                             env_c, t_c, B, l};
-            if (dc.on) CIRS_LAUNCH_SPREAD(layer_rows_fwd<true>, cdiv(B, 32), 40 * 1024, 0, s, fa, dc);
-            else CIRS_LAUNCH_SPREAD(layer_rows_fwd<false>, cdiv(B, 32), 40 * 1024, 0, s, fa, dc);
+            seat = emb_order_seat(ord, cdiv(B, 32));
+            if (dc.on) CIRS_LAUNCH_SPREAD_X(layer_rows_fwd<true>, cdiv(B, 32), seat.n_blocks, 40 * 1024, 0, s, fa, dc, seat);
+            else CIRS_LAUNCH_SPREAD_X(layer_rows_fwd<false>, cdiv(B, 32), seat.n_blocks, 40 * 1024, 0, s, fa, dc, seat);
             continue;
         }
-        if (ep) ATT_EP(attn_fwd_ep, false, (const float*)sc.QKV[l], offsets, lens, L, sc.ATT[l], dc, l, (dc.on && !state_out) ? reinterpret_cast<uint32_t*>(sc.P[l]) : (uint32_t*)nullptr);
+        if (ep) {
+            seat = ep_bytes(false) >= 1024 ? emb_order_seat(ord, B) : emb_order_none();
+            ATT_EP(attn_fwd_ep, false, seat.n_blocks, (const float*)sc.QKV[l], offsets, lens, L, sc.ATT[l], dc, l,
+                   (dc.on && !state_out) ? reinterpret_cast<uint32_t*>(sc.P[l]) : (uint32_t*)nullptr, seat);
+        }
         else ATT_DISPATCH_SH(attn_fwd, (size_t)4 * NH * L * sizeof(float), sc.QKV[l], row_env, row_t, offsets, R, L, sc.P[l], sc.ATT[l], dc, l, sc.PM[l]);
         if (state_out && l == nl - 1) {
             static_assert(tD == 32, "prefix_last_rows_kernel maps 32 columns to 32 threads");
@@ -1803,16 +1839,18 @@
                                lens, B, ATTc, Hc, env_c, t_c);
             LayerFwdArgs fa{ATTc, Hc, y, nullptr, nullptr, sc.XH1[l], sc.RS1[l], sc.H1N[l], sc.FF1[l], sc.XH2[l], sc.RS2[l], sc.H[l + 1], nullptr,
                             env_c, t_c, B, l};
-            if (dc.on) CIRS_LAUNCH_SPREAD(layer_rows_fwd<true>, cdiv(B, 32), 40 * 1024, 0, s, fa, dc);
-            else CIRS_LAUNCH_SPREAD(layer_rows_fwd<false>, cdiv(B, 32), 40 * 1024, 0, s, fa, dc);
+            if (dc.on) CIRS_LAUNCH_SPREAD(layer_rows_fwd<true>, cdiv(B, 32), 40 * 1024, 0, s, fa, dc, emb_order_none());
+            else CIRS_LAUNCH_SPREAD(layer_rows_fwd<false>, cdiv(B, 32), 40 * 1024, 0, s, fa, dc, emb_order_none());
             continue;
         }
         LayerFwdArgs fa{sc.ATT[l], sc.H[l], y, l + 1 < nl ? w->layer[l + 1].in_proj_w : nullptr, l + 1 < nl ? w->layer[l + 1].in_proj_b : nullptr,
                         sc.XH1[l], sc.RS1[l], sc.H1N[l], sc.FF1[l], sc.XH2[l], sc.RS2[l], sc.H[l + 1], l + 1 < nl ? sc.QKV[l + 1] : nullptr,
                         row_env, row_t, R, l};
-        if (dc.on) CIRS_LAUNCH_SPREAD(layer_rows_fwd<true>, cdiv(R, 32), 40 * 1024, 0, s, fa, dc);
-        else CIRS_LAUNCH_SPREAD(layer_rows_fwd<false>, cdiv(R, 32), 40 * 1024, 0, s, fa, dc);
-    }
+        seat = emb_order_seat(ord, cdiv(R, 32));
+        if (dc.on) CIRS_LAUNCH_SPREAD_X(layer_rows_fwd<true>, cdiv(R, 32), seat.n_blocks, 40 * 1024, 0, s, fa, dc, seat);
+        else CIRS_LAUNCH_SPREAD_X(layer_rows_fwd<false>, cdiv(R, 32), seat.n_blocks, 40 * 1024, 0, s, fa, dc, seat);
+    }
+    if (merged) { if (int rc = emb_order_finish(ord, s)) return rc; }
     CIRS_CHECK_LAUNCH("tracker forward recompute");
     if (state_out) {
         hipLaunchKernelGGL(prefix_decoder_kernel, dim3(cdiv(B, 4)), dim3(256), 0, s, (const float*)sc.H[nl], lens, B, S, w->dec_w, w->dec_b,
@@ -1826,7 +1864,6 @@
         launch_rows_gemm(false, sc.G, S, w->dec_w, tD, nullptr, B, S, tD, 0, nullptr, 0, dH, tD, s);
     } else {
         if (dstate_last) hipLaunchKernelGGL(dstate_last_full, g1((long)R * S), dim3(256), 0, s, dstate_last, row_env, offsets, lens, R, S, sc.G);
-        else hipLaunchKernelGGL(gather_dstate, g1((long)R * S), dim3(256), 0, s, dstate, row_env, row_t, R, S, B, sc.G);
         launch_rows_gemm_dw(dwl, sc.H[nl], tD, S, tD, grads->dec_w, grads->dec_b, sc.partial, false, sc.G, S, w->dec_w, tD, nullptr, R, S, tD, 0, nullptr, 0,
                             dH, tD, s);
     }
@@ -1867,7 +1904,7 @@
         dw_batch_launch(bt, R, s);
         const float* dATT = sc.T5;
         if (ep) {
-            ATT_EP(attn_bwd_ep, true, (const float*)sc.QKV[l], dATT, offsets, lens, L, sc.dQKV, dc, l, dc.on ? reinterpret_cast<const uint32_t*>(sc.P[l]) : (const uint32_t*)nullptr);
+            ATT_EP(attn_bwd_ep, true, 0, (const float*)sc.QKV[l], dATT, offsets, lens, L, sc.dQKV, dc, l, dc.on ? reinterpret_cast<const uint32_t*>(sc.P[l]) : (const uint32_t*)nullptr);
         } else {
             ATT_DISPATCH_SH(attn_bwd_q, (size_t)4 * NH * L * sizeof(float), sc.QKV[l], sc.P[l], dATT, row_env, row_t, offsets, R, L, sc.dS, sc.dQKV,
                             (const float*)sc.PM[l], dc.inv);
@@ -1889,13 +1926,11 @@
     float* CI = sc.QKV[0] + (size_t)R * tD;
     int32_t* key_user = (int32_t*)sc.RS1[0];
     int32_t* key_item = (int32_t*)sc.RS2[0];
-    const bool merged = B <= R;
     const int slot_rpw = R >= (1 << 17) ? 8 : 1;
     hipLaunchKernelGGL(slot_bwd, dim3(cdiv(R, 4 * slot_rpw)), dim3(256), 0, s, *w, dH, users, act, rew, row_env, row_t, R, B, DU, EU, DPRE,
                        sc.GIN, CU, CI, key_user, key_item, merged ? CI + (size_t)R * tD : nullptr, slot_rpw, 5.656854249492381f);
     if (merged) {
-        if (int rc = emb_scatter_merged(key_item, users, lens, CI, R, B, cfg->n_items, cfg->n_users, grads->emb_item, grads->emb_user, sc.sort,
-                                        emb_sort_bytes(R + B), s)) return rc;
+        if (int rc = emb_scatter_sums(ord, CI, grads->emb_item, grads->emb_user, s)) return rc;
     } else {
         int32_t* keys_c = (int32_t*)sc.T0;
         float* contrib_c = sc.T2;
@@ -1958,6 +1993,25 @@
                              stream, state_out, state_stride, nullptr, tf, fused);
 }
 
+extern "C" int cirs_debug_emb_order(const int32_t* key_item, const int32_t* users, const int32_t* lens, int32_t n_rows, int32_t n_env, int32_t n_items,
+                                    int32_t n_users, uint32_t* keys_out, int32_t* rows_out, void* workspace, int64_t workspace_bytes, int32_t how,
+                                    void* stream) {
+    using namespace cirs;
+    CIRS_REQUIRE(key_item && users && lens && keys_out && rows_out && workspace && n_rows >= 0 && n_env >= 0 && n_rows + (int64_t)n_env > 0, "bad arguments");
+    CIRS_REQUIRE(workspace_bytes >= cirs_embedding_scatter_workspace_bytes((int64_t)n_rows + n_env), "workspace too small");
+    hipStream_t s = (hipStream_t)stream;
+    void* ws = (void*)(((uintptr_t)workspace + 255) & ~(uintptr_t)255);
+    EmbOrderPlan pl;
+    if (int rc = emb_order_plan(pl, key_item, nullptr, nullptr, nullptr, users, lens, n_rows, n_env, n_items, n_users, nullptr, nullptr, ws,
+                                (size_t)workspace_bytes - 256, s, how == 1)) return rc;
+    if (int rc = emb_order_finish(pl, s)) return rc;
+    const size_t n = (size_t)n_rows + n_env;
+    CIRS_HIP(hipMemcpyAsync(keys_out, pl.o.k[pl.result], n * sizeof(uint32_t), hipMemcpyDeviceToDevice, s));
+    CIRS_HIP(hipMemcpyAsync(rows_out, pl.o.r[pl.result], n * sizeof(int32_t), hipMemcpyDeviceToDevice, s));
+    CIRS_CHECK_LAUNCH("cirs_debug_emb_order");
+    return CIRS_OK;
+}
+
 extern "C" int64_t cirs_embedding_scatter_workspace_bytes(int64_t n_rows) { return (int64_t)cirs::emb_sort_bytes(n_rows) + 1024; }
 
 extern "C" int cirs_embedding_scatter(const int32_t* keys, const float* contrib, int64_t n_rows, int32_t n_table_rows, float* grad_table,
diff --git a/cirs-codes_amd/csrc/tracker_rows.h b/cirs-codes_amd/csrc/tracker_rows.h
--- a/cirs-codes_amd/csrc/tracker_rows.h
+++ b/cirs-codes_amd/csrc/tracker_rows.h
@@ -43,6 +43,36 @@
     if (i >= (long)R * S) return;
     const int r = (int)(i / S), s = (int)(i % S);
     G[i] = dstate[((size_t)row_t[r] * B + row_env[r]) * S + s];
+}
+
+struct GatherSeat { const float* dstate; const int32_t *row_env, *row_t; float* G; int R, S, B, vec4, first_block, n_blocks; };
+static inline GatherSeat gather_seat_none() { GatherSeat g{}; g.first_block = 0x7fffffff; return g; }
+static inline GatherSeat gather_seat(const float* dstate, const int32_t* row_env, const int32_t* row_t, int R, int S, int B, float* G, int first_block) {
+    GatherSeat g{dstate, row_env, row_t, G, R, S, B, 0, first_block, 0};
+    g.vec4 = (S % 4 == 0) && (((uintptr_t)dstate | (uintptr_t)G) & 15) == 0;
+    const long units = (long)R * (g.vec4 ? S / 4 : S);
+    g.n_blocks = (int)std::min<long>(512, cdiv(units, 64 * 4));
+    return g;
+}
+__device__ __forceinline__ void gather_dstate_seat(const GatherSeat& g, int blk) {
+    const int lane = threadIdx.x & 63;
+    const long step = (long)g.n_blocks * 64;
+    if (g.vec4) {
+        const int S4 = g.S >> 2;
+        const f32x4* __restrict__ src = reinterpret_cast<const f32x4*>(g.dstate);
+        f32x4* __restrict__ dst = reinterpret_cast<f32x4*>(g.G);
+#pragma unroll 4
+        for (long i = (long)blk * 64 + lane; i < (long)g.R * S4; i += step) {
+            const int r = (int)(i / S4), c = (int)(i % S4);
+            dst[i] = src[((size_t)g.row_t[r] * g.B + g.row_env[r]) * S4 + c];
+        }
+        return;
+    }
+#pragma unroll 4
+    for (long i = (long)blk * 64 + lane; i < (long)g.R * g.S; i += step) {
+        const int r = (int)(i / g.S), c = (int)(i % g.S);
+        g.G[i] = g.dstate[((size_t)g.row_t[r] * g.B + g.row_env[r]) * g.S + c];
+    }
 }
 
 __device__ __forceinline__ float lane_bcast(float x, int k) {
@@ -214,57 +244,227 @@
     return CIRS_OK;
 }
 
-static __global__ __launch_bounds__(256) void scatter_keys2_kernel(const int32_t* __restrict__ key_item, const int32_t* __restrict__ users,
-                                                            const int32_t* __restrict__ lens, int R, int B, int n_items, int n_users,
-                                                            uint32_t* __restrict__ keys_u, int32_t* __restrict__ rows,
-                                                            float* __restrict__ zero_table , long zero_floats) {
-    const int p = blockIdx.x * blockDim.x + threadIdx.x;
-    if (zero_table)
-        for (long i = (long)p * 4; i < zero_floats; i += (long)gridDim.x * blockDim.x * 4) *reinterpret_cast<f32x4*>(zero_table + i) = f32x4{0.f, 0.f, 0.f, 0.f};
-    if (p >= R + B) return;
-    const uint32_t sent = (uint32_t)n_items + (uint32_t)n_users;
-    uint32_t k = sent;
-    if (p < R) {
-        const int32_t v = key_item[p];
-        if (v >= 0 && v < n_items) k = (uint32_t)v;
+constexpr int kOrdChunk = 512, kOrdRounds = kOrdChunk / 64, kOrdMaxBlocks = 128;
+constexpr int kOrdLibraryPairs = 1 << 17;
+struct EmbOrder {
+    const int32_t *key_item;
+    const int64_t* act;
+    const int32_t *row_env, *row_t, *users, *lens;
+    uint32_t* k[2];
+    int32_t* r[2];
+    uint32_t* hist;
+    float* zero_table;
+    long zero_floats;
+    int R, B, n_items, n_users, N, chunk, nblk, npass;
+    int stage, first_block, n_blocks;
+};
+static inline EmbOrder emb_order_none() { EmbOrder o{}; o.stage = -1; o.first_block = 0x7fffffff; return o; }
+
+__device__ __forceinline__ uint32_t emb_order_key(const EmbOrder& o, int p) {
+    uint32_t k = (uint32_t)o.n_items + (uint32_t)o.n_users;
+    if (p < o.R) {
+        int32_t v = -1;
+        if (o.key_item) v = o.key_item[p];
+        else {
+            const int t = o.row_t[p];
+            if (t > 0) v = (int32_t)o.act[(size_t)(t - 1) * o.B + o.row_env[p]];
+        }
+        if (v >= 0 && v < o.n_items) k = (uint32_t)v;
     } else {
-        const int b = p - R;
-        const int32_t u = users[b];
-        if (lens[b] > 0 && u >= 0 && u < n_users) k = (uint32_t)n_items + (uint32_t)u;
-    }
-    keys_u[p] = k;
-    rows[p] = p;
+        const int b = p - o.R;
+        const int32_t u = o.users[b];
+        if (o.lens[b] > 0 && u >= 0 && u < o.n_users) k = (uint32_t)o.n_items + (uint32_t)u;
+    }
+    return k;
+}
+
+__device__ __forceinline__ void emb_order_stage(const EmbOrder& o, int blk, uint32_t* __restrict__ sH) {
+    const int lane = threadIdx.x & 63;
+    const int ps = o.stage >> 1, shift = 8 * ps;
+    const int i_begin = blk * o.chunk, i_end = min(o.N, i_begin + o.chunk);
+    if (o.stage == 0 && o.zero_table)
+        for (long i = ((long)blk * 64 + lane) * 4; i < o.zero_floats; i += (long)o.n_blocks * 64 * 4)
+            *reinterpret_cast<f32x4*>(o.zero_table + i) = f32x4{0.f, 0.f, 0.f, 0.f};
+    if (blk >= o.nblk) return;
+    const uint32_t* __restrict__ ks = o.k[ps & 1];
+    uint32_t* __restrict__ hist = o.hist + (size_t)ps * o.nblk * 256;
+    if (!(o.stage & 1)) {
+        for (int q = lane; q < 256; q += 64) sH[q] = 0u;
+        __syncthreads();
+        for (int i0 = i_begin; i0 < i_end; i0 += kOrdChunk)
+#pragma unroll
+        for (int u = 0; u < kOrdRounds; ++u) {
+            const int i = i0 + u * 64 + lane;
+            if (i < i_end) {
+                uint32_t key;
+                if (ps == 0) { key = emb_order_key(o, i); o.k[0][i] = key; o.r[0][i] = i; }
+                else key = ks[i];
+                atomicAdd(&sH[(key >> shift) & 255u], 1u);
+            }
+        }
+        __syncthreads();
+        for (int q = lane; q < 256; q += 64) hist[(size_t)blk * 256 + q] = sH[q];
+        return;
+    }
+    const int32_t* __restrict__ rs = o.r[ps & 1];
+    uint32_t key[kOrdRounds];
+    int32_t row[kOrdRounds];
+#pragma unroll
+    for (int u = 0; u < kOrdRounds; ++u) {
+        const int i = i_begin + u * 64 + lane;
+        key[u] = i < i_end ? ks[i] : 0u;
+        row[u] = ps == 0 ? i : (i < i_end ? rs[i] : 0);
+    }
+    uint32_t before[4] = {0u, 0u, 0u, 0u}, total[4] = {0u, 0u, 0u, 0u};
+#pragma unroll 4
+    for (int j = 0; j < o.nblk; ++j) {
+        const uint4 v = *reinterpret_cast<const uint4*>(hist + (size_t)j * 256 + 4 * lane);
+        total[0] += v.x; total[1] += v.y; total[2] += v.z; total[3] += v.w;
+        if (j < blk) { before[0] += v.x; before[1] += v.y; before[2] += v.z; before[3] += v.w; }
+    }
+    const uint32_t mine = total[0] + total[1] + total[2] + total[3];
+    uint32_t inc = mine;
+#pragma unroll
+    for (int d = 1; d < 64; d <<= 1) {
+        const uint32_t t = (uint32_t)__shfl_up((int)inc, d, CIRS_WAVE);
+        if (lane >= d) inc += t;
+    }
+    uint32_t ex = inc - mine;
+#pragma unroll
+    for (int q = 0; q < 4; ++q) { sH[4 * lane + q] = ex + before[q]; ex += total[q]; }
+    __syncthreads();
+    uint32_t* __restrict__ kd = o.k[(ps & 1) ^ 1];
+    int32_t* __restrict__ rd = o.r[(ps & 1) ^ 1];
+    for (int i0 = i_begin; i0 < i_end; i0 += kOrdChunk) {
+    if (i0 > i_begin) {
+#pragma unroll
+        for (int u = 0; u < kOrdRounds; ++u) {
+            const int i = i0 + u * 64 + lane;
+            key[u] = i < i_end ? ks[i] : 0u;
+            row[u] = ps == 0 ? i : (i < i_end ? rs[i] : 0);
+        }
+    }
+#pragma unroll
+    for (int u = 0; u < kOrdRounds; ++u) {
+        const bool ok = i0 + u * 64 + lane < i_end;
+        const uint32_t d = (key[u] >> shift) & 255u;
+        unsigned long long m = __ballot(ok);
+#pragma unroll
+        for (int bit = 0; bit < 8; ++bit) {
+            const bool on = (d >> bit) & 1u;
+            const unsigned long long bl = __ballot(on);
+            m &= on ? bl : ~bl;
+        }
+        const int rank = __popcll(m & ((1ull << lane) - 1ull)), cnt = __popcll(m);
+        const uint32_t base = sH[d];
+        __syncthreads();
+        if (ok && rank == cnt - 1) sH[d] = base + (uint32_t)cnt;
+        __syncthreads();
+        const uint32_t pos = base + (uint32_t)rank;
+        if (ok && pos < (uint32_t)o.N) { kd[pos] = key[u]; rd[pos] = row[u]; }
+    }
+    }
+}
+static __global__ __launch_bounds__(64) void emb_order_stage_kernel(EmbOrder o) {
+    __shared__ uint32_t sH[256];
+    emb_order_stage(o, (int)blockIdx.x, sH);
+}
+
+struct EmbOrderPlan {
+    EmbOrder o;
+    int next;
+    int result;
+    int library;
+    float* part;
+    char* temp; size_t temp_bytes;
+};
+static int emb_order_plan(EmbOrderPlan& pl, const int32_t* key_item, const int64_t* act, const int32_t* row_env, const int32_t* row_t,
+                          const int32_t* users, const int32_t* lens, int R, int B, int n_items, int n_users, float* g_item, float* g_user,
+                          void* scratch, size_t scratch_bytes, hipStream_t s, int how = -1 ) {
+    const int N = R + B, n_table = n_items + n_users;
+    pl.library = how < 0 ? N > kOrdLibraryPairs : how;
+    EmbOrder& o = pl.o;
+    o = emb_order_none();
+    o.key_item = key_item; o.act = act; o.row_env = row_env; o.row_t = row_t; o.users = users; o.lens = lens;
+    o.R = R; o.B = B; o.n_items = n_items; o.n_users = n_users; o.N = N;
+    o.chunk = pl.library ? kOrdChunk : kOrdChunk * std::max(1, cdiv(cdiv(N, kOrdMaxBlocks), kOrdChunk));
+    o.nblk = cdiv(N, o.chunk);
+    o.k[0] = (uint32_t*)scratch;
+    o.k[1] = o.k[0] + N;
+    o.r[0] = (int32_t*)(o.k[1] + N);
+    o.r[1] = o.r[0] + N;
+    pl.part = (float*)(((uintptr_t)(o.r[1] + N) + 255) & ~(uintptr_t)255);
+    o.hist = (uint32_t*)(((uintptr_t)(pl.part + (size_t)N * tD) + 255) & ~(uintptr_t)255);
+    int end_bit = 1;
+    while ((1u << end_bit) <= (uint32_t)n_table && end_bit < 32) ++end_bit;
+    o.npass = (end_bit + 7) / 8;
+    pl.temp = (char*)(o.hist + (size_t)o.npass * o.nblk * 256);
+    CIRS_REQUIRE((size_t)(pl.temp - (char*)scratch) <= scratch_bytes, "embedding scatter: sort scratch too small");
+    pl.temp_bytes = scratch_bytes - (size_t)(pl.temp - (char*)scratch);
+    pl.result = o.npass & 1;
+    if (!g_item || !g_user) {}
+    else if (g_user + (size_t)n_users * tD == g_item) o.zero_table = g_user;
+    else if (g_item + (size_t)n_items * tD == g_user) o.zero_table = g_item;
+    if (o.zero_table && ((uintptr_t)o.zero_table & 15)) o.zero_table = nullptr;
+    o.zero_floats = (long)n_table * tD;
+    if (!g_item || !g_user) o.zero_table = nullptr;
+    else if (!o.zero_table) {
+        CIRS_HIP(hipMemsetAsync(g_item, 0, (size_t)n_items * tD * sizeof(float), s));
+        CIRS_HIP(hipMemsetAsync(g_user, 0, (size_t)n_users * tD * sizeof(float), s));
+    }
+    pl.next = 0;
+    return CIRS_OK;
+}
+static inline EmbOrder emb_order_seat(EmbOrderPlan& pl, int first_block, bool for_library = false) {
+    if (pl.next >= 2 * pl.o.npass || (pl.library && !for_library)) return emb_order_none();
+    EmbOrder o = pl.o;
+    o.stage = pl.next++;
+    o.first_block = first_block;
+    o.n_blocks = o.nblk;
+    if (o.stage == 0 && o.zero_table) o.n_blocks = std::max(o.nblk, (int)std::min<long>(256, cdiv(o.zero_floats, 64 * 4 * 8)));
+    return o;
+}
+static int emb_order_library(EmbOrderPlan& pl, hipStream_t s);
+static inline int emb_order_finish(EmbOrderPlan& pl, hipStream_t s) {
+    if (pl.library) return pl.next == 0 ? emb_order_library(pl, s) : CIRS_OK;
+    for (;;) {
+        const EmbOrder o = emb_order_seat(pl, 0);
+        if (o.stage < 0) return CIRS_OK;
+        hipLaunchKernelGGL(emb_order_stage_kernel, dim3(o.n_blocks), dim3(64), 0, s, o);
+    }
+}
+static int emb_order_library(EmbOrderPlan& pl, hipStream_t s) {
+    CIRS_REQUIRE(pl.next == 0 && pl.library, "embedding ordering: already started");
+    const EmbOrder o0 = emb_order_seat(pl, 0, true);
+    hipLaunchKernelGGL(emb_order_stage_kernel, dim3(o0.n_blocks), dim3(64), 0, s, o0);
+    const EmbOrder& o = pl.o;
+    int end_bit = 1;
+    while ((1u << end_bit) <= (uint32_t)(o.n_items + o.n_users) && end_bit < 32) ++end_bit;
+    size_t need = 0;
+    CIRS_HIP(hipcub::DeviceRadixSort::SortPairs(nullptr, need, o.k[0], o.k[1], o.r[0], o.r[1], o.N, 0, end_bit, s));
+    CIRS_REQUIRE(need <= pl.temp_bytes, "embedding scatter: sort scratch too small");
+    CIRS_HIP(hipcub::DeviceRadixSort::SortPairs(pl.temp, need, o.k[0], o.k[1], o.r[0], o.r[1], o.N, 0, end_bit, s));
+    pl.next = 2 * o.npass;
+    pl.result = 1;
+    return CIRS_OK;
+}
+static int emb_scatter_sums(const EmbOrderPlan& pl, const float* contrib, float* g_item, float* g_user, hipStream_t s) {
+    static_assert(tD == 32, "emb_segment_sum_kernel maps one lane per embedding dimension");
+    const EmbOrder& o = pl.o;
+    const uint32_t* ks = o.k[pl.result];
+    const int32_t* rs = o.r[pl.result];
+    const int n_table = o.n_items + o.n_users;
+    hipLaunchKernelGGL(emb_subrun_kernel, dim3(cdiv(o.N, 8)), dim3(256), 0, s, ks, rs, contrib, o.N, n_table, pl.part);
+    hipLaunchKernelGGL(emb_segment_sum_kernel, dim3(cdiv(o.N, 8)), dim3(256), 0, s, ks, (const float*)pl.part, o.N, n_table, g_item, o.n_items, g_user);
+    CIRS_CHECK_LAUNCH("emb_segment_sum_kernel (merged)");
+    return CIRS_OK;
 }
 static int emb_scatter_merged(const int32_t* key_item, const int32_t* users, const int32_t* lens, const float* contrib, int R, int B,
                               int n_items, int n_users, float* g_item, float* g_user, void* scratch, size_t scratch_bytes, hipStream_t s) {
-    const int N = R + B, n_table = n_items + n_users;
-    uint32_t* k_in = (uint32_t*)scratch;
-    uint32_t* k_out = k_in + N;
-    int32_t* r_in = (int32_t*)(k_out + N);
-    int32_t* r_out = r_in + N;
-    float* part = (float*)(((uintptr_t)(r_out + N) + 255) & ~(uintptr_t)255);
-    char* temp = (char*)(((uintptr_t)(part + (size_t)N * tD) + 255) & ~(uintptr_t)255);
-    const size_t avail = scratch_bytes - (size_t)(temp - (char*)scratch);
-    int end_bit = 1;
-    while ((1u << end_bit) <= (uint32_t)n_table && end_bit < 32) ++end_bit;
-    size_t need = 0;
-    CIRS_HIP(hipcub::DeviceRadixSort::SortPairs(nullptr, need, k_in, k_out, r_in, r_out, N, 0, end_bit, s));
-    CIRS_REQUIRE(need <= avail, "embedding scatter: sort scratch too small");
-    float* zero_table = nullptr;
-    if (g_user + (size_t)n_users * tD == g_item) zero_table = g_user;
-    else if (g_item + (size_t)n_items * tD == g_user) zero_table = g_item;
-    if (zero_table && ((uintptr_t)zero_table & 15)) zero_table = nullptr;
-    if (!zero_table) {
-        CIRS_HIP(hipMemsetAsync(g_item, 0, (size_t)n_items * tD * sizeof(float), s));
-        CIRS_HIP(hipMemsetAsync(g_user, 0, (size_t)n_users * tD * sizeof(float), s));
-    }
-    hipLaunchKernelGGL(scatter_keys2_kernel, dim3(cdiv(N, 256)), dim3(256), 0, s, key_item, users, lens, R, B, n_items, n_users, k_in, r_in, zero_table,
-                       (long)n_table * tD);
-    CIRS_HIP(hipcub::DeviceRadixSort::SortPairs(temp, need, k_in, k_out, r_in, r_out, N, 0, end_bit, s));
-    hipLaunchKernelGGL(emb_subrun_kernel, dim3(cdiv(N, 8)), dim3(256), 0, s, k_out, r_out, contrib, N, n_table, part);
-    hipLaunchKernelGGL(emb_segment_sum_kernel, dim3(cdiv(N, 8)), dim3(256), 0, s, k_out, (const float*)part, N, n_table, g_item, n_items, g_user);
-    CIRS_CHECK_LAUNCH("emb_segment_sum_kernel (merged)");
-    return CIRS_OK;
-}
-
-}
+    EmbOrderPlan pl;
+    if (int rc = emb_order_plan(pl, key_item, nullptr, nullptr, nullptr, users, lens, R, B, n_items, n_users, g_item, g_user, scratch, scratch_bytes, s)) return rc;
+    if (int rc = emb_order_finish(pl, s)) return rc;
+    return emb_scatter_sums(pl, contrib, g_item, g_user, s);
+}
+
+}
```

After: 6.000 million (median of 6 runs). No clear change (+0.7%).
